# microsoft/tutel

Measured on AMD Instinct MI355X. Metric: MoE-layer fwd tokens/sec, 4096 tok x H=2048 x E=64 top-2, higher is better.
Workload: dtype bf16

## Files before the change

### include/tutel_amd.h

```cpp
#ifndef TUTEL_AMD_H
#define TUTEL_AMD_H

#include <stddef.h>
#include <stdint.h>

#ifdef __cplusplus
extern "C" {
#endif

#define TUTEL_AMD_ABI_VERSION 1

typedef void *tutel_stream_t;

enum { TUTEL_F32 = 0, TUTEL_F16 = 1, TUTEL_BF16 = 2, TUTEL_F64 = 3 };
enum { TUTEL_ACT_NONE = 0, TUTEL_ACT_RELU = 1, TUTEL_ACT_GELU = 2, TUTEL_ACT_SILU = 3 };

int tutel_amd_abi_version(void);
const char *tutel_amd_target_arch(void);
const char *tutel_amd_last_error(void);

size_t tutel_amd_routing_workspace_bytes(int T, int E, int k);

int tutel_amd_gate_topk(const void *in, int dtype, int apply_softmax, int T, int E, int k,
                        int normalize_gate, void *scores_out, int32_t *idx, void *gates, void *ws,
// ... 16 lines not shown

int tutel_amd_slot_map(const int32_t *idx, const int32_t *loc, int T, int E, int k, int capacity,
                       int32_t *slot_map, tutel_stream_t stream);

int tutel_amd_cumsum_sub_one(const int32_t *mask, int32_t *out, int T, int E,
                             tutel_stream_t stream);

int tutel_amd_fast_encode(const void *x, int dtype, const int32_t *slot_map, const void *gates,
                          int gate_dtype, int T, int M, int n_slots, int capacity, int num_experts,
                          int chunk_rows, int expert_slice, int ep_world, void *out,
                          tutel_stream_t stream);

int tutel_amd_fast_decode(const void *buf, int dtype, const int32_t *idx, const int32_t *loc,
                          const void *gates, int gate_dtype, int T, int M, int k, int capacity,
                          int num_experts, int chunk_rows, int expert_slice, int ep_world, void *out,
                          tutel_stream_t stream);

int tutel_amd_gate_grad(const void *x, const void *buf, int dtype, const int32_t *idx,
                        const int32_t *loc, int T, int M, int k, int capacity, float *ggate,
                        tutel_stream_t stream);

int tutel_amd_expert_gemm(const void *A, int64_t a_stride_e, int64_t a_stride_w, int a_rows_per_w,
                          int lda, const void *W, int w_kmajor, int64_t w_stride_e, int ldw,
                          const void *bias, int64_t bias_stride_e, void *D, int64_t d_stride_e,
                          int64_t d_stride_w, int d_rows_per_w, int ldd, int E_loc, int R, int N,
                          int K, int dtype, int act, const int32_t *row_counts, int row_align,
                          tutel_stream_t stream);

int tutel_amd_expert_gemm_gather(const void *X, int ldx, const int32_t *slot_map, int T,
                                 const void *zero_row, const void *W, int w_kmajor,
                                 int64_t w_stride_e, int ldw, const void *bias,
                                 int64_t bias_stride_e, void *D, int64_t d_stride_e, int ldd,
                                 int E_loc, int R, int N, int K, int dtype, int act,
                                 const int32_t *row_counts, int row_align, tutel_stream_t stream);

int tutel_amd_expert_ffn(const void *A, int64_t x_stride_e, int ldx, const int32_t *slot_map, int T, const void *zero_row,
                         const void *W1, int64_t w1_stride_e, int ldw1, const void *b1, int64_t b1_stride_e, void *hid,
                         int64_t hid_stride_e, int ldh, const void *W2, int64_t w2_stride_e, int ldw2, const void *b2,
                         int64_t b2_stride_e, void *D, int64_t d_stride_e, int ldd, int E_loc, int R, int M, int H, int M_out,
                         int dtype, int act, tutel_stream_t stream);

int tutel_amd_expert_gemm_glu(const void *A, int64_t a_stride_e, int64_t a_stride_w,
                              int a_rows_per_w, int lda, const void *W, int w_kmajor,
                              int64_t w_stride_e, int ldw, const void *bias, int64_t bias_stride_e,
                              const void *G, void *D, int64_t d_stride_e, int64_t d_stride_w,
                              int d_rows_per_w, int ldd, int E_loc, int R, int N, int K, int dtype,
                              int act, const int32_t *row_counts, int row_align,
                              tutel_stream_t stream);

int tutel_amd_expert_gemm_gate_up(const void *A, int64_t a_stride_e, int64_t a_stride_w, int a_rows_per_w, int lda,
                                  const void *W_gate, const void *W_up, int64_t w_stride_e, int ldw, void *D, int64_t d_stride_e,
                                  int64_t d_stride_w, int d_rows_per_w, int ldd, int E_loc, int R, int N, int K, int dtype, int act,
                                  const int32_t *row_counts, int row_align, tutel_stream_t stream);

typedef struct tutel_amd_ep_comm tutel_amd_ep_comm_t;
#define TUTEL_AMD_EP_ID_BYTES 128

int tutel_amd_ep_load_rccl(const char *path_hint );
int tutel_amd_ep_unique_id(void *out, size_t bytes );
int tutel_amd_ep_comm_create(const void *id, size_t bytes, int world, int rank, tutel_amd_ep_comm_t **out);
int tutel_amd_ep_comm_destroy(tutel_amd_ep_comm_t *comm);
typedef int (*tutel_amd_exchange_fn)(void *user, const void *send, void *recv, size_t bytes_per_peer, int world);
int tutel_amd_ep_comm_create_hosted(int world, int rank, tutel_amd_exchange_fn fn, void *user, tutel_amd_ep_comm_t **out);
int tutel_amd_ep_comm_info(const tutel_amd_ep_comm_t *comm, int *world, int *rank);

typedef struct tutel_amd_ep_segment tutel_amd_ep_segment_t;
#define TUTEL_AMD_IPC_HANDLE_BYTES 64
int tutel_amd_ep_segment_alloc(size_t bytes, int flag_memory, tutel_amd_ep_segment_t **out, void *handle_out, size_t handle_bytes);
int tutel_amd_ep_segment_open(tutel_amd_ep_segment_t *seg, int world, int rank, const void *handles, size_t handle_bytes);
void *tutel_amd_ep_segment_ptr(const tutel_amd_ep_segment_t *seg, int peer);
int tutel_amd_ep_segment_read(const tutel_amd_ep_segment_t *seg, size_t off, void *dst, size_t bytes, tutel_stream_t stream);
int tutel_amd_ep_segment_free(tutel_amd_ep_segment_t *seg);
size_t tutel_amd_ep_flag_bytes(void);
int tutel_amd_ep_comm_create_ipc(int world, int rank, tutel_amd_ep_comm_t **out);
int tutel_amd_ep_comm_attach_ipc(tutel_amd_ep_comm_t *comm, tutel_amd_ep_segment_t *flags, int timeout_ms);
int tutel_amd_ep_comm_has_ipc(const tutel_amd_ep_comm_t *comm);
int tutel_amd_ep_ipc_set_timeout(tutel_amd_ep_comm_t *comm, int timeout_ms);
int tutel_amd_ep_ipc_status(tutel_amd_ep_comm_t *comm);
int tutel_amd_ep_ipc_exchange(tutel_amd_ep_comm_t *comm, tutel_amd_ep_segment_t *seg, const void *send, size_t bytes_per_peer,
                              size_t recv_off, tutel_stream_t stream);
int tutel_amd_ep_ipc_selfcheck(tutel_amd_ep_comm_t *comm, tutel_amd_ep_segment_t *seg, size_t bytes_per_peer, int passes, int flavour,
                               int side_stream, unsigned long long *mismatch, tutel_stream_t stream);

int tutel_amd_ep_all_to_all(tutel_amd_ep_comm_t *comm, const void *send, void *recv, size_t bytes_per_peer,
                            tutel_stream_t stream);

typedef int (*tutel_amd_exchange_v_fn)(void *user, const void *send, void *recv, const uint64_t *send_bytes,
                                       const uint64_t *send_offsets, const uint64_t *recv_bytes, int world);
int tutel_amd_ep_comm_set_hosted_v(tutel_amd_ep_comm_t *comm, tutel_amd_exchange_v_fn fn);
int tutel_amd_ep_all_to_all_v(tutel_amd_ep_comm_t *comm, const void *send, void *recv, const uint64_t *send_bytes,
                              const uint64_t *recv_bytes, tutel_stream_t stream);
int tutel_amd_ep_all_gather_v(tutel_amd_ep_comm_t *comm, const void *send, void *recv, const uint64_t *recv_bytes,
                              tutel_stream_t stream);

typedef struct {
  int sliced;
  int experts_per_stage;
  int chunk;
  int rows;
  int gemm_rows;
} tutel_amd_ep_plan_t;
int tutel_amd_ep_plan(int num_experts, int world, int capacity, int degree, int allow_sliced, tutel_amd_ep_plan_t *out);

typedef struct {
  int T, M, H, M_out;
  int num_experts, world, k;
  int capacity;
  int degree;
  int allow_sliced;
  int dtype, gate_dtype, act;
  int is_postscore;
  int w2_kmajor;
  int fuse_encode;
  const void *x;
  const int32_t *slot_map;
  const int32_t *idx, *loc;
  const void *gates;
  const void *w1, *b1, *w2, *b2;
  void *enc, *recv, *hid, *send, *back;
  const void *zero_row;
  const int32_t *row_counts;
  int row_align;
  void *y;
  const struct tutel_amd_ep_segment *peer_seg;
} tutel_amd_ep_args_t;
int tutel_amd_ep_forward(tutel_amd_ep_comm_t *comm, const tutel_amd_ep_args_t *args, tutel_stream_t stream);

typedef struct {
  tutel_amd_ep_args_t ep;
  const void *logits;
  int logits_dtype;
  int normalize_gate;
  void *ws;
  size_t ws_bytes;
  int32_t *dispatch_count;
  int32_t *stats;
  void *l_aux;
  int capacity_limit, alignment, max_capacity;
  int *capacity_out;
  const void *gate_w;
  float *gate_partials;
  size_t gate_partial_bytes;
  void *logits_out;
  void *fl_ws;
  size_t fl_ws_bytes;
} tutel_amd_moe_args_t;
#define TUTEL_AMD_EAGAIN 1000
#define TUTEL_AMD_ENOTSUP 1001
int tutel_amd_moe_forward(tutel_amd_ep_comm_t *comm, const tutel_amd_moe_args_t *args, tutel_stream_t stream);

typedef struct {
  void *ws;
  size_t ws_bytes;
  int32_t *offsets;
  int32_t *capacity;
} tutel_amd_packed_args_t;
typedef struct {
  int rows_bound;
  int tiles_bound;
  int tile_rows;
  int row_limit;
  size_t ws_bytes;
} tutel_amd_packed_plan_t;
int tutel_amd_packed_plan(int T, int E, int k, int M, int H, int M_out, int dtype, int capacity_limit, int alignment,
                          tutel_amd_packed_plan_t *out);
size_t tutel_amd_moe_packed_workspace_bytes(int T, int E, int k, int M, int H, int M_out, int dtype, int capacity_limit,
                                            int alignment);
int tutel_amd_moe_forward_packed(tutel_amd_ep_comm_t *comm, const tutel_amd_moe_args_t *args,
                                 const tutel_amd_packed_args_t *packed, tutel_stream_t stream);
int tutel_amd_moe_forward_packed_glu(tutel_amd_ep_comm_t *comm, const tutel_amd_moe_args_t *args,
                                     const tutel_amd_packed_args_t *packed, const void *w_up, tutel_stream_t stream);

int tutel_amd_packed_layout(const int32_t *dispatch_count, const int32_t *idx, const int32_t *loc, int T, int E, int k,
                            int capacity_limit, int alignment, int rows_bound, int tiles_bound, int32_t *offsets, int32_t *tiles,
                            int32_t *ntiles, int32_t *capacity, int32_t *slot_map, tutel_stream_t stream);
int tutel_amd_expert_gemm_packed(const void *A, int lda, const int32_t *a_rows, int T, const void *zero_row, const void *W,
                                 int w_kmajor, int64_t w_stride_e, int ldw, const void *bias, int64_t bias_stride_e, const void *mul,
// ... 55 lines not shown
```

### tutel_amd/_lib.py

```python
import ctypes
import os
import subprocess

_HERE = os.path.dirname(os.path.abspath(__file__))
LIB_PATH = os.path.join(_HERE, "lib", "libtutel_amd.so")
CSRC_DIR = os.path.join(_HERE, "csrc")

F32, F16, BF16, F64 = 0, 1, 2, 3
ACT_NONE, ACT_RELU, ACT_GELU, ACT_SILU = 0, 1, 2, 3
OPT_GEMM_IMPL, OPT_GEMM_TILE, OPT_DECODE, OPT_EP_STAGE_GRID, OPT_GEMM_PERSIST, OPT_EP_STREAMS, OPT_EP_CANARY, OPT_GEMM_SPLITK, OPT_GEMM_GATHER, OPT_FUSED_LOCATION, OPT_GEMM_STORE, OPT_TIE_RULE, OPT_FFN_FUSED = 0, 1, 2, 3, 4, 5, 6, 7, 8, 9, 10, 11, 12

_vp, _i, _i64, _sz = ctypes.c_void_p, ctypes.c_int, ctypes.c_int64, ctypes.c_size_t

SIGNATURES = {
    "tutel_amd_abi_version": (_i, []),
    "tutel_amd_target_arch": (ctypes.c_char_p, []),
    "tutel_amd_last_error": (ctypes.c_char_p, []),
    "tutel_amd_routing_workspace_bytes": (_sz, [_i, _i, _i]),
    "tutel_amd_gate_topk": (_i, [_vp, _i, _i, _i, _i, _i, _i, _vp, _vp, _vp, _vp, _sz, _vp, _i, _vp]),
    "tutel_amd_gate_proj_splits": (_i, [_i, _i, _i, _i]),
    "tutel_amd_gate_proj": (_i, [_vp, _vp, _i, _i, _i, _i, _vp, _sz, _vp]),
    "tutel_amd_gate_topk_partials": (_i, [_vp, _i, _i, _i, _i, _i, _i, _vp, _vp, _vp, _vp, _vp, _sz, _vp, _i, _vp]),
    "tutel_amd_cache_warm": (_i, [_vp, _sz, _i, _sz, _i, _vp, _vp]),
    "tutel_amd_compute_location": (_i, [_vp, _i, _i, _i, _i, _vp, _sz, _vp, _vp, _vp, _vp, _i, _i, _vp, _i, _vp]),
    "tutel_amd_slot_map": (_i, [_vp, _vp, _i, _i, _i, _i, _vp, _vp]),
    "tutel_amd_cumsum_sub_one": (_i, [_vp, _vp, _i, _i, _vp]),
    "tutel_amd_fast_encode": (_i, [_vp, _i, _vp, _vp, _i, _i, _i, _i, _i, _i, _i, _i, _i, _vp, _vp]),
    "tutel_amd_fast_decode": (_i, [_vp, _i, _vp, _vp, _vp, _i, _i, _i, _i, _i, _i, _i, _i, _i, _vp, _vp]),
    "tutel_amd_gate_grad": (_i, [_vp, _vp, _i, _vp, _vp, _i, _i, _i, _i, _vp, _vp]),
    "tutel_amd_expert_gemm": (_i, [_vp, _i64, _i64, _i, _i, _vp, _i, _i64, _i, _vp, _i64, _vp, _i64,
                                   _i64, _i, _i, _i, _i, _i, _i, _i, _i, _vp, _i, _vp]),
    "tutel_amd_expert_gemm_gather": (_i, [_vp, _i, _vp, _i, _vp, _vp, _i, _i64, _i, _vp, _i64, _vp, _i64, _i,
                                          _i, _i, _i, _i, _i, _i, _vp, _i, _vp]),
    "tutel_amd_expert_ffn": (_i, [_vp, _i64, _i, _vp, _i, _vp, _vp, _i64, _i, _vp, _i64, _vp, _i64, _i, _vp, _i64, _i, _vp, _i64, _vp, _i64, _i,
                                  _i, _i, _i, _i, _i, _i, _i, _vp]),
    "tutel_amd_expert_gemm_glu": (_i, [_vp, _i64, _i64, _i, _i, _vp, _i, _i64, _i, _vp, _i64, _vp, _vp, _i64,
                                       _i64, _i, _i, _i, _i, _i, _i, _i, _i, _vp, _i, _vp]),
    "tutel_amd_expert_gemm_gate_up": (_i, [_vp, _i64, _i64, _i, _i, _vp, _vp, _i64, _i, _vp, _i64, _i64, _i, _i,
                                           _i, _i, _i, _i, _i, _i, _vp, _i, _vp]),
    "tutel_amd_set_option": (_i, [_i, _i]),
    "tutel_amd_probe_tr16": (_i, [_vp, _vp]),
}



class EpPlan(ctypes.Structure):
    _fields_ = [(n, _i) for n in ("sliced", "experts_per_stage", "chunk", "rows", "gemm_rows")]


class EpArgs(ctypes.Structure):
    _fields_ = ([(n, _i) for n in ("T", "M", "H", "M_out", "num_experts", "world", "k", "capacity", "degree", "allow_sliced",
                                   "dtype", "gate_dtype", "act", "is_postscore", "w2_kmajor", "fuse_encode")] +
                [(n, _vp) for n in ("x", "slot_map", "idx", "loc", "gates", "w1", "b1", "w2", "b2",
                                    "enc", "recv", "hid", "send", "back", "zero_row", "row_counts")] +
                [("row_align", _i), ("y", _vp), ("peer_seg", _vp)])


class MoeArgs(ctypes.Structure):
    _fields_ = [("ep", EpArgs), ("logits", _vp), ("logits_dtype", _i), ("normalize_gate", _i), ("ws", _vp), ("ws_bytes", _sz),
                ("dispatch_count", _vp), ("stats", _vp), ("l_aux", _vp),
                ("capacity_limit", _i), ("alignment", _i), ("max_capacity", _i), ("capacity_out", ctypes.POINTER(_i)),
                ("gate_w", _vp), ("gate_partials", _vp), ("gate_partial_bytes", _sz), ("logits_out", _vp),
                ("fl_ws", _vp), ("fl_ws_bytes", _sz)]


class PackedArgs(ctypes.Structure):
    _fields_ = [("ws", _vp), ("ws_bytes", _sz), ("offsets", _vp), ("capacity", _vp)]


class PackedPlan(ctypes.Structure):
    _fields_ = [("rows_bound", _i), ("tiles_bound", _i), ("tile_rows", _i), ("row_limit", _i), ("ws_bytes", _sz)]


SIGNATURES.update({
    "tutel_amd_moe_forward": (_i, [_vp, ctypes.POINTER(MoeArgs), _vp]),
    "tutel_amd_packed_plan": (_i, [_i] * 9 + [ctypes.POINTER(PackedPlan)]),
    "tutel_amd_moe_packed_workspace_bytes": (_sz, [_i] * 9),
    "tutel_amd_moe_forward_packed": (_i, [_vp, ctypes.POINTER(MoeArgs), ctypes.POINTER(PackedArgs), _vp]),
    "tutel_amd_moe_forward_packed_glu": (_i, [_vp, ctypes.POINTER(MoeArgs), ctypes.POINTER(PackedArgs), _vp, _vp]),
    "tutel_amd_packed_layout": (_i, [_vp, _vp, _vp] + [_i] * 7 + [_vp] * 6),
    "tutel_amd_expert_gemm_packed": (_i, [_vp, _i, _vp, _i, _vp, _vp, _i, _i64, _i, _vp, _i64, _vp, _vp] + [_i] * 7 + [_vp] * 4 + [_i, _vp]),
    "tutel_amd_expert_wgrad_packed": (_i, [_vp, _i, _vp, _i, _vp, _i, _i, _vp, _vp] + [_i] * 5 + [_vp, _vp]),
    "tutel_amd_expert_bgrad_packed": (_i, [_vp, _i, _vp, _i, _i, _i, _vp, _vp]),
    "tutel_amd_expert_wgrad_packed_f32": (_i, [_vp, _i, _vp, _i, _vp, _i, _i, _vp, _vp] + [_i] * 5 + [_vp, _vp]),
    "tutel_amd_expert_bgrad_packed_f32": (_i, [_vp, _i, _vp, _i, _i, _i, _vp, _vp]),
    "tutel_amd_gate_grad_packed": (_i, [_vp, _vp, _i, _vp, _vp] + [_i] * 4 + [_vp, _vp, _vp]),
    "tutel_amd_fast_decode_packed": (_i, [_vp, _i, _vp, _vp, _vp] + [_i] * 5 + [_vp, _vp, _vp]),
    "tutel_amd_ep_load_rccl": (_i, [ctypes.c_char_p]),
    "tutel_amd_ep_unique_id": (_i, [_vp, _sz]),
    "tutel_amd_ep_comm_create": (_i, [_vp, _sz, _i, _i, ctypes.POINTER(_vp)]),
    "tutel_amd_ep_comm_destroy": (_i, [_vp]),
    "tutel_amd_ep_comm_create_hosted": (_i, [_i, _i, _vp, _vp, ctypes.POINTER(_vp)]),
    "tutel_amd_ep_comm_info": (_i, [_vp, ctypes.POINTER(_i), ctypes.POINTER(_i)]),
    "tutel_amd_ep_all_to_all": (_i, [_vp, _vp, _vp, _sz, _vp]),
    "tutel_amd_ep_comm_set_hosted_v": (_i, [_vp, _vp]),
    "tutel_amd_ep_all_to_all_v": (_i, [_vp, _vp, _vp, ctypes.POINTER(ctypes.c_uint64), ctypes.POINTER(ctypes.c_uint64), _vp]),
    "tutel_amd_ep_all_gather_v": (_i, [_vp, _vp, _vp, ctypes.POINTER(ctypes.c_uint64), _vp]),
    "tutel_amd_ep_plan": (_i, [_i, _i, _i, _i, _i, ctypes.POINTER(EpPlan)]),
    "tutel_amd_ep_forward": (_i, [_vp, ctypes.POINTER(EpArgs), _vp]),
    "tutel_amd_ep_segment_alloc": (_i, [_sz, _i, ctypes.POINTER(_vp), _vp, _sz]),
    "tutel_amd_ep_segment_open": (_i, [_vp, _i, _i, _vp, _sz]),
    "tutel_amd_ep_segment_ptr": (_vp, [_vp, _i]),
    "tutel_amd_ep_segment_read": (_i, [_vp, _sz, _vp, _sz, _vp]),
    "tutel_amd_ep_segment_free": (_i, [_vp]),
    "tutel_amd_ep_flag_bytes": (_sz, []),
    "tutel_amd_ep_comm_create_ipc": (_i, [_i, _i, ctypes.POINTER(_vp)]),
    "tutel_amd_ep_comm_attach_ipc": (_i, [_vp, _vp, _i]),
    "tutel_amd_ep_comm_has_ipc": (_i, [_vp]),
# ... 64 lines not shown
```

### tutel_amd/csrc/common.h

```cpp
#pragma once
#include <hip/hip_runtime.h>
#include <stdint.h>
#include <stdio.h>
#include <string.h>

#include "../../include/tutel_amd.h"

#define WAVE 64

void tutel_set_error(const char *fmt, ...);
int tutel_get_option(int key);

int tutel_stage_begin(int stage, hipStream_t st);
void tutel_stage_end(int token, hipStream_t st);
void tutel_stage_hint(int stage);
void tutel_gemm_corun_hint(int on);
int tutel_gemm_corun();
void tutel_stage_range_push(int stage);
void tutel_stage_range_pop();
struct StageScope {
  int token;
  hipStream_t st;
  StageScope(int stage, hipStream_t s) : token(tutel_stage_begin(stage, s)), st(s) { tutel_stage_range_push(stage); }
  ~StageScope() {
    tutel_stage_end(token, st);
    tutel_stage_range_pop();
  }
};

#define EP_NCAN 16
struct PeerCanary {
  const uint32_t *epoch;
  long long off;
  int world;
  int stale;
};
struct EncodePeer {
  const uint64_t *tab;
  long long off;
  int rank, rows;
  int slot0;
  PeerCanary can;
};
int tutel_encode_launch(const void *x, int dtype, const int32_t *slot_map, const void *gates, int gate_dtype, int T, int M,
                        int n_slots, int capacity, int num_experts, int chunk_rows, int expert_slice, int ep_world, void *out,
                        const EncodePeer &peer, hipStream_t st);
int tutel_expert_gemm_peer(const void *A, int64_t a_stride_e, int64_t a_stride_w, int a_rows_per_w, int lda, const void *W,
                           int w_kmajor, int64_t w_stride_e, int ldw, const void *bias, int64_t bias_stride_e,
                           const uint64_t *d_peer, int64_t d_peer_off, int64_t d_stride_e, int d_rows_per_w, int ldd, int E_loc,
                           int R, int N, int K, int dtype, int act, const PeerCanary &can, hipStream_t st);

int tutel_expert_gemm_gather_fl(const void *X, int ldx, int32_t *slot_map, int T, const void *zero_row, const void *W, int64_t w_stride_e,
                                int ldw, const void *bias, int64_t bias_stride_e, void *D, int64_t d_stride_e, int ldd, int E_loc, int R,
                                int N, int K, int dtype, int act, const uint8_t *idx8, int n, int32_t *loc, hipStream_t st);
int tutel_expert_ffn(const void *X, int64_t x_stride_e, int ldx, const int32_t *slot_map, int T, const void *zero_row, const void *W1,
                     int64_t w1_stride_e, int ldw1, const void *b1, int64_t b1_stride_e, void *hid, int64_t hid_stride_e, int ldh,
                     const void *W2, int64_t w2_stride_e, int ldw2, const void *b2, int64_t b2_stride_e, void *D, int64_t d_stride_e, int ldd,
                     int E_loc, int R, int M, int H, int M_out, int dtype, int act, const uint8_t *idx8, int n, int32_t *loc, int query,
                     hipStream_t st);
struct RouteFinish;
void tutel_route_finish_args(int T, int E, int k, void *ws, RouteFinish *out);
int tutel_decode_finish_launch(const void *buf, int dtype, const int32_t *idx, const int32_t *loc, const void *gates, int gate_dtype, int T, int M,
                               int k, int capacity, int num_experts, void *out, const RouteFinish &fin, hipStream_t st);
#define PK_TILE_ROWS 256
int tutel_expert_gemm_packed(const void *A, int lda, const int32_t *a_rows, int T, const void *zero_row, const void *W, int64_t w_stride_e,
                             int ldw, const void *bias, int64_t bias_stride_e, void *D, int ldd, int E, int rows_bound, int N, int K, int dtype,
                             int act, const int32_t *off, const int32_t *tiles, const int32_t *ntiles, const int32_t *cap, int tiles_bound,
                             hipStream_t st);
int tutel_expert_gemm_packed_ex(const void *A, int lda, const int32_t *a_rows, int T, const void *zero_row, const void *W, int w_kmajor,
                                int64_t w_stride_e, int ldw, const void *bias, int64_t bias_stride_e, const void *mul, void *D, int ldd, int E,
                                int rows_bound, int N, int K, int dtype, int act, const int32_t *off, const int32_t *tiles, const int32_t *ntiles,
                                const int32_t *cap, int tiles_bound, hipStream_t st);
int tutel_expert_gemm_gate_up_packed(const void *A, int lda, const int32_t *a_rows, int T, const void *zero_row, const void *W_gate,
                                     const void *W_up, int64_t w_stride_e, int ldw, void *D, int ldd, int E, int rows_bound, int N, int K,
                                     int dtype, int act, const int32_t *off, const int32_t *tiles, const int32_t *ntiles, const int32_t *cap,
                                     int tiles_bound, hipStream_t st);
int tutel_decode_packed_launch(const void *buf, int dtype, const int32_t *idx, const int32_t *loc, const void *gates, int gate_dtype, int T,
                               int M, int k, int row_limit, const int32_t *off, void *out, hipStream_t st);
int tutel_gate_topk_launch(const void *in, const float *partials, int splits, int dtype, int T, int E, int k, int normalize_gate,
                           void *logits_out, int32_t *idx, void *gates, void *ws, int32_t *clear_map, int clear_n, uint8_t *idx8,
                           hipStream_t st);

#define TUTEL_REQUIRE(cond, ...)           \
  do {                                     \
    if (!(cond)) {                         \
      tutel_set_error(__VA_ARGS__);        \
      return -1;                           \
    }                                      \
  } while (0)

#define TUTEL_CHECK_LAUNCH(what)                                                    \
  do {                                                                              \
    hipError_t _e = hipGetLastError();                                              \
    if (_e != hipSuccess) {                                                         \
      tutel_set_error("%s: launch failed: %s", what, hipGetErrorString(_e));        \
      return (int)_e;                                                               \
    }                                                                               \
  } while (0)

struct bf16_t { uint16_t v; };
struct f16_t { _Float16 v; };

__device__ __forceinline__ uint16_t f32_to_bf16_bits(float f) {
  uint32_t u = __float_as_uint(f);
  if ((u & 0x7fffffffu) > 0x7f800000u) return 0x7fc0;
  u += 0x7fffu + ((u >> 16) & 1u);
  return (uint16_t)(u >> 16);
// ... 127 lines not shown
```

### tutel_amd/csrc/ep.hip

```cpp
#include <dlfcn.h>
#include <stdlib.h>

#include <vector>

#include <rccl/rccl.h>

#include "common.h"
#include "routing_dev.h"

struct RcclApi {
  void *handle;
  ncclResult_t (*GetUniqueId)(ncclUniqueId *);
  ncclResult_t (*CommInitRank)(ncclComm_t *, int, ncclUniqueId, int);
  ncclResult_t (*CommDestroy)(ncclComm_t);
  ncclResult_t (*AllToAll)(const void *, void *, size_t, ncclDataType_t, ncclComm_t, hipStream_t);
  const char *(*GetErrorString)(ncclResult_t);
  ncclResult_t (*GroupStart)();
  ncclResult_t (*GroupEnd)();
  ncclResult_t (*Send)(const void *, size_t, ncclDataType_t, int, ncclComm_t, hipStream_t);
  ncclResult_t (*Recv)(void *, size_t, ncclDataType_t, int, ncclComm_t, hipStream_t);
};
static RcclApi g_rccl = {};

extern "C" int tutel_amd_ep_load_rccl(const char *path) {
// ... 646 lines not shown

extern "C" int tutel_amd_ep_plan(int E, int W, int capacity, int degree, int allow_sliced, tutel_amd_ep_plan_t *out) {
  TUTEL_REQUIRE(out != nullptr && E >= 1 && W >= 1 && E % W == 0 && degree >= 1 && degree <= EP_MAX_SPLIT && capacity >= 0,
                "tutel_amd_ep_plan: bad sizes E=%d W=%d C=%d degree=%d", E, W, capacity, degree);
  const int E_loc = E / W;
  out->sliced = (allow_sliced && E_loc >= degree && E_loc % degree == 0) ? 1 : 0;
  if (out->sliced) {
    out->experts_per_stage = E_loc / degree;
    out->chunk = capacity;
  } else {
    TUTEL_REQUIRE(capacity % degree == 0, "tutel_amd_ep_plan: capacity %d is not a multiple of a2a_ffn_overlap_degree %d", capacity, degree);
    out->experts_per_stage = E_loc;
    out->chunk = capacity / degree;
  }
  out->rows = out->experts_per_stage * out->chunk;
  out->gemm_rows = W * out->chunk;
  return 0;
}

extern "C" int tutel_amd_ep_forward(tutel_amd_ep_comm_t *c, const tutel_amd_ep_args_t *a, tutel_stream_t stream) {
  TUTEL_REQUIRE(a != nullptr, "tutel_amd_ep_forward: null arguments");
  const int W = a->world, E = a->num_experts, C = a->capacity, T = a->T, M = a->M, H = a->H, Mo = a->M_out, k = a->k;
  TUTEL_REQUIRE(W >= 1 && E >= 1 && E % W == 0 && T >= 0 && M >= 1 && H >= 1 && Mo >= 1 && k >= 1 && C >= 0,
                "tutel_amd_ep_forward: bad sizes");
  TUTEL_REQUIRE(c == nullptr ? W == 1 : c->world == W, "tutel_amd_ep_forward: communicator world size does not match (%d)", W);
  TUTEL_REQUIRE(a->dtype == TUTEL_BF16 || a->dtype == TUTEL_F16, "tutel_amd_ep_forward: bf16 / fp16 experts only (got dtype %d)", a->dtype);
  TUTEL_REQUIRE((T == 0 || (a->x && a->idx && a->loc && a->y)) && (a->slot_map || C == 0) && a->w1 && a->w2, "tutel_amd_ep_forward: null pointer");
  if (T == 0 && c == nullptr) return 0;
  const int E_loc = E / W, es = 2;
  hipStream_t cur = (hipStream_t)stream;
  const void *enc_gates = a->is_postscore ? nullptr : a->gates;
  const void *dec_gates = a->is_postscore ? a->gates : nullptr;
  TUTEL_REQUIRE(a->gates != nullptr || T == 0, "tutel_amd_ep_forward: null gates");
  TUTEL_REQUIRE(a->row_counts == nullptr || (W == 1 && c == nullptr && a->degree <= 1), "tutel_amd_ep_forward: row counts (megablocks) need a single rank");
  const int32_t *rcnt = a->row_counts;
  const int ralign = a->row_counts != nullptr && a->row_align >= 1 ? a->row_align : 1;

  if (C == 0) {
    if (T > 0) HIP_CHECK(hipMemsetAsync(a->y, 0, (size_t)T * Mo * es, cur), "hipMemsetAsync");
    return 0;
  }

  if (c == nullptr && a->degree <= 1 && a->is_postscore && a->fuse_encode) {
    TUTEL_REQUIRE(a->hid && a->send && a->zero_row, "tutel_amd_ep_forward: null workspace");
    int rc = TUTEL_AMD_ENOTSUP;
    if (rcnt == nullptr && a->w2_kmajor) {
      Range r("tutel_amd.expert_ffn");
      rc = tutel_expert_ffn(a->x, 0, M, a->slot_map, T, a->zero_row, a->w1, (int64_t)H * M, M, a->b1, H, a->hid, (int64_t)C * H, H, a->w2,
                            (int64_t)H * Mo, H, a->b2, Mo, a->send, (int64_t)C * Mo, Mo, E_loc, C, M, H, Mo, a->dtype, a->act, nullptr, 0, nullptr, 0, cur);
      if (rc != 0 && rc != TUTEL_AMD_ENOTSUP) return rc;
    }
    if (rc == TUTEL_AMD_ENOTSUP) {
      Range r("tutel_amd.expert_fc1");
      rc = tutel_amd_expert_gemm_gather(a->x, M, a->slot_map, T, a->zero_row, a->w1, 1, (int64_t)H * M, M, a->b1, H, a->hid,
                                        (int64_t)C * H, H, E_loc, C, H, M, a->dtype, a->act, rcnt, ralign, cur);
      if (rc) return rc;
      Range r2("tutel_amd.expert_fc2");
      rc = tutel_amd_expert_gemm(a->hid, (int64_t)C * H, 0, C, H, a->w2, a->w2_kmajor, (int64_t)H * Mo, a->w2_kmajor ? H : Mo, a->b2,
                                 Mo, a->send, (int64_t)C * Mo, 0, C, Mo, E_loc, C, Mo, H, a->dtype, TUTEL_ACT_NONE, rcnt, ralign, cur);
      if (rc) return rc;
    }
    Range r("tutel_amd.fast_decode");
    return tutel_amd_fast_decode(a->send, a->dtype, a->idx, a->loc, dec_gates, a->gate_dtype, T, Mo, k, C, E, 0, 0, 1, a->y, cur);
  }

  const bool ipc = a->peer_seg != nullptr;
  TUTEL_REQUIRE(a->recv && a->hid && a->back && (ipc || (a->enc && a->send)), "tutel_amd_ep_forward: null workspace");
  TUTEL_REQUIRE(rcnt == nullptr, "tutel_amd_ep_forward: row counts need the fused-encode single-rank route (is_postscore, fuse_encode)");
  const int degree = a->degree < 1 ? 1 : a->degree;
  tutel_amd_ep_plan_t pl;
  if (tutel_amd_ep_plan(E, W, C, degree, a->allow_sliced, &pl) != 0) return -1;
  const int s = pl.experts_per_stage, cc = pl.chunk, rows = pl.rows, R = pl.gemm_rows;
  const int chunk_rows = pl.sliced ? 0 : cc, expert_slice = pl.sliced ? s : 0;
  int rc;

  const size_t msg_in = (size_t)W * rows * M * es, msg_out = (size_t)W * rows * Mo * es;
  const size_t hid_stage = (size_t)s * R * H * es;
  const tutel_amd_ep_segment *seg = a->peer_seg;
  long long recv_off = 0, back_off = 0;
  if (ipc) {
    if (ipc_check(c, "tutel_amd_ep_forward") != 0) return -1;
    TUTEL_REQUIRE(seg->tab_dev != nullptr && seg->world == W && seg->rank == c->rank, "tutel_amd_ep_forward: the peer segment is not open for this communicator");
    recv_off = (const char *)a->recv - (const char *)seg->local;
    back_off = (const char *)a->back - (const char *)seg->local;
    TUTEL_REQUIRE(recv_off >= 0 && back_off >= 0 && (size_t)recv_off + degree * msg_in <= seg->bytes && (size_t)back_off + degree * msg_out <= seg->bytes &&
                      recv_off % 16 == 0 && back_off % 16 == 0,
                  "tutel_amd_ep_forward: recv / back must lie inside the peer segment");
  }
  auto stage_gemms = [&](int i, hipStream_t st) -> int {
    const char *recv_i = (const char *)a->recv + (size_t)i * msg_in;
    char *hid_i = (char *)a->hid + (size_t)i * hid_stage;
    const int e0 = pl.sliced ? i * s : 0;
    const char *w1 = (const char *)a->w1 + (size_t)e0 * H * M * es, *w2 = (const char *)a->w2 + (size_t)e0 * H * Mo * es;
    const char *b1 = a->b1 ? (const char *)a->b1 + (size_t)e0 * H * es : nullptr, *b2 = a->b2 ? (const char *)a->b2 + (size_t)e0 * Mo * es : nullptr;
    int r1;
    {
      Range r("tutel_amd.expert_fc1");
      tutel_stage_hint(TUTEL_STAGE_FC1);
      r1 = tutel_amd_expert_gemm(recv_i, (int64_t)cc * M, (int64_t)rows * M, cc, M, w1, 1, (int64_t)H * M, M, b1, H, hid_i,
                                 (int64_t)R * H, 0, R, H, s, R, H, M, a->dtype, a->act, nullptr, 1, st);
      tutel_stage_hint(-1);
      if (r1) return r1;
    }
    Range r("tutel_amd.expert_fc2");
    if (ipc)
      return tutel_expert_gemm_peer(hid_i, (int64_t)R * H, 0, R, H, w2, a->w2_kmajor, (int64_t)H * Mo, a->w2_kmajor ? H : Mo, b2, Mo, seg->tab_dev,
                                    back_off + (long long)(((size_t)i * W + c->rank) * rows * Mo * es), (int64_t)cc * Mo, cc, Mo, s, R, Mo, H, a->dtype,
                                    TUTEL_ACT_NONE, producer_canary(c, seg, 1, i), st);
    char *send_i = (char *)a->send + (size_t)i * msg_out;
    return tutel_amd_expert_gemm(hid_i, (int64_t)R * H, 0, R, H, w2, a->w2_kmajor, (int64_t)H * Mo, a->w2_kmajor ? H : Mo, b2, Mo, send_i,
                                 (int64_t)cc * Mo, (int64_t)rows * Mo, cc, Mo, s, R, Mo, H, a->dtype, TUTEL_ACT_NONE, nullptr, 1, st);
  };
// ... 135 lines not shown
    splits = tutel_amd_gate_proj_splits(T, a.M, E, a.dtype);
    TUTEL_REQUIRE(splits > 0, "tutel_amd_moe_forward: the in-call gate projection does not cover T=%d, M=%d, E=%d, dtype=%d (pass logits)", T, a.M, E, a.dtype);
    TUTEL_REQUIRE(a.x != nullptr && m->gate_partials != nullptr && m->gate_partial_bytes >= (size_t)splits * T * E * sizeof(float),
                  "tutel_amd_moe_forward: gate_partials must hold %d x %d x %d floats", splits, T, E);
  }
  TUTEL_REQUIRE(a.slot_map && (T == 0 || (a.idx && a.loc && a.gates)), "tutel_amd_moe_forward: null routing buffers");
  if (T == 0 && c == nullptr) return 0;
  const bool dropless = a.capacity <= 0;
  TUTEL_REQUIRE(!dropless || (c == nullptr && a.world == 1 && m->stats != nullptr && m->capacity_out != nullptr && m->max_capacity >= 1),
                "tutel_amd_moe_forward: dropless routing needs a single rank, stats, capacity_out and max_capacity");
  int32_t *smap = const_cast<int32_t *>(a.slot_map);
  int rc;
  const int Ho = a.H, Mo = a.M_out;
  bool fl = !dropless && c == nullptr && a.world == 1 && a.degree <= 1 && a.is_postscore && a.fuse_encode && T > 0 && k <= 8 && E <= 128 &&
            (long long)k * T <= 15360 && m->fl_ws != nullptr && m->fl_ws_bytes >= (((size_t)k * T + 15) & ~(size_t)15) &&
            (a.dtype == TUTEL_BF16 || a.dtype == TUTEL_F16) && a.row_counts == nullptr && a.hid && a.send && a.zero_row && a.loc && a.w1 &&
            ((uintptr_t)m->fl_ws & 15) == 0;
  if (fl) {
    TUTEL_REQUIRE(k >= 1 && k <= E, "tutel_amd_moe_forward: need 1 <= k <= E (got k=%d, E=%d)", k, E);
    TUTEL_REQUIRE(m->ws_bytes >= tutel_amd_routing_workspace_bytes(T, E, k), "tutel_amd_moe_forward: routing workspace too small (%zu bytes, need %zu)",
                  m->ws_bytes, tutel_amd_routing_workspace_bytes(T, E, k));
  }
  if (fl) {
    char keep[512];
    strncpy(keep, tutel_amd_last_error(), sizeof(keep) - 1);
    keep[sizeof(keep) - 1] = 0;
    fl = tutel_expert_gemm_gather_fl(a.x, a.M, smap, T, a.zero_row, a.w1, (int64_t)Ho * a.M, a.M, a.b1, Ho, a.hid, (int64_t)a.capacity * Ho, Ho, E,
                                     a.capacity, Ho, a.M, a.dtype, a.act, (const uint8_t *)m->fl_ws, k * T, nullptr, (hipStream_t)stream) == 0;
    if (!fl) tutel_set_error("%s", keep);
  }
  if (fl) {
    hipStream_t st = (hipStream_t)stream;
    uint8_t *idx8 = (uint8_t *)m->fl_ws;
    if (project) {
      rc = tutel_amd_gate_proj(a.x, m->gate_w, a.dtype, T, a.M, E, m->gate_partials, m->gate_partial_bytes, stream);
      if (rc) return rc;
    }
    rc = tutel_gate_topk_launch(project ? nullptr : m->logits, project ? m->gate_partials : nullptr, splits, m->logits_dtype, T, E, k,
                                m->normalize_gate, project ? m->logits_out : nullptr, const_cast<int32_t *>(a.idx), const_cast<void *>(a.gates),
                                m->ws, nullptr, 0, idx8, st);
    if (rc) return rc;
    if (m->capacity_out != nullptr) *m->capacity_out = a.capacity;
    rc = TUTEL_AMD_ENOTSUP;
    if (a.w2_kmajor) {
      Range r("tutel_amd.expert_ffn");
      rc = tutel_expert_ffn(a.x, 0, a.M, smap, T, a.zero_row, a.w1, (int64_t)Ho * a.M, a.M, a.b1, Ho, a.hid, (int64_t)a.capacity * Ho, Ho, a.w2,
                            (int64_t)Ho * Mo, Ho, a.b2, Mo, a.send, (int64_t)a.capacity * Mo, Mo, E, a.capacity, a.M, Ho, Mo, a.dtype, a.act, idx8, k * T,
                            const_cast<int32_t *>(a.loc), 0, st);
      if (rc != 0 && rc != TUTEL_AMD_ENOTSUP) return rc;
    }
    if (rc == TUTEL_AMD_ENOTSUP) {
      Range r("tutel_amd.expert_fc1");
      rc = tutel_expert_gemm_gather_fl(a.x, a.M, smap, T, a.zero_row, a.w1, (int64_t)Ho * a.M, a.M, a.b1, Ho, a.hid, (int64_t)a.capacity * Ho, Ho,
                                       E, a.capacity, Ho, a.M, a.dtype, a.act, idx8, k * T, const_cast<int32_t *>(a.loc), st);
      if (rc) return rc;
      Range r2("tutel_amd.expert_fc2");
      rc = tutel_amd_expert_gemm(a.hid, (int64_t)a.capacity * Ho, 0, a.capacity, Ho, a.w2, a.w2_kmajor, (int64_t)Ho * Mo, a.w2_kmajor ? Ho : Mo,
                                 a.b2, Mo, a.send, (int64_t)a.capacity * Mo, 0, a.capacity, Mo, E, a.capacity, Mo, Ho, a.dtype, TUTEL_ACT_NONE,
                                 nullptr, 1, stream);
      if (rc) return rc;
    }
    Range r("tutel_amd.fast_decode");
    RouteFinish fin;
    tutel_route_finish_args(T, E, k, m->ws, &fin);
    fin.on = 1;
    fin.dispatch_count = m->dispatch_count;
    fin.stats = m->stats;
    fin.l_aux = m->l_aux;
    fin.l_aux_dtype = m->logits_dtype;
    return tutel_decode_finish_launch(a.send, a.dtype, a.idx, a.loc, a.gates, m->logits_dtype, T, Mo, k, a.capacity, E, a.y, fin, st);
  }
  if (project && T > 0) {
    rc = tutel_amd_gate_proj(a.x, m->gate_w, a.dtype, T, a.M, E, m->gate_partials, m->gate_partial_bytes, stream);
    if (rc) return rc;
    rc = tutel_amd_gate_topk_partials(m->gate_partials, splits, a.dtype, T, E, k, m->normalize_gate, m->logits_out, nullptr,
                                      const_cast<int32_t *>(a.idx), const_cast<void *>(a.gates), m->ws, m->ws_bytes,
                                      dropless ? nullptr : smap, dropless ? 0 : E * a.capacity, stream);
  } else {
    rc = tutel_amd_gate_topk(m->logits, m->logits_dtype, 1, T, E, k, m->normalize_gate, nullptr, const_cast<int32_t *>(a.idx),
                             const_cast<void *>(a.gates), m->ws, m->ws_bytes, dropless ? nullptr : smap, dropless ? 0 : E * a.capacity, stream);
  }
  if (rc) return rc;
  rc = tutel_amd_compute_location(a.idx, T, E, k, 1, m->ws, m->ws_bytes, const_cast<int32_t *>(a.loc), m->dispatch_count, m->stats,
                                  m->l_aux, m->logits_dtype, dropless ? 0 : a.capacity, dropless ? nullptr : smap, dropless ? 0 : 1, stream);
  if (rc) return rc;
  tutel_amd_ep_args_t e = a;
  e.gate_dtype = m->logits_dtype;
  if (dropless) {
    hipStream_t st = (hipStream_t)stream;
    HIP_CHECK(hipMemcpyAsync(m->capacity_out, m->stats, sizeof(int), hipMemcpyDeviceToHost, st), "hipMemcpyAsync");
    HIP_CHECK(hipStreamSynchronize(st), "hipStreamSynchronize");
    int cap = *m->capacity_out;
    if (m->capacity_limit > 0 && cap > m->capacity_limit) cap = m->capacity_limit;
    const int al = m->alignment >= 1 ? m->alignment : 1;
    cap = (cap + al - 1) / al * al;
    *m->capacity_out = cap;
    if (cap > m->max_capacity) return TUTEL_AMD_EAGAIN;
    if (cap == 0) return hipMemsetAsync(a.y, 0, (size_t)T * a.M_out * 2, st) == hipSuccess ? 0 : -1;
    rc = tutel_amd_slot_map(a.idx, a.loc, T, E, k, cap, smap, stream);
    if (rc) return rc;
    e.capacity = cap;
  } else if (m->capacity_out != nullptr) {
    *m->capacity_out = a.capacity;
  }
  return tutel_amd_ep_forward(c, &e, stream);
}
```

### tutel_amd/csrc/expert_gemm.hip

```cpp
#include <stdlib.h>

#include <mutex>

#include "common.h"

#include "gemm_dev.h"

template <typename T, bool W_KMAJOR, int ACT, bool NT, bool ROT, bool PACKED = false>
__global__ __launch_bounds__(GM_THREADS, 2) void expert_gemm_kernel(GemmArgs p) {
  constexpr int BK = 64, NBUF = 2;
  constexpr int LDK = BK + 8;
  constexpr int A_TILE = GM_BM * LDK;
  constexpr int W_TILE = W_KMAJOR ? GM_BN * LDK : BK * GM_LDN;
  constexpr int CPR = BK / 8;
  constexpr int RPP = GM_THREADS / CPR;
  constexpr int NLA = GM_BM / RPP;
  constexpr int NLW = W_KMAJOR ? GM_BN / RPP : BK / 16;
  extern __shared__ __attribute__((aligned(16))) unsigned char smem[];
  uint16_t *sA = reinterpret_cast<uint16_t *>(smem);
  uint16_t *sW = sA + NBUF * A_TILE;

  const int tid = threadIdx.x, lane = tid & 63, wid = tid >> 6;
  const int wm = wid >> 1, wn = wid & 1;

  int nb = gridDim.x;
  if (PACKED) {
    nb = min(nb, __builtin_amdgcn_readfirstlane(*p.pk_ntiles) * 2 * p.ntn);
    if ((int)blockIdx.x >= nb) return;
  }
  int w;
  {
    const int b = blockIdx.x, q = nb >> 3, r = nb & 7, xcd = b & 7, pos = b >> 3;
    w = (xcd < r ? xcd * (q + 1) : r * (q + 1) + (xcd - r) * q) + pos;
  }
  int nt, e, m0, row_limit;
  bool rot_on = p.rot_on;
  if (PACKED) {
    const int h = w / p.ntn, ti = h >> 1;
    nt = w % p.ntn;
    e = __builtin_amdgcn_readfirstlane(p.pk_tiles[2 * ti]);
    m0 = __builtin_amdgcn_readfirstlane(p.pk_tiles[2 * ti + 1]) + (h & 1) * GM_BM;
    row_limit = __builtin_amdgcn_readfirstlane(p.pk_off[e + 1]);
    rot_on = __builtin_amdgcn_readfirstlane(*p.pk_cap) < GB_BM;
  } else {
    const int mt = w % p.ntm;
    nt = (w / p.ntm) % p.ntn;
    e = w / (p.ntm * p.ntn);
    m0 = mt * GM_BM;
    row_limit = p.R;
    if (p.row_counts != nullptr) {
      int c = p.row_counts[e];
      c = (c + p.row_align - 1) / p.row_align * p.row_align;
      row_limit = min(row_limit, c);
    }
  }
  const int n0 = nt * GM_BN;
  if (m0 >= row_limit) return;

  const uint16_t *Ae = reinterpret_cast<const uint16_t *>(p.A) + (size_t)e * p.a_stride_e;
// ... 220 lines not shown
  do {                                                                                 \
    _Pragma("unroll") for (int mi = 0; mi < 2; ++mi)                                   \
      FA[mi] = *reinterpret_cast<const u32x4 *>(ca + a_row + mi * 32 * GL_BK + frag_k[KK]); \
    _Pragma("unroll") for (int ni = 0; ni < 2; ++ni) {                                 \
      if (W_KMAJOR) {                                                                  \
        FW[ni] = *reinterpret_cast<const u32x4 *>(cw + wk_row + ni * 32 * GL_BK + frag_k[KK]); \
      } else {                                                                         \
        const uint16_t *ptr = cw + wt_row + (KK) * 16 * GM_BN + (ni ? wt_c1 : wt_c0);  \
        s16x4_t lo = __builtin_amdgcn_ds_read_tr16_b64_v4i16(                          \
            (__attribute__((address_space(3))) s16x4_t *)(ptr));                       \
        s16x4_t hi = __builtin_amdgcn_ds_read_tr16_b64_v4i16(                          \
            (__attribute__((address_space(3))) s16x4_t *)(ptr + 4 * GM_BN));           \
        u32x2 lo2 = __builtin_bit_cast(u32x2, lo), hi2 = __builtin_bit_cast(u32x2, hi); \
        u32x4 f = {lo2[0], lo2[1], hi2[0], hi2[1]};                                    \
        FW[ni] = f;                                                                    \
      }                                                                                \
    }                                                                                  \
  } while (0)
#define GL_MMA(FA, FW)                                                                 \
  do {                                                                                 \
    _Pragma("unroll") for (int ni = 0; ni < 2; ++ni)                                   \
      _Pragma("unroll") for (int mi = 0; mi < 2; ++mi)                                 \
        acc[ni][mi] = Mma<T>::run(FW[ni], FA[mi], acc[ni][mi]);                        \
  } while (0)

  GL_ISSUE(0, 0);
  __syncthreads();

  for (int kt = 0; kt < nk; ++kt) {
    const int buf = kt & 1;
    if (kt + 1 < nk) GL_ISSUE(kt + 1, buf ^ 1);

    const uint16_t *ca = sA + buf * GL_STAGE, *cw = sW + buf * GL_STAGE;
    u32x4 fa[4][2], fw[4][2];
    GL_LOAD_FRAGS(fa[0], fw[0], 0);
    GL_LOAD_FRAGS(fa[1], fw[1], 1);
    GL_LOAD_FRAGS(fa[2], fw[2], 2);
    GL_LOAD_FRAGS(fa[3], fw[3], 3);
    __builtin_amdgcn_sched_barrier(0);
    GL_MMA(fa[0], fw[0]);
    GL_MMA(fa[1], fw[1]);
    GL_MMA(fa[2], fw[2]);
    GL_MMA(fa[3], fw[3]);

    __syncthreads();
  }
#undef GL_ISSUE
#undef GL_LOAD_FRAGS
#undef GL_MMA

  gemm_epilogue<T, ACT>(p, acc, bias_r, e, m0, n0, wm, wn, l31, kg, row_limit);
}

template <typename T, bool W_KMAJOR, int ACT, int NI, int NS, bool BUF = false, int BM = GB_BM, bool FL = false>
__global__ __launch_bounds__(BM * 2, 2) void expert_gemm_big_kernel(GemmArgs p) {
  extern __shared__ __attribute__((aligned(16))) unsigned char smem[];
  const int nb = gridDim.x;
  int w;
  {
    const int b = blockIdx.x, q = nb >> 3, r = nb & 7, xcd = b & 7, pos = b >> 3;
    w = (xcd < r ? xcd * (q + 1) : r * (q + 1) + (xcd - r) * q) + pos;
  }
  gemm_big_tile<T, W_KMAJOR, ACT, NI, NS, BUF, BM, FL>(p, w / (p.ntm * p.ntn), w % p.ntm, (w / p.ntm) % p.ntn, smem);
}

#define PP_BUF (4 * GL_STAGE)

template <typename T, int ACT, bool W_ONCE, bool RAGGED = false, bool EARLY_BIAS = false, bool SPLITK = false, bool PACKED = false,
          bool GATE_UP = false>
__global__ __launch_bounds__(GB_THREADS, 2) void expert_gemm_pp_kernel(GemmArgs p) {
  extern __shared__ __attribute__((aligned(16))) unsigned char smem[];
  uint16_t *lds = reinterpret_cast<uint16_t *>(smem);

  const int tid = threadIdx.x, lane = tid & 63;
  const int wid = __builtin_amdgcn_readfirstlane(tid >> 6);
  const int wm = wid >> 1, wn = wid & 1;

  static_assert(!(PACKED && SPLITK), "the packed layout never splits K");
  static_assert(!GATE_UP || (!SPLITK && !EARLY_BIAS), "the gate/up form: no split, no bias");
  constexpr bool packed = PACKED;
  int nb = gridDim.x;
  if (packed) {
    nb = min(nb, __builtin_amdgcn_readfirstlane(*p.pk_ntiles) * p.ntn);
    if ((int)blockIdx.x >= nb) return;
  }
  int w;
  {
    const int b = blockIdx.x, q = nb >> 3, r = nb & 7, xcd = b & 7, pos = b >> 3;
    w = (xcd < r ? xcd * (q + 1) : r * (q + 1) + (xcd - r) * q) + pos;
  }
  const int half = SPLITK ? (w & 1) : 0;
  if (SPLITK) w >>= 1;
  const int tile_id = w;
  int e, nt, m0, row_limit;
  bool rot_on = p.rot_on;
  if constexpr (packed) {
    const int ti = w / p.ntn;
    nt = w % p.ntn;
    e = __builtin_amdgcn_readfirstlane(p.pk_tiles[2 * ti]);
    m0 = __builtin_amdgcn_readfirstlane(p.pk_tiles[2 * ti + 1]);
    row_limit = __builtin_amdgcn_readfirstlane(p.pk_off[e + 1]);
    rot_on = __builtin_amdgcn_readfirstlane(*p.pk_cap) < GB_BM;
  } else {
    const int mt = w % p.ntm;
    nt = (w / p.ntm) % p.ntn;
    e = w / (p.ntm * p.ntn);
    m0 = mt * GB_BM;
    row_limit = p.R;
    if (p.row_counts != nullptr) {
      int c = p.row_counts[e];
      c = (c + p.row_align - 1) / p.row_align * p.row_align;
      row_limit = min(row_limit, c);
    }
  }
  const int n0 = nt * (GATE_UP ? 128 : 256);
  if (m0 >= row_limit) return;
// ... 314 lines not shown
  const size_t lds = (size_t)8 * 64 * EP_PITCH;
  auto kern = expert_gemm_pp_kernel<T, ACT, false, false, false, true>;
  if (!tutel_lds_optin((const void *)kern, lds)) return -1;
  hipLaunchKernelGGL(kern, dim3((unsigned)(2 * tiles)), dim3(GB_THREADS), lds, st, b);
  TUTEL_CHECK_LAUNCH("tutel_amd_expert_gemm");
  return 0;
}

template <typename T, int ACT>
static int launch_pp(const GemmArgs &a, hipStream_t st) {
  GemmArgs b = a;
  b.ntm = (a.R + GB_BM - 1) / GB_BM;
  b.ntn = (a.N + 255) / 256;
  const int tail_rows = b.R % GB_BM;
  const bool ragged = b.row_counts != nullptr || (tail_rows != 0 && tail_rows <= GB_BM - 32);
  const bool early = tutel_get_option(TUTEL_OPT_GEMM_PERSIST) != 0;
  if (b.ntm == 1 && (long long)b.E_loc * b.ntn >= 256)
    return ragged ? launch_pp_cfg<T, ACT, true, true>(b, st) : (early ? launch_pp_cfg<T, ACT, true, false, true>(b, st) : launch_pp_cfg<T, ACT, true>(b, st));
  return ragged ? launch_pp_cfg<T, ACT, false, true>(b, st) : (early ? launch_pp_cfg<T, ACT, false, false, true>(b, st) : launch_pp_cfg<T, ACT, false>(b, st));
}

template <typename T, int ACT>
static int launch_pp_packed(const GemmArgs &a, int tiles_bound, hipStream_t st) {
  GemmArgs b = a;
  b.ntm = 1;
  b.ntn = (a.N + 255) / 256;
  const long long grid = (long long)tiles_bound * b.ntn;
  TUTEL_REQUIRE(grid >= 1 && grid < 0x7fffffffLL, "tutel_expert_gemm_packed: grid too large");
  const size_t lds = (size_t)8 * 64 * EP_PITCH;
  auto kern = (long long)a.E_loc * b.ntn >= 256 ? expert_gemm_pp_kernel<T, ACT, true, true, false, false, true>
                                                 : expert_gemm_pp_kernel<T, ACT, false, true, false, false, true>;
  if (!tutel_lds_optin((const void *)kern, lds)) return -1;
  hipLaunchKernelGGL(kern, dim3((unsigned)grid), dim3(GB_THREADS), lds, st, b);
  TUTEL_CHECK_LAUNCH("tutel_expert_gemm_packed");
  return 0;
}

template <typename T, int ACT, bool PACKED>
static int launch_gate_up(const GemmArgs &a, int tiles_bound, hipStream_t st) {
  GemmArgs b = a;
  b.ntm = PACKED ? 1 : (a.R + GB_BM - 1) / GB_BM;
  b.ntn = (a.N + 127) / 128;
  const long long grid = PACKED ? (long long)tiles_bound * b.ntn : (long long)a.E_loc * b.ntm * b.ntn;
  TUTEL_REQUIRE(grid >= 1 && grid < 0x7fffffffLL, "tutel_amd_expert_gemm_gate_up: grid too large");
  const size_t lds = (size_t)8 * 64 * EP_PITCH;
  auto kern = PACKED && (long long)a.E_loc * b.ntn >= 256 ? expert_gemm_pp_kernel<T, ACT, PACKED, true, false, false, PACKED, true>
                                                          : expert_gemm_pp_kernel<T, ACT, false, true, false, false, PACKED, true>;
  if (!tutel_lds_optin((const void *)kern, lds)) return -1;
  hipLaunchKernelGGL(kern, dim3((unsigned)grid), dim3(GB_THREADS), lds, st, b);
  TUTEL_CHECK_LAUNCH("tutel_amd_expert_gemm_gate_up");
  return 0;
}

template <typename T, bool KM, int ACT, int NI, int NS = 2, bool BUF = false, int BM = GB_BM, bool FL = false>
static int launch_big(const GemmArgs &a, hipStream_t st) {
  GemmArgs b = a;
  b.ntm = (a.R + BM - 1) / BM;
  b.ntn = (a.N + NI * 64 - 1) / (NI * 64);
  const size_t lds_k = (size_t)NS * (BM / 128 + NI / 2) * GL_STAGE * 2 + (FL ? 16384 : 0), lds_e = BUF ? (size_t)(BM / 32) * 64 * (NI * 64 + 16) : 0;
  const size_t lds = lds_k > lds_e ? lds_k : lds_e;
  auto kern = expert_gemm_big_kernel<T, KM, ACT, NI, NS, BUF, BM, FL>;
  if (!tutel_lds_optin((const void *)kern, lds)) return -1;
  hipLaunchKernelGGL(kern, dim3(a.E_loc * b.ntm * b.ntn), dim3(BM * 2), lds, st, b);
  TUTEL_CHECK_LAUNCH("tutel_amd_expert_gemm");
  return 0;
}

template <typename T, bool KM, int ACT>
static int launch_glds(const GemmArgs &a, int grid, hipStream_t st) {
  hipLaunchKernelGGL((expert_gemm_glds_kernel<T, KM, ACT, true, true>), dim3(grid), dim3(GM_THREADS),
                     (size_t)4 * GL_STAGE * 2, st, a);
  TUTEL_CHECK_LAUNCH("tutel_amd_expert_gemm");
  return 0;
}

__global__ void probe_tr16_kernel(uint16_t *out) {
  __shared__ __attribute__((aligned(16))) uint16_t lds[256];
  const int l = threadIdx.x;
  for (int i = l; i < 256; i += 64) lds[i] = (uint16_t)i;
  __syncthreads();
  s16x4_t t = __builtin_amdgcn_ds_read_tr16_b64_v4i16((__attribute__((address_space(3))) s16x4_t *)(lds + l * 4));
#pragma unroll
  for (int j = 0; j < 4; ++j) out[l * 4 + j] = (uint16_t)t[j];
}

extern "C" int tutel_amd_probe_tr16(uint16_t *out, tutel_stream_t stream) {
  TUTEL_REQUIRE(out != nullptr, "tutel_amd_probe_tr16: null pointer");
  hipLaunchKernelGGL(probe_tr16_kernel, dim3(1), dim3(64), 0, (hipStream_t)stream, out);
  TUTEL_CHECK_LAUNCH("tutel_amd_probe_tr16");
  return 0;
}

static constexpr size_t gemm_lds_bytes(bool kmajor) {
  return (size_t)(2 * GM_BM * (64 + 8) + 2 * (kmajor ? GM_BN * (64 + 8) : 64 * GM_LDN)) * 2;
}

template <typename T, bool KM, int ACT>
static int launch_cfg(const GemmArgs &a, int grid, hipStream_t st) {
  const size_t lds = gemm_lds_bytes(KM);
  auto kern = expert_gemm_kernel<T, KM, ACT, true, true>;
  if (lds > 65536 && !tutel_lds_optin((const void *)kern, lds)) return -1;
  hipLaunchKernelGGL(kern, dim3(grid), dim3(GM_THREADS), lds, st, a);
  TUTEL_CHECK_LAUNCH("tutel_amd_expert_gemm");
  return 0;
}

template <typename T, bool KM, int ACT>
static int launch_gemm(const GemmArgs &a, int grid, hipStream_t st) {
  const int impl = tutel_get_option(TUTEL_OPT_GEMM_IMPL), big = tutel_get_option(TUTEL_OPT_GEMM_TILE);
  const bool ring256_ok = KM && a.fits32 && a.N >= 256 && a.R <= GM_BM;
  const bool ring256 = ring256_ok && (impl == 4 || (impl < 0 && (long long)a.E_loc * ((a.N + 255) / 256) >= 256));
  if (a.fl_idx8 != nullptr) {
    if (!(ring256 && KM && big <= 0 && a.a_rows != nullptr && a.row_counts == nullptr && a.fl_n >= 1 && a.fl_n <= 15360 && a.E_loc <= 128 && a.K >= 2 * GL_BK)) {
      tutel_set_error("tutel_expert_gemm_gather_fl: this launch does not take the fused-location ring kernel");
      return TUTEL_AMD_ENOTSUP;
    }
    if (a.fl_loc == nullptr) return 0;
    return launch_big<T, true, ACT, 4, 3, true, 128, KM>(a, st);
  }
  if (a.N >= GM_BN && big != 0) {
    const long long mt256 = (long long)a.E_loc * ((a.R + GB_BM - 1) / GB_BM);
    const long long t256 = mt256 * ((a.N + 255) / 256), t128 = mt256 * ((a.N + 127) / 128);
    const bool corun_pp = tutel_gemm_corun() && big < 0 && a.R > GM_BM && t256 >= 96 && t256 < 192;
    if (KM && a.fits32 && a.mul == nullptr && a.R > GM_BM && t256 >= 96 && t256 < 192 && (big < 0 || big == 4) &&
        tutel_get_option(TUTEL_OPT_GEMM_SPLITK) == 1) {
      const int rc = launch_pp_splitk<T, ACT>(a, st);
      if (rc <= 0) return rc;
    }
    const bool pp_one_round = big < 0 && a.R > GM_BM && t256 > 128 && t256 < 192;
    if (KM && a.fits32 && (big == 4 || corun_pp || pp_one_round || (big < 0 && a.R > GM_BM && t256 >= 192))) return launch_pp<T, ACT>(a, st);
    if (big == 1 || big == 4 || (big < 0 && a.R > GM_BM && t256 >= 192)) return launch_big<T, KM, ACT, 4>(a, st);
    if (KM && big == 2) return launch_big<T, true, ACT, 2, 2>(a, st);
    if (KM && (big == 3 || (big < 0 && a.R > GM_BM && t128 >= 192)))
      return a.fits32 && tutel_get_option(TUTEL_OPT_GEMM_IMPL) != 2 ? launch_big<T, true, ACT, 2, 3, true>(a, st) : launch_big<T, true, ACT, 2, 3>(a, st);
  }
  if (ring256) return launch_big<T, true, ACT, 4, 3, true, 128>(a, st);
  const bool use_dma = impl < 0 ? KM : (impl == 1 || impl == 4);
  if (use_dma) return launch_glds<T, KM, ACT>(a, grid, st);
  return launch_cfg<T, KM, ACT>(a, grid, st);
}

template <typename T, bool KM>
static int launch_gemm_act(const GemmArgs &a, int act, int grid, hipStream_t st) {
  switch (act) {
    case TUTEL_ACT_NONE: return launch_gemm<T, KM, TUTEL_ACT_NONE>(a, grid, st);
    case TUTEL_ACT_RELU: return launch_gemm<T, KM, TUTEL_ACT_RELU>(a, grid, st);
    case TUTEL_ACT_GELU: return launch_gemm<T, KM, TUTEL_ACT_GELU>(a, grid, st);
    case TUTEL_ACT_SILU: return launch_gemm<T, KM, TUTEL_ACT_SILU>(a, grid, st);
    default: tutel_set_error("tutel_amd_expert_gemm: unknown activation %d", act); return -1;
  }
}

int tutel_gemm_args(const void *A, int64_t a_stride_e, int64_t a_stride_w, int a_rows_per_w, int lda, const void *W, int w_kmajor,
                    int64_t w_stride_e, int ldw, const void *bias, int64_t bias_stride_e, void *D, int64_t d_stride_e, int64_t d_stride_w,
                    int d_rows_per_w, int ldd, int E_loc, int R, int N, int K, int dtype, int act, const int32_t *row_counts, int row_align,
                    const int32_t *a_rows, int a_rows_mod, const void *a_zero, const void *mul, const uint64_t *d_peer, int64_t d_peer_off,
                    const PeerCanary *d_can, const uint8_t *fl_idx8, int fl_n, int32_t *fl_loc, GemmArgs *out) {
  (void)w_kmajor; (void)act;
  TUTEL_REQUIRE(dtype == TUTEL_BF16 || dtype == TUTEL_F16, "tutel_amd_expert_gemm: dtype must be bf16 or fp16 (got %d)", dtype);
  TUTEL_REQUIRE(E_loc >= 0 && R >= 0 && N >= 1 && K >= 1, "tutel_amd_expert_gemm: bad sizes E_loc=%d R=%d N=%d K=%d", E_loc, R, N, K);
  TUTEL_REQUIRE(K % 64 == 0, "tutel_amd_expert_gemm: K=%d must be a multiple of 64", K);
  TUTEL_REQUIRE(N % 8 == 0, "tutel_amd_expert_gemm: N=%d must be a multiple of 8", N);
  if (E_loc == 0 || R == 0) return 1;
  TUTEL_REQUIRE(A && W && (D || d_peer), "tutel_amd_expert_gemm: null pointer");
  TUTEL_REQUIRE(d_peer == nullptr || (mul == nullptr && d_peer_off % 16 == 0), "tutel_amd_expert_gemm: peer stores exclude the gated form");
  TUTEL_REQUIRE(a_rows_per_w >= 1 && d_rows_per_w >= 1, "tutel_amd_expert_gemm: rows_per_w must be >= 1");
  TUTEL_REQUIRE(lda % 8 == 0 && ldw % 8 == 0 && ldd % 4 == 0 && a_stride_e % 8 == 0 && a_stride_w % 8 == 0 &&
                    w_stride_e % 8 == 0 && d_stride_e % 4 == 0 && d_stride_w % 4 == 0 && bias_stride_e % 4 == 0,
                "tutel_amd_expert_gemm: leading dimensions / strides must keep rows 16-byte aligned");
  TUTEL_REQUIRE(((uintptr_t)A % 16) == 0 && ((uintptr_t)W % 16) == 0 && ((uintptr_t)D % 8) == 0 && ((uintptr_t)bias % 8) == 0,
                "tutel_amd_expert_gemm: pointers must be 16-byte aligned");
  TUTEL_REQUIRE(row_counts == nullptr || row_align >= 1, "tutel_amd_expert_gemm: row_align must be >= 1");

  GemmArgs &a = *out;
  a.A = A; a.a_stride_e = a_stride_e; a.a_stride_w = a_stride_w; a.a_rpw = a_rows_per_w; a.lda = lda;
  a.W = W; a.w_stride_e = w_stride_e; a.ldw = ldw;
  a.bias = bias; a.bias_stride_e = bias_stride_e;
  a.D = D; a.d_stride_e = d_stride_e; a.d_stride_w = d_stride_w; a.d_rpw = d_rows_per_w; a.ldd = ldd;
  a.E_loc = E_loc; a.R = R; a.N = N; a.K = K;
  a.row_counts = row_counts; a.row_align = row_align < 1 ? 1 : row_align;
  a.a_rows = a_rows; a.a_rows_mod = a_rows_mod; a.a_zero = a_zero;
  a.a_span_bytes = 0;
  bool fits32 = true;
  {
    const long long span = a_rows != nullptr ? (long long)a_rows_mod * lda * 2
                                             : ((long long)((R - 1) / a_rows_per_w) * a_stride_w + (long long)a_rows_per_w * lda) * 2;
    fits32 = span < 0x7ffff000LL;
    a.a_span_bytes = (int)span;
  }
  fits32 = fits32 && ((long long)N * ldw + K) * 2 < 0xffffff00LL;
  a.fits32 = fits32;
  a.rot_on = R < GB_BM;
  a.sgather = tutel_get_option(TUTEL_OPT_GEMM_GATHER) != 0 && (long long)E_loc * R * 4 < 0x7fffffffLL;
  {
    const int ds = tutel_get_option(TUTEL_OPT_GEMM_STORE);
    const long long span = ((long long)((R - 1) / d_rows_per_w) * (d_stride_w < 0 ? -d_stride_w : d_stride_w) + (long long)(d_rows_per_w < R ? d_rows_per_w : R) * ldd + N) * 2;
    a.d_store = (ds == 0 || span >= 0x7fffffffLL) ? 0 : (ds == 2 ? 2 : 1);
    if (d_peer != nullptr) {
      const long long pspan = ((long long)E_loc * d_stride_e + (long long)d_rows_per_w * ldd + N) * 2;
      a.d_store = (ds != 0 && d_rows_per_w % 8 == 0 && pspan < 0x7fffffffLL) ? 1 : 0;
    }
  }
  a.mul = mul;
  a.fl_idx8 = fl_idx8; a.fl_n = fl_n; a.fl_loc = fl_loc;
  a.d_peer = d_peer; a.d_peer_off = d_peer_off;
  a.d_can = d_can != nullptr ? *d_can : PeerCanary{nullptr, 0, 0, 0};
  TUTEL_REQUIRE(((uintptr_t)mul % 8) == 0, "tutel_amd_expert_gemm_glu: gating operand must be 8-byte aligned");
  TUTEL_REQUIRE(a_rows == nullptr || (a_rows_mod >= 1 && a_zero != nullptr && ((uintptr_t)a_zero % 16) == 0),
                "tutel_amd_expert_gemm_gather: need a_rows_mod >= 1 and a 16-byte aligned zero row");
  a.ntm = (R + GM_BM - 1) / GM_BM;
  a.ntn = (N + GM_BN - 1) / GM_BN;
  a.pk_off = a.pk_tiles = a.pk_ntiles = a.pk_cap = nullptr;
  a.w_up = nullptr;
  return 0;
}

static int expert_gemm_impl(const void *A, int64_t a_stride_e, int64_t a_stride_w,
                                     int a_rows_per_w, int lda, const void *W, int w_kmajor,
                                     int64_t w_stride_e, int ldw, const void *bias,
                                     int64_t bias_stride_e, void *D, int64_t d_stride_e,
                                     int64_t d_stride_w, int d_rows_per_w, int ldd, int E_loc,
                                     int R, int N, int K, int dtype, int act,
                                     const int32_t *row_counts, int row_align,
                                     const int32_t *a_rows, int a_rows_mod, const void *a_zero,
                                     const void *mul, tutel_stream_t stream, const uint64_t *d_peer = nullptr,
                                     int64_t d_peer_off = 0, const PeerCanary *d_can = nullptr, const uint8_t *fl_idx8 = nullptr,
                                     int fl_n = 0, int32_t *fl_loc = nullptr) {
  GemmArgs a;
  const int brc = tutel_gemm_args(A, a_stride_e, a_stride_w, a_rows_per_w, lda, W, w_kmajor, w_stride_e, ldw, bias, bias_stride_e, D, d_stride_e,
                                  d_stride_w, d_rows_per_w, ldd, E_loc, R, N, K, dtype, act, row_counts, row_align, a_rows, a_rows_mod, a_zero, mul,
                                  d_peer, d_peer_off, d_can, fl_idx8, fl_n, fl_loc, &a);
  if (brc != 0) return brc < 0 ? brc : 0;
  long long grid_ll = (long long)E_loc * a.ntm * a.ntn;
  TUTEL_REQUIRE(grid_ll < 0x7fffffffLL, "tutel_amd_expert_gemm: grid too large");
  const int grid = (int)grid_ll;
  hipStream_t st = (hipStream_t)stream;
  auto go = [&]() -> int {
    if (dtype == TUTEL_BF16)
      return w_kmajor ? launch_gemm_act<bf16_t, true>(a, act, grid, st) : launch_gemm_act<bf16_t, false>(a, act, grid, st);
    return w_kmajor ? launch_gemm_act<f16_t, true>(a, act, grid, st) : launch_gemm_act<f16_t, false>(a, act, grid, st);
  };
  if (fl_idx8 != nullptr && fl_loc == nullptr) return go();
  StageScope stage(act != TUTEL_ACT_NONE ? TUTEL_STAGE_FC1 : TUTEL_STAGE_FC2, st);
  return go();
}

extern "C" int tutel_amd_expert_gemm(const void *A, int64_t a_stride_e, int64_t a_stride_w,
                                     int a_rows_per_w, int lda, const void *W, int w_kmajor,
                                     int64_t w_stride_e, int ldw, const void *bias,
                                     int64_t bias_stride_e, void *D, int64_t d_stride_e,
                                     int64_t d_stride_w, int d_rows_per_w, int ldd, int E_loc,
                                     int R, int N, int K, int dtype, int act,
                                     const int32_t *row_counts, int row_align,
                                     tutel_stream_t stream) {
  return expert_gemm_impl(A, a_stride_e, a_stride_w, a_rows_per_w, lda, W, w_kmajor, w_stride_e, ldw, bias,
                          bias_stride_e, D, d_stride_e, d_stride_w, d_rows_per_w, ldd, E_loc, R, N, K, dtype, act,
                          row_counts, row_align, nullptr, 0, nullptr, nullptr, stream);
}

int tutel_expert_gemm_peer(const void *A, int64_t a_stride_e, int64_t a_stride_w, int a_rows_per_w, int lda, const void *W,
                           int w_kmajor, int64_t w_stride_e, int ldw, const void *bias, int64_t bias_stride_e,
                           const uint64_t *d_peer, int64_t d_peer_off, int64_t d_stride_e, int d_rows_per_w, int ldd, int E_loc,
                           int R, int N, int K, int dtype, int act, const PeerCanary &can, hipStream_t st) {
  TUTEL_REQUIRE(d_peer != nullptr, "tutel_expert_gemm_peer: null peer table");
  return expert_gemm_impl(A, a_stride_e, a_stride_w, a_rows_per_w, lda, W, w_kmajor, w_stride_e, ldw, bias, bias_stride_e, nullptr,
                          d_stride_e, 0, d_rows_per_w, ldd, E_loc, R, N, K, dtype, act, nullptr, 1, nullptr, 0, nullptr, nullptr,
                          (tutel_stream_t)st, d_peer, d_peer_off, &can);
}

int tutel_expert_gemm_gather_fl(const void *X, int ldx, int32_t *slot_map, int T, const void *zero_row, const void *W, int64_t w_stride_e,
                                int ldw, const void *bias, int64_t bias_stride_e, void *D, int64_t d_stride_e, int ldd, int E_loc, int R,
                                int N, int K, int dtype, int act, const uint8_t *idx8, int n, int32_t *loc, hipStream_t st) {
  TUTEL_REQUIRE(slot_map != nullptr && idx8 != nullptr && T >= 1 && ((uintptr_t)idx8 & 15) == 0, "tutel_expert_gemm_gather_fl: bad arguments");
  if (tutel_get_option(TUTEL_OPT_FUSED_LOCATION) == 0) return TUTEL_AMD_ENOTSUP;
  return expert_gemm_impl(X, 0, 0, R > 0 ? R : 1, ldx, W, 1, w_stride_e, ldw, bias, bias_stride_e, D, d_stride_e, 0, R > 0 ? R : 1, ldd, E_loc,
                          R, N, K, dtype, act, nullptr, 1, slot_map, T, zero_row, nullptr, (tutel_stream_t)st, nullptr, 0, nullptr, idx8, n, loc);
}

extern "C" int tutel_amd_expert_gemm_glu(const void *A, int64_t a_stride_e, int64_t a_stride_w,
                                         int a_rows_per_w, int lda, const void *W, int w_kmajor,
                                         int64_t w_stride_e, int ldw, const void *bias,
                                         int64_t bias_stride_e, const void *G, void *D, int64_t d_stride_e,
                                         int64_t d_stride_w, int d_rows_per_w, int ldd, int E_loc,
                                         int R, int N, int K, int dtype, int act,
                                         const int32_t *row_counts, int row_align,
                                         tutel_stream_t stream) {
  TUTEL_REQUIRE(G != nullptr || E_loc == 0 || R == 0, "tutel_amd_expert_gemm_glu: null gating operand");
  return expert_gemm_impl(A, a_stride_e, a_stride_w, a_rows_per_w, lda, W, w_kmajor, w_stride_e, ldw, bias,
                          bias_stride_e, D, d_stride_e, d_stride_w, d_rows_per_w, ldd, E_loc, R, N, K, dtype, act,
                          row_counts, row_align, nullptr, 0, nullptr, G, stream);
}

extern "C" int tutel_amd_expert_gemm_gather(const void *X, int ldx, const int32_t *slot_map, int T,
                                            const void *zero_row, const void *W, int w_kmajor,
                                            int64_t w_stride_e, int ldw, const void *bias,
                                            int64_t bias_stride_e, void *D, int64_t d_stride_e, int ldd,
                                            int E_loc, int R, int N, int K, int dtype, int act,
                                            const int32_t *row_counts, int row_align,
                                            tutel_stream_t stream) {
  TUTEL_REQUIRE(slot_map != nullptr && T >= 1, "tutel_amd_expert_gemm_gather: need a slot map and T >= 1");
  return expert_gemm_impl(X, 0, 0, R > 0 ? R : 1, ldx, W, w_kmajor, w_stride_e, ldw, bias, bias_stride_e, D,
                          d_stride_e, 0, R > 0 ? R : 1, ldd, E_loc, R, N, K, dtype, act, row_counts, row_align,
                          slot_map, T, zero_row, nullptr, stream);
}

int tutel_expert_gemm_packed(const void *A, int lda, const int32_t *a_rows, int T, const void *zero_row, const void *W, int64_t w_stride_e,
                             int ldw, const void *bias, int64_t bias_stride_e, void *D, int ldd, int E, int rows_bound, int N, int K, int dtype,
                             int act, const int32_t *off, const int32_t *tiles, const int32_t *ntiles, const int32_t *cap, int tiles_bound,
                             hipStream_t st) {
  return tutel_expert_gemm_packed_ex(A, lda, a_rows, T, zero_row, W, 1, w_stride_e, ldw, bias, bias_stride_e, nullptr, D, ldd, E, rows_bound, N,
                                     K, dtype, act, off, tiles, ntiles, cap, tiles_bound, st);
}

template <typename T, int ACT>
static int launch_packed_nmajor(const GemmArgs &a, int tiles_bound, hipStream_t st) {
  GemmArgs b = a;
  b.ntm = 1;
  b.ntn = (a.N + GM_BN - 1) / GM_BN;
  const long long grid = (long long)tiles_bound * 2 * b.ntn;
  TUTEL_REQUIRE(grid >= 1 && grid < 0x7fffffffLL, "tutel_amd_expert_gemm_packed: grid too large");
  const size_t lds = gemm_lds_bytes(false);
  auto kern = expert_gemm_kernel<T, false, ACT, true, true, true>;
  if (lds > 65536 && !tutel_lds_optin((const void *)kern, lds)) return -1;
  hipLaunchKernelGGL(kern, dim3((unsigned)grid), dim3(GM_THREADS), lds, st, b);
  TUTEL_CHECK_LAUNCH("tutel_amd_expert_gemm_packed");
  return 0;
}

int tutel_expert_gemm_packed_ex(const void *A, int lda, const int32_t *a_rows, int T, const void *zero_row, const void *W, int w_kmajor,
                                int64_t w_stride_e, int ldw, const void *bias, int64_t bias_stride_e, const void *mul, void *D, int ldd, int E,
// ... 88 lines not shown
```

### tutel_amd/csrc/gemm_dev.h

```cpp
#pragma once
#include "common.h"

#ifndef GEMM_PROBE
#define GEMM_PROBE(i)
#endif

struct GemmArgs;
int tutel_gemm_args(const void *A, int64_t a_stride_e, int64_t a_stride_w, int a_rows_per_w, int lda, const void *W, int w_kmajor,
                    int64_t w_stride_e, int ldw, const void *bias, int64_t bias_stride_e, void *D, int64_t d_stride_e, int64_t d_stride_w,
                    int d_rows_per_w, int ldd, int E_loc, int R, int N, int K, int dtype, int act, const int32_t *row_counts, int row_align,
                    const int32_t *a_rows, int a_rows_mod, const void *a_zero, const void *mul, const uint64_t *d_peer, int64_t d_peer_off,
                    const PeerCanary *d_can, const uint8_t *fl_idx8, int fl_n, int32_t *fl_loc, GemmArgs *out);
bool tutel_lds_optin(const void *kern, size_t lds);

#define GM_BM 128
#define GM_BN 128
#define GM_THREADS 256
#define GM_LDN (GM_BN + 32)

typedef __attribute__((ext_vector_type(16))) float f32x16;
typedef __attribute__((ext_vector_type(8))) __bf16 bf16x8_t;
typedef __attribute__((ext_vector_type(8))) _Float16 f16x8_t;
typedef __attribute__((ext_vector_type(4))) short s16x4_t;
typedef __attribute__((ext_vector_type(4))) uint32_t u32x4;
typedef __attribute__((ext_vector_type(2))) uint32_t u32x2;
typedef int sgv4 __attribute__((ext_vector_type(4)));
typedef int sgv8 __attribute__((ext_vector_type(8)));

template <typename T> struct Mma;
template <> struct Mma<bf16_t> {
  __device__ static __forceinline__ f32x16 run(u32x4 a, u32x4 b, f32x16 c) {
    return __builtin_amdgcn_mfma_f32_32x32x16_bf16(__builtin_bit_cast(bf16x8_t, a),
                                                  __builtin_bit_cast(bf16x8_t, b), c, 0, 0, 0);
  }
};
template <> struct Mma<f16_t> {
  __device__ static __forceinline__ f32x16 run(u32x4 a, u32x4 b, f32x16 c) {
    return __builtin_amdgcn_mfma_f32_32x32x16_f16(__builtin_bit_cast(f16x8_t, a),
                                                 __builtin_bit_cast(f16x8_t, b), c, 0, 0, 0);
  }
};

#define GEMM_ACT_RUNTIME 99
template <int ACT> __device__ __forceinline__ float activate(float v) {
  if (ACT == TUTEL_ACT_RELU) return fmaxf(v, 0.f);
  if (ACT == TUTEL_ACT_GELU) return 0.5f * v * (1.f + erff(v * 0.70710678118654752440f));
  if (ACT == TUTEL_ACT_SILU) return v / (1.f + expf(-v));
  return v;
}

#define GM_PRELOAD_BIAS() GM_PRELOAD_BIAS_N(2)
#define GM_PRELOAD_BIAS_N(NI_)                                                                    \
  uint2 bias_r[NI_][4];                                                                           \
  {                                                                                               \
    const uint16_t *be_ = p.bias ? reinterpret_cast<const uint16_t *>(p.bias) + (size_t)e * p.bias_stride_e : nullptr; \
    _Pragma("unroll") for (int ni_ = 0; ni_ < NI_; ++ni_)                                         \
      _Pragma("unroll") for (int rg_ = 0; rg_ < 4; ++rg_) {                                       \
        int n_ = n0 + wn * (NI_ * 32) + ni_ * 32 + rg_ * 8 + kg * 4;                              \
        n_ = n_ < p.N ? n_ : p.N - 4;                                                             \
        bias_r[ni_][rg_] = be_ ? *reinterpret_cast<const uint2 *>(be_ + n_) : make_uint2(0u, 0u); \
      }                                                                                           \
  }

struct GemmArgs {
  const void *A; long long a_stride_e, a_stride_w; int a_rpw, lda;
  const void *W; long long w_stride_e; int ldw;
  const void *bias; long long bias_stride_e;
  void *D; long long d_stride_e, d_stride_w; int d_rpw, ldd;
  int E_loc, R, N, K;
  const int32_t *row_counts; int row_align;
  const int32_t *a_rows; int a_rows_mod; const void *a_zero;
  int a_span_bytes;
  bool fits32;
  bool rot_on;
  bool sgather;
  int d_store;
  const uint8_t *fl_idx8; int fl_n; int32_t *fl_loc;
  const void *mul;
  const uint64_t *d_peer; long long d_peer_off;
  PeerCanary d_can;
  float *sk_ws; uint32_t *sk_flags;
  int ntm, ntn;
  int act_rt;
  const int32_t *pk_off, *pk_tiles, *pk_ntiles, *pk_cap;
  const void *w_up;
};

__device__ __forceinline__ uint16_t *gemm_out_row(const GemmArgs &p, int e, int m) {
  const int w = m / p.d_rpw, l = m % p.d_rpw;
  if (p.d_peer != nullptr)
    return reinterpret_cast<uint16_t *>(p.d_peer[w] + p.d_peer_off) + (size_t)e * p.d_stride_e + (size_t)l * p.ldd;
  return reinterpret_cast<uint16_t *>(p.D) + (size_t)e * p.d_stride_e + (size_t)w * p.d_stride_w + (size_t)l * p.ldd;
}

template <typename T, int ACT, int NI = 2>
__device__ __forceinline__ void gemm_epilogue(const GemmArgs &p, f32x16 (&acc)[NI][2], uint2 (&bias_r)[NI][4],
                                              int e, int m0, int n0, int wm, int wn, int l31, int kg,
                                              int row_limit) {
  uint16_t *De = reinterpret_cast<uint16_t *>(p.D) + (size_t)e * p.d_stride_e;
  const uint16_t *Me = p.mul ? reinterpret_cast<const uint16_t *>(p.mul) + (size_t)e * p.d_stride_e : nullptr;
  const bool has_bias = p.bias != nullptr;
#pragma unroll
  for (int mi = 0; mi < 2; ++mi) {
    const int m = m0 + wm * 64 + mi * 32 + l31;
    if (m >= row_limit) continue;
    const size_t roff = (size_t)(m / p.d_rpw) * p.d_stride_w + (size_t)(m % p.d_rpw) * p.ldd;
    uint16_t *drow = p.d_peer != nullptr ? gemm_out_row(p, e, m) : De + roff;
#pragma unroll
    for (int ni = 0; ni < NI; ++ni) {
#pragma unroll
      for (int rg = 0; rg < 4; ++rg) {
        const int n = n0 + wn * (NI * 32) + ni * 32 + rg * 8 + kg * 4;
        if (n >= p.N) continue;
        float v[4];
#pragma unroll
        for (int r = 0; r < 4; ++r) v[r] = acc[ni][mi][rg * 4 + r];
        if (has_bias) {
          const uint2 bb = bias_r[ni][rg];
          uint16_t b4[4] = {(uint16_t)(bb.x & 0xffff), (uint16_t)(bb.x >> 16), (uint16_t)(bb.y & 0xffff), (uint16_t)(bb.y >> 16)};
#pragma unroll
          for (int r = 0; r < 4; ++r) {
            T tb;
            __builtin_memcpy(&tb, &b4[r], 2);
            v[r] += Elem<T>::to_f32(tb);
          }
        }
#pragma unroll
        for (int r = 0; r < 4; ++r) v[r] = activate<ACT>(v[r]);
        if (Me) {
          const uint2 mm = *reinterpret_cast<const uint2 *>(Me + roff + n);
          uint16_t m4[4] = {(uint16_t)(mm.x & 0xffff), (uint16_t)(mm.x >> 16), (uint16_t)(mm.y & 0xffff), (uint16_t)(mm.y >> 16)};
#pragma unroll
          for (int r = 0; r < 4; ++r) {
            T tm;
            __builtin_memcpy(&tm, &m4[r], 2);
            v[r] *= Elem<T>::to_f32(tm);
          }
        }
        uint16_t o[4];
#pragma unroll
        for (int r = 0; r < 4; ++r) {
          T tv = Elem<T>::from_f32(v[r]);
          __builtin_memcpy(&o[r], &tv, 2);
        }
        uint2 ov;
        ov.x = (uint32_t)o[0] | ((uint32_t)o[1] << 16);
        ov.y = (uint32_t)o[2] | ((uint32_t)o[3] << 16);
        *reinterpret_cast<uint2 *>(drow + n) = ov;
      }
    }
  }
  if (p.d_peer != nullptr) peer_canary_store(p.d_peer, p.d_can);
}

__device__ __forceinline__ void gather_rows4(const GemmArgs &p, int e, const int (&gr)[4], int (&q)[4]) {
  q[0] = q[1] = q[2] = q[3] = 0;
  if (p.a_rows != nullptr) {
    const int32_t *m = p.a_rows + (size_t)e * p.R;
    const int q0 = m[gr[0]], q1 = m[gr[1]], q2 = m[gr[2]], q3 = m[gr[3]];
    q[0] = q0; q[1] = q1; q[2] = q2; q[3] = q3;
  }
}

template <bool NT> __device__ __forceinline__ u32x4 ld16(const uint16_t *p) {
  if (NT) return __builtin_nontemporal_load(reinterpret_cast<const u32x4 *>(p));
  return *reinterpret_cast<const u32x4 *>(p);
}

#define GL_BK 64
#define GL_STAGE (GM_BM * GL_BK)

__device__ __forceinline__ void glds16(const uint16_t *g, uint16_t *l, bool nt) {
  if (nt)
    __builtin_amdgcn_global_load_lds((const __attribute__((address_space(1))) void *)g,
                                     (__attribute__((address_space(3))) void *)l, 16, 0, 2);
  else
    __builtin_amdgcn_global_load_lds((const __attribute__((address_space(1))) void *)g,
                                     (__attribute__((address_space(3))) void *)l, 16, 0, 0);
}

template <bool NT>
__device__ __forceinline__ void bdma16(__amdgpu_buffer_rsrc_t rs, int voff, int soff, uint16_t *l) {
  __builtin_amdgcn_raw_ptr_buffer_load_lds(rs, (__attribute__((address_space(3))) void *)l, 16, voff, soff, 0, NT ? 2 : 0);
}

#define EP_PITCH 272
template <typename T, int ACT, int NI = 4, bool GATE_UP = false>
__device__ __forceinline__ void gemm_epilogue_lds(const GemmArgs &p, f32x16 (&acc)[GATE_UP ? 2 * NI : NI][2], uint2 (&bias_r)[NI][4],
                                                  unsigned char *stage, int e, int m0, int n0, int wm, int wn,
                                                  int lane, int row_limit) {
  constexpr int PITCH = NI * 64 + 16;
  const int l31 = lane & 31, kg = lane >> 5;
  uint16_t *De = reinterpret_cast<uint16_t *>(p.D) + (size_t)e * p.d_stride_e;
  const uint16_t *Me = p.mul ? reinterpret_cast<const uint16_t *>(p.mul) + (size_t)e * p.d_stride_e : nullptr;
  const bool has_bias = p.bias != nullptr;
#pragma unroll
  for (int mi = 0; mi < 2; ++mi) {
    const int m = m0 + wm * 64 + mi * 32 + l31;
    size_t roff = 0;
    if (Me) {
      const int mc = min(m, p.R - 1);
      roff = (size_t)(mc / p.d_rpw) * p.d_stride_w + (size_t)(mc % p.d_rpw) * p.ldd;
    }
    unsigned char *srow = stage + (mi * 32 + l31) * PITCH + kg * 8;
#pragma unroll
    for (int ni = 0; ni < NI; ++ni) {
#pragma unroll
      for (int rg = 0; rg < 4; ++rg) {
        float v[4];
#pragma unroll
        for (int r = 0; r < 4; ++r) v[r] = acc[ni][mi][rg * 4 + r];
        if constexpr (GATE_UP) {
#pragma unroll
          for (int r = 0; r < 4; ++r) {
            float a = activate<ACT>(v[r]);
            asm("" : "+v"(a));
            const T g = Elem<T>::from_f32(a);
            v[r] = acc[NI + ni][mi][rg * 4 + r];
            v[r] *= Elem<T>::to_f32(g);
          }
        } else {
        if (has_bias) {
          const uint2 bb = bias_r[ni][rg];
          uint16_t b4[4] = {(uint16_t)(bb.x & 0xffff), (uint16_t)(bb.x >> 16), (uint16_t)(bb.y & 0xffff), (uint16_t)(bb.y >> 16)};
#pragma unroll
          for (int r = 0; r < 4; ++r) {
            T tb;
            __builtin_memcpy(&tb, &b4[r], 2);
            v[r] += Elem<T>::to_f32(tb);
          }
        }
#pragma unroll
        for (int r = 0; r < 4; ++r) v[r] = activate<ACT>(v[r]);
        }
        if (Me) {
          const int n = min(n0 + wn * (NI * 32) + ni * 32 + rg * 8 + kg * 4, p.N - 4);
// ... 22 lines not shown
  constexpr int LPR = NI * 4, RPI = 64 / LPR;
  const int c16 = lane % LPR, r4 = lane / LPR;
  const int n = n0 + wn * (NI * 32) + c16 * 8;
  if (p.d_store != 0 && p.d_peer != nullptr) {
    const int mw = __builtin_amdgcn_readfirstlane(m0 + wm * 64);
    const int wmax = (p.R - 1) / p.d_rpw;
#pragma unroll 4
    for (int it = 0; it < 64 / RPI; ++it) {
      const int mf = mw + it * RPI;
      const int w = min(mf / p.d_rpw, wmax), l0 = mf - (mf / p.d_rpw) * p.d_rpw;
      const __amdgpu_buffer_rsrc_t rs_w = __builtin_amdgcn_make_buffer_rsrc(reinterpret_cast<void *>(p.d_peer[w] + p.d_peer_off), 0, -1, 0x00020000);
      const int row = it * RPI + r4;
      const u32x4 val = *reinterpret_cast<const u32x4 *>(stage + row * PITCH + c16 * 16);
      if (mw + row < row_limit && n < p.N)
        __builtin_amdgcn_raw_buffer_store_b128(val, rs_w, (int)(((size_t)e * p.d_stride_e + (size_t)(l0 + r4) * p.ldd + n) * 2), 0, 17);
    }
    peer_canary_store(p.d_peer, p.d_can);
    return;
  }
  if (p.d_store != 0) {
    const __amdgpu_buffer_rsrc_t rs_d = __builtin_amdgcn_make_buffer_rsrc(De, 0, -1, 0x00020000);
#define EP_STORE_LOOP(AUX)                                                                                        \
    _Pragma("unroll 4") for (int it = 0; it < 64 / RPI; ++it) {                                                   \
      const int row = it * RPI + r4;                                                                              \
      const int m = m0 + wm * 64 + row;                                                                           \
      const u32x4 val = *reinterpret_cast<const u32x4 *>(stage + row * PITCH + c16 * 16);                         \
      if (m < row_limit && n < p.N) {                                                                             \
        const size_t roff = (size_t)(m / p.d_rpw) * p.d_stride_w + (size_t)(m % p.d_rpw) * p.ldd;                 \
        __builtin_amdgcn_raw_buffer_store_b128(val, rs_d, (int)((roff + n) * 2), 0, AUX);                         \
      }                                                                                                           \
    }
    if (p.d_store == 1) { EP_STORE_LOOP(17); } else { EP_STORE_LOOP(2); }
#undef EP_STORE_LOOP
    return;
  }
#pragma unroll 4
  for (int it = 0; it < 64 / RPI; ++it) {
    const int row = it * RPI + r4;
    const int m = m0 + wm * 64 + row;
    const u32x4 val = *reinterpret_cast<const u32x4 *>(stage + row * PITCH + c16 * 16);
    if (m < row_limit && n < p.N) {
      const size_t roff = (size_t)(m / p.d_rpw) * p.d_stride_w + (size_t)(m % p.d_rpw) * p.ldd;
      uint16_t *drow = p.d_peer != nullptr ? gemm_out_row(p, e, m) : De + roff;
      *reinterpret_cast<u32x4 *>(drow + n) = val;
    }
  }
  if (p.d_peer != nullptr) peer_canary_store(p.d_peer, p.d_can);
}

#define GB_BM 256
#define GB_THREADS 512

struct GemmNoHook { __device__ __forceinline__ void operator()() const {} };
template <typename T, bool W_KMAJOR, int ACT, int NI, int NS, bool BUF = false, int BM = GB_BM, bool FL = false, typename Tail = GemmNoHook>
__device__ __forceinline__ void gemm_big_tile(const GemmArgs &p, const int e, const int mt, const int nt, unsigned char *smem,
                                              Tail tail = Tail()) {
  static_assert(!FL || (BUF && NS == 3 && BM == 128 && W_KMAJOR), "FL: the 128 x 256 ring kernel only");
  constexpr int NW = BM / 32;
  constexpr int NSUB = NI / 2;
  constexpr int WPW = 16 * NSUB / NW;
  constexpr int BN = NI * 64;
  constexpr int A_STAGE = (BM / 128) * GL_STAGE;
  uint16_t *sA = reinterpret_cast<uint16_t *>(smem);
  uint16_t *sW = sA + NS * A_STAGE;

  const int tid = threadIdx.x, lane = tid & 63;
  const int wid = __builtin_amdgcn_readfirstlane(tid >> 6);
  const int wm = wid >> 1, wn = wid & 1;
  const int wsub = (wn * NI * 32) / GM_BN, wcol = (wn * NI * 32) % GM_BN;

  const int m0 = mt * BM, n0 = nt * BN;
  GEMM_PROBE(0);

  int row_limit = p.R;
  if (p.row_counts != nullptr) {
    int c = p.row_counts[e];
    c = (c + p.row_align - 1) / p.row_align * p.row_align;
    row_limit = min(row_limit, c);
  }
  if (m0 >= row_limit) {
    tail();
    return;
  }

  const uint16_t *Ae = reinterpret_cast<const uint16_t *>(p.A) + (size_t)e * p.a_stride_e;
  const uint16_t *We = reinterpret_cast<const uint16_t *>(p.W) + (size_t)e * p.w_stride_e;

  const uint16_t *a_src[4], *w_src[WPW];
  int gr4[4], slot4[4];
  constexpr bool SG = BUF && NS == 3;
  typedef int sgv8u __attribute__((ext_vector_type(8), aligned(4)));
  sgv8u sg_q[4];
  const bool fl_on = FL && p.fl_idx8 != nullptr;
  const int mo_ = e * p.R + m0 + 32 * wid;
  const bool sg_on = SG && p.a_rows != nullptr && p.sgather && !fl_on && mo_ + 32 <= p.E_loc * p.R;
#pragma unroll
  for (int i = 0; i < 4; ++i) gr4[i] = min(m0 + 8 * (wid * 4 + i) + (lane >> 3), p.R - 1);
  if (!sg_on && !fl_on) gather_rows4(p, e, gr4, slot4);
#define GB_A_ADDR()                                                                                             \
  _Pragma("unroll") for (int i = 0; i < 4; ++i) {                                                              \
    const int r = 8 * (wid * 4 + i) + (lane >> 3);                                                             \
    const int c = (lane & 7) ^ ((r >> 1) & 7);                                                                 \
    const int gr = gr4[i];                                                                                     \
    a_src[i] = Ae + (size_t)(gr / p.a_rpw) * p.a_stride_w + (size_t)(gr % p.a_rpw) * p.lda + c * 8;            \
    if (p.a_rows != nullptr) {                                                                                 \
      const int q = slot4[i];                                                                                  \
      a_src[i] = (q >= 0 ? reinterpret_cast<const uint16_t *>(p.A) + (size_t)(q % p.a_rows_mod) * p.lda        \
                         : reinterpret_cast<const uint16_t *>(p.a_zero)) + c * 8;                              \
    }                                                                                                          \
  }
  if (!sg_on && !fl_on) { GB_A_ADDR(); }
#pragma unroll
  for (int i = 0; i < WPW; ++i) {
    const int g = wid * WPW + i, dg = g >> 4, j = g & 15;
    if (W_KMAJOR) {
      const int r = 8 * j + (lane >> 3);
      const int c = (lane & 7) ^ ((r >> 1) & 7);
      const int gn = min(n0 + dg * GM_BN + r, p.N - 1);
      w_src[i] = We + (size_t)gn * p.ldw + c * 8;
    } else {
      const int kr = 4 * j + (lane >> 4);
      const int cn = (lane & 15) ^ ((kr & 3) << 2);
      const int gn = min(n0 + dg * GM_BN + cn * 8, p.N - 8);
      w_src[i] = We + (size_t)kr * p.ldw + gn;
    }
  }
  const size_t w_step = W_KMAJOR ? (size_t)GL_BK : (size_t)GL_BK * p.ldw;
  const int piece_a = wid * 4 * 512, piece_w = wid * WPW * 512;
  int a_off[4], w_off[WPW];
  const uint16_t *abase = p.a_rows != nullptr ? reinterpret_cast<const uint16_t *>(p.A) : Ae;
#define GB_A_OFF()                                                                                              \
  _Pragma("unroll") for (int i = 0; i < 4; ++i) {                                                              \
    const int r = 8 * (wid * 4 + i) + (lane >> 3);                                                             \
    a_off[i] = (int)(unsigned)((const char *)a_src[i] - (const char *)abase);                                  \
    if ((p.a_rows != nullptr && slot4[i] < 0) || m0 + r >= row_limit)                                          \
      a_off[i] = (int)0x7ffff000u + (((lane & 7) ^ ((r >> 1) & 7)) << 4);   \
  }
  if (BUF) {
    if (!sg_on && !fl_on) { GB_A_OFF(); }
#pragma unroll
    for (int i = 0; i < WPW; ++i) w_off[i] = (int)(unsigned)((const char *)w_src[i] - (const char *)We);
  }
  const __amdgpu_buffer_rsrc_t rs_a = __builtin_amdgcn_make_buffer_rsrc(
      const_cast<uint16_t *>(p.a_rows != nullptr ? reinterpret_cast<const uint16_t *>(p.A) : Ae), 0, p.a_span_bytes, 0x00020000);
  const __amdgpu_buffer_rsrc_t rs_w = __builtin_amdgcn_make_buffer_rsrc(const_cast<uint16_t *>(We), 0, -1, 0x00020000);
  const bool w_once = NI == 4 && p.ntm == 1 && gridDim.x >= 256;

  f32x16 acc[NI][2];
#pragma unroll
  for (int i = 0; i < NI; ++i)
#pragma unroll
    for (int j = 0; j < 2; ++j)
#pragma unroll
      for (int r = 0; r < 16; ++r) acc[i][j][r] = 0.f;

  const int l31 = lane & 31, kg = lane >> 5;
  const int sw = (l31 >> 1) & 7;
  int frag_k[4];
#pragma unroll
  for (int kk = 0; kk < 4; ++kk) frag_k[kk] = (((kk * 2 + kg) ^ sw) << 3);
  const int a_row = (wm * 64 + l31) * GL_BK;
  const int wk_row = (wcol + l31) * GL_BK;
  const int g16 = lane >> 4, i16 = lane & 15, q4 = i16 >> 2;
  const int c_lo = wcol / 8 + (g16 & 1) * 2 + ((i16 & 3) >> 1);
  const int wt_row = ((g16 >> 1) * 8 + q4) * GM_BN;
  int wt_c[NI];
#pragma unroll
  for (int ni = 0; ni < NI; ++ni) wt_c[ni] = (((c_lo + 4 * ni) ^ (q4 << 2)) << 3) + (i16 & 1) * 4;

  const int nk = p.K / GL_BK;
  const int npair = NI == 4 ? p.ntn : (p.ntn + 1) >> 1, pair = NI == 4 ? nt : nt >> 1;
  const int rot = p.rot_on ? (int)(((long long)(pair + 3 * e) * nk / npair) % nk) : 0;

#define GB_ISSUE_A(KT, STG)                                                            \
  do {                                                                                 \
    int kr_ = (KT) + rot; kr_ = kr_ >= nk ? kr_ - nk : kr_;                            \
    uint16_t *da_ = sA + (STG) * A_STAGE + piece_a;                                    \
    if (BUF) {                                                                         \
      const int ao_ = kr_ * (GL_BK * 2);                                               \
      _Pragma("unroll") for (int i_ = 0; i_ < 4; ++i_) bdma16<false>(rs_a, a_off[i_], ao_, da_ + i_ * 512); \
    } else {                                                                           \
      const size_t ao_ = (size_t)kr_ * GL_BK;                                          \
      _Pragma("unroll") for (int i_ = 0; i_ < 4; ++i_) glds16(a_src[i_] + ao_, da_ + i_ * 512, false); \
    }                                                                                  \
  } while (0)
#define GB_ISSUE_W(KT, STG)                                                            \
  do {                                                                                 \
    int kr_ = (KT) + rot; kr_ = kr_ >= nk ? kr_ - nk : kr_;                            \
    uint16_t *dw_ = sW + (STG) * NSUB * GL_STAGE + piece_w;                            \
    if (BUF) {                                                                         \
      const int wo_ = (int)(kr_ * (w_step * 2));                                       \
      if (w_once) { _Pragma("unroll") for (int i_ = 0; i_ < WPW; ++i_) bdma16<true>(rs_w, w_off[i_], wo_, dw_ + i_ * 512); } \
      else { _Pragma("unroll") for (int i_ = 0; i_ < WPW; ++i_) bdma16<false>(rs_w, w_off[i_], wo_, dw_ + i_ * 512); } \
    } else {                                                                           \
      const size_t wo_ = (size_t)kr_ * w_step;                                         \
      _Pragma("unroll") for (int i_ = 0; i_ < WPW; ++i_) glds16(w_src[i_] + wo_, dw_ + i_ * 512, w_once); \
    }                                                                                  \
  } while (0)
#define GB_ISSUE(KT, STG) do { GB_ISSUE_A(KT, STG); GB_ISSUE_W(KT, STG); } while (0)
#define GB_LOAD_FRAGS(FA, FW, KK)                                                      \
  do {                                                                                 \
    _Pragma("unroll") for (int mi = 0; mi < 2; ++mi)                                   \
      FA[mi] = *reinterpret_cast<const u32x4 *>(ca + a_row + mi * 32 * GL_BK + frag_k[KK]); \
    _Pragma("unroll") for (int ni = 0; ni < NI; ++ni) {                                \
      if (W_KMAJOR) {                                                                  \
        FW[ni] = *reinterpret_cast<const u32x4 *>(cw + wk_row + ni * 32 * GL_BK + frag_k[KK]); \
      } else {                                                                         \
        const uint16_t *ptr = cw + wt_row + (KK) * 16 * GM_BN + wt_c[ni];              \
        s16x4_t lo = __builtin_amdgcn_ds_read_tr16_b64_v4i16(                          \
            (__attribute__((address_space(3))) s16x4_t *)(ptr));                       \
        s16x4_t hi = __builtin_amdgcn_ds_read_tr16_b64_v4i16(                          \
            (__attribute__((address_space(3))) s16x4_t *)(ptr + 4 * GM_BN));           \
        u32x2 lo2 = __builtin_bit_cast(u32x2, lo), hi2 = __builtin_bit_cast(u32x2, hi); \
        u32x4 f = {lo2[0], lo2[1], hi2[0], hi2[1]};                                    \
        FW[ni] = f;                                                                    \
      }                                                                                \
    }                                                                                  \
  } while (0)
#define GB_MMA(FA, FW)                                                                 \
  do {                                                                                 \
    _Pragma("unroll") for (int ni = 0; ni < NI; ++ni)                                  \
      _Pragma("unroll") for (int mi = 0; mi < 2; ++mi)                                 \
        acc[ni][mi] = Mma<T>::run(FW[ni], FA[mi], acc[ni][mi]);                        \
  } while (0)

#define GB_TILE(BUF)                                                                   \
  do {                                                                                 \
    const uint16_t *ca = sA + (BUF) * A_STAGE, *cw = sW + ((BUF) * NSUB + wsub) * GL_STAGE; \
                                                     \
    u32x4 fa[2][2], fw[2][NI];                                                         \
    GB_LOAD_FRAGS(fa[0], fw[0], 0);                                                    \
    GB_LOAD_FRAGS(fa[1], fw[1], 1);                                                    \
    __builtin_amdgcn_sched_barrier(0);                                                 \
    GB_MMA(fa[0], fw[0]);                                                              \
    GB_MMA(fa[1], fw[1]);                                                              \
    __builtin_amdgcn_sched_barrier(0);                                                 \
    GB_LOAD_FRAGS(fa[0], fw[0], 2);                                                    \
    GB_LOAD_FRAGS(fa[1], fw[1], 3);                                                    \
    __builtin_amdgcn_sched_barrier(0);                                                 \
    GB_MMA(fa[0], fw[0]);                                                              \
    GB_MMA(fa[1], fw[1]);                                                              \
  } while (0)

  if (NS == 2) {
    GB_ISSUE(0, 0);
    __syncthreads();
    for (int kt = 0; kt < nk; ++kt) {
      const int buf = kt & 1;
      if (kt + 1 < nk) GB_ISSUE(kt + 1, buf ^ 1);
      GB_TILE(buf);
      __syncthreads();
    }
  } else {
    constexpr int OPS = 4 + WPW;
    static_assert(NS <= 3, "the prologue order below is worked out for rings of at most three slots");
    constexpr int FL_CH = 4;
    unsigned char *s_fl = smem + (size_t)NS * (A_STAGE + NSUB * GL_STAGE) * 2;
    if (FL && fl_on) {
      static_assert(!FL || WPW * (NS - 1) == 16, "the vmcnt(16) of the fused-location prologue counts the weight ops of the first two tiles");
      const __amdgpu_buffer_rsrc_t rs_i = __builtin_amdgcn_make_buffer_rsrc(const_cast<uint8_t *>(p.fl_idx8), 0, (p.fl_n + 15) & ~15, 0x00020000);
      const int per_ = (((p.fl_n + 255) >> 8) + 15) & ~15, ipw = per_ >> 4;
      for (int i = wid * ipw; i < (wid + 1) * ipw; ++i)
        if (i < 15) bdma16<false>(rs_i, i * 1024 + lane * 16, 0, reinterpret_cast<uint16_t *>(s_fl + i * 1024));
    }
    if (sg_on) {
      asm volatile("" ::"s"(reinterpret_cast<uintptr_t>(We)), "s"(rot), "s"(nk), "s"((int)w_once), "s"((int)(w_step * 2)));
#pragma unroll
      for (int i = 0; i < WPW; ++i) asm volatile("" ::"v"(w_off[i]));
      const __attribute__((address_space(4))) sgv8u *mp =
          reinterpret_cast<const __attribute__((address_space(4))) sgv8u *>(reinterpret_cast<uintptr_t>(p.a_rows) + (size_t)mo_ * 4);
#pragma unroll
      for (int i = 0; i < 4; ++i) sg_q[i] = mp[i];
    }
#pragma unroll
    for (int t = 0; t < NS - 1; ++t)
      if (t < nk) GB_ISSUE_W(t, t);
    if (sg_on) {
      const int rl_ = lane >> 3;
#pragma unroll
      for (int i = 0; i < 4; ++i) {
        int q = sg_q[i][0];
#pragma unroll
        for (int j = 1; j < 8; ++j) q = (rl_ == j) ? sg_q[i][j] : q;
        slot4[i] = q;
      }
      GB_A_ADDR();
      GB_A_OFF();
    }
    if (FL && fl_on) {
      int *s_slot = reinterpret_cast<int *>(s_fl + 15360);
      int *s_wt = s_slot + 128;
      if (tid < 128) s_slot[tid] = -1;
      asm volatile("s_waitcnt vmcnt(16)" ::: "memory");
      const int per = (((p.fl_n + 255) >> 8) + 15) & ~15;
      const int nch = per >> 4;
      const int fl_e0 = tid * per;
      const uint32_t eb = (uint32_t)e * 0x01010101u;
      uint32_t fl_t[FL_CH][4];
      int cnt = 0;
#pragma unroll
      for (int c = 0; c < FL_CH; ++c) {
        if (c < nch) {
          const u32x4 v = *reinterpret_cast<const u32x4 *>(s_fl + min(fl_e0 + c * 16, 15360 - 16));
#pragma unroll
          for (int d = 0; d < 4; ++d) {
            const uint32_t x = v[d] ^ eb;
            fl_t[c][d] = ~(((x & 0x7f7f7f7fu) + 0x7f7f7f7fu) | x | 0x7f7f7f7fu);
          }
        } else {
#pragma unroll
          for (int d = 0; d < 4; ++d) fl_t[c][d] = 0u;
        }
      }
      if (fl_e0 + per > p.fl_n) {
#pragma unroll
        for (int c = 0; c < FL_CH; ++c)
#pragma unroll
          for (int d = 0; d < 4; ++d) {
            const int nv = p.fl_n - (fl_e0 + c * 16 + d * 4);
            fl_t[c][d] = nv >= 4 ? fl_t[c][d] : (nv <= 0 ? 0u : (fl_t[c][d] & ((1u << (8 * nv)) - 1u)));
          }
      }
#pragma unroll
      for (int c = 0; c < FL_CH; ++c)
#pragma unroll
        for (int d = 0; d < 4; ++d) cnt += __popc(fl_t[c][d]);
      int below = 0;
#pragma unroll
      for (int bit = 0; bit < 7; ++bit) {
        const unsigned long long bb = __ballot((cnt >> bit) & 1);
        below += __popcll(bb & ((1ull << lane) - 1ull)) << bit;
      }
      const int wtot = __shfl(below + cnt, 63, 64);
      if (lane == 0) s_wt[wid] = wtot;
      asm volatile("s_waitcnt lgkmcnt(0)" ::: "memory");
      __builtin_amdgcn_s_barrier();
      asm volatile("" ::: "memory");
      int r = below;
      for (int w2 = 0; w2 < wid; ++w2) r += s_wt[w2];
      const bool first_tile = nt == 0;
      if (cnt != 0) {
#pragma unroll
        for (int c = 0; c < FL_CH; ++c)
#pragma unroll
          for (int d = 0; d < 4; ++d) {
            uint32_t t = fl_t[c][d];
            while (t) {
              const int q = fl_e0 + c * 16 + d * 4 + ((__ffs(t) - 1) >> 3);
              if (first_tile) p.fl_loc[q] = r;
              if (r < p.R) s_slot[r] = q;
              ++r;
              t &= t - 1;
            }
          }
      }
      asm volatile("s_waitcnt lgkmcnt(0)" ::: "memory");
      __builtin_amdgcn_s_barrier();
      asm volatile("" ::: "memory");
#pragma unroll
      for (int i = 0; i < 4; ++i) slot4[i] = s_slot[8 * (wid * 4 + i) + (lane >> 3)];
      if (first_tile && tid < p.R) const_cast<int32_t *>(p.a_rows)[(size_t)e * p.R + tid] = s_slot[tid];
      GB_A_ADDR();
      GB_A_OFF();
    }
#pragma unroll
    for (int t = 0; t < NS - 1; ++t)
      if (t < nk) GB_ISSUE_A(t, t);
    int kt = 0, slot = 0;
    GEMM_PROBE(1);
    for (; kt + NS - 1 < nk; ++kt) {
      if (kt == 0) asm volatile("s_waitcnt vmcnt(%0)" ::"n"(4 * (NS - 2)) : "memory");
      else asm volatile("s_waitcnt vmcnt(%0)" ::"n"(OPS * (NS - 2)) : "memory");
      __builtin_amdgcn_s_barrier();
      if (kt == 0) { GEMM_PROBE(2); }
      const int nslot = slot == 0 ? NS - 1 : slot - 1;
      GB_ISSUE(kt + NS - 1, nslot);
      GB_TILE(slot);
      slot = slot + 1 == NS ? 0 : slot + 1;
    }
    GEMM_PROBE(3);
    for (; kt < nk; ++kt) {
      asm volatile("s_waitcnt vmcnt(0)" ::: "memory");
      __builtin_amdgcn_s_barrier();
      GB_TILE(slot);
      slot = slot + 1 == NS ? 0 : slot + 1;
    }
    GEMM_PROBE(4);
  }
#undef GB_TILE
#undef GB_A_ADDR
#undef GB_A_OFF
#undef GB_ISSUE
#undef GB_ISSUE_A
#undef GB_ISSUE_W
#undef GB_LOAD_FRAGS
#undef GB_MMA

  tail();
  GM_PRELOAD_BIAS_N(NI);
  if (BUF && !((p.ldd & 7) || (p.d_stride_e & 7) || (p.d_stride_w & 7) || (reinterpret_cast<uintptr_t>(p.D) & 15))) {
    __syncthreads();
    unsigned char *stage = smem + wid * (64 * (NI * 64 + 16));
    if (ACT == GEMM_ACT_RUNTIME) {
      if (p.act_rt == TUTEL_ACT_NONE) gemm_epilogue_lds<T, TUTEL_ACT_NONE, NI>(p, acc, bias_r, stage, e, m0, n0, wm, wn, lane, row_limit);
      else if (p.act_rt == TUTEL_ACT_RELU) gemm_epilogue_lds<T, TUTEL_ACT_RELU, NI>(p, acc, bias_r, stage, e, m0, n0, wm, wn, lane, row_limit);
      else if (p.act_rt == TUTEL_ACT_GELU) gemm_epilogue_lds<T, TUTEL_ACT_GELU, NI>(p, acc, bias_r, stage, e, m0, n0, wm, wn, lane, row_limit);
      else gemm_epilogue_lds<T, TUTEL_ACT_SILU, NI>(p, acc, bias_r, stage, e, m0, n0, wm, wn, lane, row_limit);
      return;
    }
    gemm_epilogue_lds<T, ACT == GEMM_ACT_RUNTIME ? TUTEL_ACT_NONE : ACT, NI>(p, acc, bias_r, stage, e, m0, n0, wm, wn, lane, row_limit);
    return;
  }
  static_assert(ACT != GEMM_ACT_RUNTIME || BUF, "the run-time activation switch lives in the LDS epilogue");
  gemm_epilogue<T, ACT == GEMM_ACT_RUNTIME ? TUTEL_ACT_NONE : ACT, NI>(p, acc, bias_r, e, m0, n0, wm, wn, l31, kg, row_limit);
}
```

### tutel_amd/experts/ffn.py

```python
import os

import torch
import torch.nn.functional as F

from .. import net, ops

_PREPACK = int(os.environ.get("TUTEL_AMD_PREPACK", "1")) != 0
_TRAIN_FUSED = int(os.environ.get("TUTEL_AMD_TRAIN_FUSED", "1")) != 0


def _FFN_FUSED_ON():
    from .. import _lib
    return ops.get_option(_lib.OPT_FFN_FUSED) > 0


class _FFNTrain(torch.autograd.Function):

    @staticmethod
    def forward(ctx, x, w1, b1, w2, b2):
        hid = ops.expert_gemm(x, w1, b1, True, act="relu")
        y = ops.expert_gemm(hid, w2, b2, False)
        ctx.save_for_backward(x, w1, w2, hid)
        ctx.has_bias = (b1 is not None, b2 is not None)
        return y

    @staticmethod
    def backward(ctx, gy):
        x, w1, w2, hid = ctx.saved_tensors
        gy = gy.contiguous()
        need_x, need_w1, need_b1, need_w2, need_b2 = ctx.needs_input_grad
        gx = gw1 = gb1 = gw2 = gb2 = None
        if need_w2:
            gw2 = torch.matmul(hid.transpose(1, 2), gy)
        if need_b2 and ctx.has_bias[1]:
            gb2 = gy.sum(dim=1)
        if need_x or need_w1 or (need_b1 and ctx.has_bias[0]):
            ghid = ops.expert_gemm(gy, w2, None, True, mul=(hid > 0).to(hid.dtype))
            if need_x:
                gx = ops.expert_gemm(ghid, w1, None, False)
            if need_w1:
                gw1 = torch.matmul(ghid.transpose(1, 2), x)
            if need_b1 and ctx.has_bias[0]:
                gb1 = ghid.sum(dim=1)
        return gx, gw1, gb1, gw2, gb2


class KMajorCache:

    def __init__(self):
        self._store = {}

    def get(self, name, w, transpose=True, dtype=None):
        try:
            version = w._version
        except RuntimeError:
            version = -1
        key = (w.data_ptr(), version, w.dtype, w.device, tuple(w.shape), bool(transpose), dtype)
        hit = self._store.get(name)
        if hit is None or hit[0] != key:
            t = w.detach()
            if dtype is not None and t.dtype != dtype:
                t = t.to(dtype)
            t = t.transpose(1, 2).contiguous() if transpose else t.contiguous()
            hit = (key, t)
            self._store[name] = hit
        return hit[1]

    def invalidate(self):
        self._store.clear()


def _probe_points():
    lin = torch.linspace(-16.0, 16.0, 2049)
    mag = torch.logspace(-30, 38, 545)
    big = torch.tensor([60000.0, 65504.0, 1e5, 3.3e38])
    return torch.cat([lin, mag, -mag, big, -big, torch.zeros(1)])


_PROBE = _probe_points()
_REFS = (("relu", F.relu), ("gelu", F.gelu), ("silu", F.silu), ("none", lambda t: t))
_KNOWN_FNS = {F.relu: "relu", torch.relu: "relu", F.gelu: "gelu", F.silu: "silu"}


def classify_activation(fn, dtype=None):
    if isinstance(fn, str):
        return fn if fn in ops.ACT_CODES else None
    tag = getattr(fn, "_tutel_amd_act", None)
    if tag in ops.ACT_CODES:
        return tag
    try:
        if fn in _KNOWN_FNS:
            return _KNOWN_FNS[fn]
    except TypeError:
        pass
    if isinstance(fn, torch.nn.Module):
        if type(fn) is torch.nn.ReLU:
            return "relu"
        if type(fn) is torch.nn.SiLU:
            return "silu"
        if type(fn) is torch.nn.GELU and getattr(fn, "approximate", "none") == "none":
            return "gelu"
        if type(fn) is torch.nn.Identity:
            return "none"
    try:
        with torch.no_grad():
            found = None
            for dt in ([torch.float32] + ([dtype] if dtype not in (None, torch.float32) else [])):
                lim = torch.finfo(dt).max
                probe = _PROBE.clamp(-lim, lim).to(dt)
                a, b = fn(probe.clone()), fn(probe.clone())
                if not (torch.is_tensor(a) and a.shape == probe.shape and a.dtype == dt and torch.equal(a, b)):
                    return None
                name = None
                for cand, ref in _REFS:
                    r = ref(probe)
                    if torch.allclose(a.float(), r.float(), rtol=0, atol=1e-7 if dt == torch.float32 else 0.0, equal_nan=True):
                        name = cand
                        break
                if name is None or (found is not None and name != found):
# ... 71 lines not shown
        key = (self.training, self.batched_fc1_w.dtype)
        if key not in self._act_cache:
            self._act_cache[key] = classify_activation(self.activation_fn, key[1])
        return self._act_cache[key]

    def _no_autograd(self, x):
        return not (torch.is_grad_enabled() and (x.requires_grad or any(p.requires_grad for p in self.parameters())))

    def compute_dtype(self, x):
        w = self.batched_fc1_w
        if x.dtype not in (torch.bfloat16, torch.float16):
            return None
        if w.dtype == x.dtype:
            return x.dtype
        if torch.is_autocast_enabled() and w.dtype == torch.float32 and x.dtype == torch.get_autocast_dtype(x.device.type):
            return x.dtype
        return None

    def can_fuse(self, x, ctx):
        if self.skip_expert or not x.is_cuda or not self._no_autograd(x):
            return False
        if getattr(ctx, "adaptive_degree", 1) == 0 or getattr(ctx, "sharded_count", 1) > 1:
            return False
        w1, w2 = self.batched_fc1_w, self.batched_fc2_w
        dt = self.compute_dtype(x)
        return (dt is not None and ops.gemm_supported(dt, w1.size(1), w1.size(2)) and
                ops.gemm_supported(dt, w2.size(2), w2.size(1)) and self.fused_activation() is not None)

    def can_fuse_training(self, x, ctx):
        if (not _TRAIN_FUSED or self.skip_expert or not x.is_cuda or x.dim() != 3 or self._no_autograd(x)
                or getattr(ctx, "adaptive_degree", 1) == 0 or getattr(ctx, "sharded_count", 1) > 1):
            return False
        w1, w2 = self.batched_fc1_w, self.batched_fc2_w
        dt = self.compute_dtype(x)
        b2 = self.batched_fc2_bias
        return (dt is not None and self.fused_activation() == "relu" and x.size(0) == w1.size(0) and (b2 is None or b2.size(-1) == self.output_dim)
                and ops.gemm_supported(dt, w1.size(1), w1.size(2)) and ops.gemm_supported(dt, w2.size(2), w2.size(1))
                and ops.gemm_supported(dt, w2.size(1), w2.size(2)) and ops.gemm_supported(dt, w1.size(2), w1.size(1)))

    def fused_params(self, dtype):
        w1, b1, w2, b2 = self.batched_fc1_w, self.batched_fc1_bias, self.batched_fc2_w, self.batched_fc2_bias
        cast = None if w1.dtype == dtype else dtype
        kmajor = self.w2_kmajor_now()
        if cast is not None:
            w1 = self._kmajor.get("fc1.cast", w1, transpose=False, dtype=cast)
            b1 = self._kmajor.get("b1.cast", b1, transpose=False, dtype=cast) if b1 is not None else None
        if kmajor or cast is not None:
            w2 = self._kmajor.get("fc2", w2, transpose=kmajor, dtype=cast)
        if b2 is not None:
            if b2.size(-1) != self.output_dim or cast is not None:
                b2 = self._kmajor.get("b2.cast", b2[:, :self.output_dim], transpose=False, dtype=cast)
        return w1, b1, w2, b2, kmajor

    def forward_fused(self, x, ctx, a_layout=None, R=None, out=None, d_layout=None, slot_map=None, expert_range=None):
        counts, align = None, 1
        if getattr(ctx, "megablocks_size", 0) > 0:
            counts, align = ctx.dispatch_count, int(ctx.megablocks_size)
        w1, b1, w2, b2, w2_kmajor = self.fused_params(self.compute_dtype(x))
        if expert_range is not None:
            lo, hi = expert_range
            w1, w2 = w1[lo:hi], w2[lo:hi]
            b1 = b1[lo:hi] if b1 is not None else None
            b2 = b2[lo:hi] if b2 is not None else None
            assert counts is None, "megablocks row counts are not sliced"
        if _FFN_FUSED_ON() and w2_kmajor and counts is None and out is None and a_layout is None and d_layout is None and (slot_map is not None or x.dim() == 3):
            y = ops.expert_ffn(x, w1, b1, w2, b2, self.fused_activation(), R=R, smap=slot_map)
            if y is not None:
                return y
        if slot_map is not None:
            h = ops.expert_gemm_gather(x, slot_map, w1, b1, True, self.fused_activation(), R,
                                       row_counts=counts, row_align=align)
        else:
            h = ops.expert_gemm(x, w1, b1, True, act=self.fused_activation(), E_loc=w1.size(0), R=R,
                                a_layout=a_layout, row_counts=counts, row_align=align)
        return ops.expert_gemm(h, w2, b2, w2_kmajor, out=out, d_layout=d_layout, row_counts=counts, row_align=align)

    def w2_kmajor_now(self):
        return _PREPACK and not self.training

    def invalidate_prepacked(self):
        self._kmajor.invalidate()

    def train(self, mode=True):
        self._kmajor.invalidate()
        return super().train(mode)

    def _apply(self, fn, *args, **kwargs):
        self._kmajor.invalidate()
        return super()._apply(fn, *args, **kwargs)

    def _load_from_state_dict(self, *args, **kwargs):
        self._kmajor.invalidate()
        return super()._load_from_state_dict(*args, **kwargs)

    def forward(self, x, ctx):
        if self.skip_expert:
            return x
        if self.can_fuse(x, ctx):
            return self.forward_fused(x.contiguous(), ctx)

        if self.can_fuse_training(x, ctx):
            dt = self.compute_dtype(x)
            b1, b2 = self.batched_fc1_bias, self.batched_fc2_bias
            return _FFNTrain.apply(x.contiguous(), self.batched_fc1_w.to(dt), b1.to(dt) if b1 is not None else None,
                                   self.batched_fc2_w.to(dt), b2.to(dt) if b2 is not None else None)

        w1, w2 = self.batched_fc1_w, self.batched_fc2_w
        b1 = self.batched_fc1_bias.unsqueeze(1) if self.batched_fc1_bias is not None else None
        b2 = self.batched_fc2_bias.unsqueeze(1) if self.batched_fc2_bias is not None else None

        if ctx.adaptive_degree == 0:
            E = ctx.num_global_experts
            w1 = net.zero_gather(w1, group=ctx.group).view(E, -1, w1.size(2))
            w2 = net.zero_gather(w2, group=ctx.group).view(E, -1, w2.size(2))
            if b1 is not None:
                b1 = net.zero_gather(b1, group=ctx.group).view(E, 1, -1)
            if b2 is not None:
                b2 = net.zero_gather(b2, group=ctx.group).view(E, 1, -1)
        elif ctx.sharded_count > 1:
            mesh = net.get_world_size(ctx.group)
            if 1 < mesh < net.get_world_size():
                ctx.adaptive_degree = ctx.sharded_count
            group_size = ctx.sharded_count // ctx.adaptive_degree
            if group_size > 1:
                zg = net.create_groups_from_world(group_count=-group_size, parent_group=ctx.group).model_group
                w1 = net.zero_gather(w1, group=zg).view(1, -1, ctx.model_dim)
                w2 = net.zero_gather(w2, group=zg).view(1, -1, self.output_dim)
                if b1 is not None:
# ... 32 lines not shown
```

### tutel_amd/impls/ep_native.py

```python
import ctypes
import logging
import os

import torch
import torch.distributed as dist

from .. import _lib, ops

ENABLED = int(os.environ.get("TUTEL_AMD_NATIVE_EP", "1")) != 0
FAST_PATH = int(os.environ.get("TUTEL_AMD_FAST_PATH", "1")) != 0
_FUSED_LOCATION = int(os.environ.get("TUTEL_AMD_FUSED_LOCATION", "1")) != 0
HOSTED = int(os.environ.get("TUTEL_AMD_NATIVE_HOSTED", "0")) != 0
TRANSPORT = os.environ.get("TUTEL_AMD_EP_TRANSPORT", "auto").lower()
IPC_VERIFIED = os.environ.get("TUTEL_AMD_EP_IPC_VERIFIED", "0") == "1"
IPC_TIMEOUT_MS = int(os.environ.get("TUTEL_AMD_EP_TIMEOUT_MS", "120000"))
_FORCE_COMM = False
_comms = {}
_groups = {}
_zero_rows = {}


class Segment:

    def __init__(self, handle, nbytes):
# ... 437 lines not shown
        a.is_postscore, a.fuse_encode = int(bool(layer.is_postscore)), int(fuse)
        self.bufs = {}

        def buf(name, rows, cols, alias=None):
            t = self.bufs[alias] if alias is not None else torch.empty([rows, cols], dtype=dt, device=dev)
            self.bufs[name] = t
            setattr(a, name, t.data_ptr())
        buf("hid", E_loc * W * C_cap, H)
        self.segment = None
        if comm is not None and comm.ipc:
            es = x.element_size()
            recv_bytes = (E * C_cap * M * es + 255) // 256 * 256
            sg = comm.segment(("ep", M, Mo, str(dt), E, C_cap), recv_bytes + E * C_cap * Mo * es)
            a.recv, a.back, a.peer_seg = sg.ptr, sg.ptr + recv_bytes, sg.handle
            self.segment = sg
            self.args, self.comm = a, comm
            return
        buf("send", E * C_cap, Mo)
        if not fuse:
            buf("enc", E * C_cap, M)
            buf("recv", E * C_cap, M, alias="enc" if comm is None else None)
            buf("back", E * C_cap, Mo, alias="send" if comm is None else None)
        else:
            z = _zero_rows.get((dev, dt))
            if z is None or z.numel() < M:
                z = _zero_rows[(dev, dt)] = torch.zeros([max(M, 8192)], dtype=dt, device=dev)
            self.bufs["zero_row"] = z
            a.zero_row = z.data_ptr()
        self.args, self.comm = a, comm
        if comm is not None and hasattr(comm, "register"):
            for t in self.bufs.values():
                comm.register(t)


def _workspace(layer, static_key, T, C, make, exact_capacity=False):
    import collections
    cache = layer.__dict__.get("_ep_workspaces")
    if not isinstance(cache, collections.OrderedDict):
        cache = layer.__dict__["_ep_workspaces"] = collections.OrderedDict()
    C_cap = _bucket_capacity(C)
    for key, ws in cache.items():
        if key[0] == static_key and ws.T_cap >= T and (ws.C_cap == C_cap if exact_capacity else ws.C_cap >= C):
            cache.move_to_end(key)
            return ws
    T_cap = _bucket_tokens(T)
    ws = make(T_cap, C_cap)
    cache[(static_key, T_cap, C_cap)] = ws
    layer.__dict__["_ep_workspace_allocations"] = layer.__dict__.get("_ep_workspace_allocations", 0) + 1
    while len(cache) > WS_MAX:
        cache.popitem(last=False)
    return ws


def forward(layer, x, crit, degree):
    ex = layer.experts
    W = layer.world_size
    with_comm = W > 1 or (_FORCE_COMM and dist.is_initialized())
    comm = communicator(layer.group, x.device) if with_comm else None
    if with_comm and comm is None:
        return None
    if getattr(layer, "megablocks_size", 0) > 0 and with_comm:
        return None
    if not with_comm:
        degree = 1
    k = crit.idx2d.shape[0]
    key = ("ep", x.shape[1], x.dtype, x.device, crit[0], k, degree, bool(layer.is_postscore), ex.fused_activation(), ops._stream(), with_comm,
           bool(comm is not None and comm.ipc))
    ws = _workspace(layer, key, x.shape[0], crit[4], lambda Tc, Cc: _Workspace(layer, x, crit[0], Cc, k, degree, comm, Tc),
                    exact_capacity=bool(comm is not None and comm.ipc))
    a = ws.args
    a.T, a.capacity = x.shape[0], crit[4]
    w1, b1, w2, b2, kmajor = ex.fused_params(x.dtype)
    gates = crit.gates2d
    y = torch.empty([x.shape[0], ex.output_dim], dtype=x.dtype, device=x.device)
    a.w2_kmajor = int(kmajor)
    a.x, a.slot_map, a.idx, a.loc, a.gates = x.data_ptr(), crit.slot_map.data_ptr(), crit.idx2d.data_ptr(), crit.loc2d.data_ptr(), gates.data_ptr()
    a.gate_dtype = ops._DT[gates.dtype]
    a.w1, a.w2 = w1.data_ptr(), w2.data_ptr()
    a.b1 = b1.data_ptr() if b1 is not None else None
    a.b2 = b2.data_ptr() if b2 is not None else None
    a.y = y.data_ptr()
    mega = int(getattr(layer, "megablocks_size", 0))
    if mega > 0 and not with_comm:
        a.row_counts, a.row_align = layer.dispatch_count.data_ptr(), mega
    else:
        a.row_counts, a.row_align = None, 1
    _lib.check(_lib.lib().tutel_amd_ep_forward(comm.handle if comm is not None else None, ctypes.byref(a), ops._stream()),
               "tutel_amd_ep_forward")
    layer.protected_shape = torch.Size([layer.num_local_experts, W * crit[4], ex.output_dim])
    return y


class _MoeWorkspace(_Workspace):

    def __init__(self, layer, x, logits, k, capacity, degree, comm, T_cap):
        E, T = logits.shape[1], int(T_cap)
        dev = x.device
        super().__init__(layer, x, E, capacity, k, degree, comm, T_cap)
        self.idx = torch.empty([k, T], dtype=torch.int32, device=dev)
        self.loc = torch.empty([k, T], dtype=torch.int32, device=dev)
        self.gates = torch.empty([k, T], dtype=logits.dtype, device=dev)
        self.slot_map = torch.empty([E * capacity], dtype=torch.int32, device=dev)
        self.ws = torch.empty([max(int(_lib.lib().tutel_amd_routing_workspace_bytes(64 * 128, E, k)), 4)], dtype=torch.uint8, device=dev)
        self.stats = torch.empty([1], dtype=torch.int32, device=dev)
        self.cap_host = torch.zeros([1], dtype=torch.int32).pin_memory()
        self.cap_c = ctypes.c_int.from_address(self.cap_host.data_ptr())
        m = _lib.MoeArgs()
        m.ep = self.args
        m.ep.slot_map, m.ep.idx, m.ep.loc, m.ep.gates = (self.slot_map.data_ptr(), self.idx.data_ptr(), self.loc.data_ptr(),
                                                          self.gates.data_ptr())
        m.logits_dtype = ops._DT[logits.dtype]
        m.ws, m.ws_bytes, m.stats = self.ws.data_ptr(), self.ws.numel(), self.stats.data_ptr()
        m.capacity_out = ctypes.pointer(self.cap_c)
        self.margs = m
        self.gate_partials, self.gate_partials_keep = None, []
        self.fl_ws = None
        if comm is None and _FUSED_LOCATION:
            self.fl_ws = torch.empty([(k * T + 15) // 16 * 16 + 16], dtype=torch.uint8, device=dev)
            m.fl_ws, m.fl_ws_bytes = self.fl_ws.data_ptr(), self.fl_ws.numel()


def forward_from_logits(layer, x, logits, k, capacity, degree, normalize_gate, want_loss, dropless=None, megablocks_size=0, gate_w=None):
    ex = layer.experts
    W = layer.world_size
    with_comm = W > 1 or (_FORCE_COMM and dist.is_initialized())
    if dropless is not None and with_comm:
        return None
    comm = communicator(layer.group, x.device) if with_comm else None
    if with_comm and comm is None:
        return None
    if not with_comm:
        degree = 1
    sizes = layer.__dict__.setdefault("_ep_dropless_cap", {})
    skey = (tuple(x.shape), logits.shape[1], k)
    if dropless is not None:
        capacity = max(capacity, sizes.get(skey, 0))
    for attempt in range(4):
        key = ("moe", x.shape[1], x.dtype, x.device, logits.shape[1], logits.dtype, k, degree, bool(layer.is_postscore),
               ex.fused_activation(), ops._stream(), with_comm, bool(comm is not None and comm.ipc))
        ws = _workspace(layer, key, x.shape[0], capacity, lambda Tc, Cc: _MoeWorkspace(layer, x, logits, k, Cc, degree, comm, Tc),
                        exact_capacity=bool(comm is not None and comm.ipc))
        m = ws.margs
        a = m.ep
        a.T = x.shape[0]
        w1, b1, w2, b2, kmajor = ex.fused_params(x.dtype)
        dev = x.device
        y = torch.empty([x.shape[0], ex.output_dim], dtype=x.dtype, device=dev)
        cnt = torch.empty([logits.shape[1]], dtype=torch.int32, device=dev)
        l_aux = torch.empty([1], dtype=logits.dtype, device=dev) if want_loss else None
        a.w2_kmajor = int(kmajor)
        a.x, a.w1, a.w2 = x.data_ptr(), w1.data_ptr(), w2.data_ptr()
        a.b1 = b1.data_ptr() if b1 is not None else None
        a.b2 = b2.data_ptr() if b2 is not None else None
        a.y = y.data_ptr()
        if megablocks_size > 0 and not with_comm:
            a.row_counts, a.row_align = cnt.data_ptr(), int(megablocks_size)
        else:
            a.row_counts, a.row_align = None, 1
        m.normalize_gate = int(bool(normalize_gate))
        if gate_w is None:
            m.logits, m.gate_w, m.logits_out = logits.data_ptr(), None, None
        else:
            need = ops.gate_proj_splits(x.shape[0], x.shape[1], logits.shape[1], x.dtype) * x.shape[0] * logits.shape[1]
            if ws.gate_partials is None or ws.gate_partials.numel() < need:
                ws.gate_partials_keep.append(ws.gate_partials)
                ws.gate_partials = torch.empty([need], dtype=torch.float32, device=dev)
            m.logits, m.gate_w = None, gate_w.data_ptr()
            m.gate_partials, m.gate_partial_bytes = ws.gate_partials.data_ptr(), ws.gate_partials.numel() * 4
            layer.last_logits = torch.empty(list(logits.shape), dtype=x.dtype, device=dev) if getattr(layer, "_keep_routing", False) else None
            m.logits_out = layer.last_logits.data_ptr() if layer.last_logits is not None else None
        m.dispatch_count = cnt.data_ptr()
        m.l_aux = l_aux.data_ptr() if l_aux is not None else None
        cap_out = ws.cap_c
        if dropless is not None:
            a.capacity = 0
            m.capacity_limit, m.alignment, m.max_capacity = int(dropless[0]), int(dropless[1]), int(ws.C_cap)
        else:
            a.capacity = int(capacity)
            m.capacity_limit, m.alignment, m.max_capacity = 0, 1, int(capacity)
        rc = _lib.lib().tutel_amd_moe_forward(comm.handle if comm is not None else None, ctypes.byref(m), ops._stream())
        if rc == _lib.EAGAIN and dropless is not None:
            capacity = (int(cap_out.value) * 5 // 4 + 31) // 32 * 32
            sizes[skey] = capacity
            continue
        _lib.check(rc, "tutel_amd_moe_forward")
        used = int(cap_out.value) if dropless is not None else int(capacity)
        if getattr(layer, "_keep_routing", False):
            n = k * x.shape[0]
            layer.last_routing = (ws.idx.view(-1)[:n].view(k, -1).clone(), ws.loc.view(-1)[:n].view(k, -1).clone())
        layer.protected_shape = torch.Size([layer.num_local_experts, W * used, ex.output_dim])
        return y, (l_aux[0] if l_aux is not None else None), cnt, used
    raise _lib.TutelAmdError("tutel_amd_moe_forward: the dropless capacity kept growing")


def packed_plan(T, E, k, M, H, M_out, dtype, capacity_limit, alignment):
    p = _lib.PackedPlan()
    rc = _lib.lib().tutel_amd_packed_plan(int(T), int(E), int(k), int(M), int(H), int(M_out), ops._DT[dtype] if isinstance(dtype, torch.dtype)
                                          else int(dtype), int(capacity_limit), int(alignment), ctypes.byref(p))
    if rc == _lib.ENOTSUP:
        return None, _lib.lib().tutel_amd_last_error().decode("utf-8", "replace")
    _lib.check(rc, "tutel_amd_packed_plan")
    return {n: int(getattr(p, n)) for n, _ in _lib.PackedPlan._fields_}, None


def _swiglu(ex):
    from ..experts.llama_ffn import LlamaFFNNetwork
# ... 150 lines not shown
```

### tutel_amd/ops.py

```python
import torch

from . import _lib

_DT = {torch.float32: _lib.F32, torch.float16: _lib.F16, torch.bfloat16: _lib.BF16}
ACT_CODES = {"none": _lib.ACT_NONE, "relu": _lib.ACT_RELU, "gelu": _lib.ACT_GELU, "silu": _lib.ACT_SILU}


def _code(t):
    try:
        return _DT[t.dtype]
    except KeyError:
        raise _lib.TutelAmdError(f"tutel_amd: dtype {t.dtype} is not supported by the HIP kernels") from None


def _dev(*tensors):
    for t in tensors:
        if t is not None and not t.is_cuda:
            raise _lib.TutelAmdError(
                "tutel_amd: the MoE hot path runs on the HIP device only (got a CPU tensor); "
                "there is no CPU fallback.")


def _ptr(t):
    return None if t is None else t.data_ptr()
# ... 155 lines not shown


def fast_encode(x, smap, gates, n_slots, capacity=0, num_experts=0, chunk_rows=0, expert_slice=0, ep_world=1):
    _dev(x, smap, gates)
    assert x.dim() == 2 and x.is_contiguous() and smap.dtype == torch.int32 and smap.numel() == n_slots
    x = _a16(x)
    T, M = x.shape
    out = torch.empty([n_slots, M], dtype=x.dtype, device=x.device)
    if gates is not None:
        assert gates.is_contiguous()
    _lib.check(_lib.lib().tutel_amd_fast_encode(_ptr(x), _code(x), _ptr(smap), _ptr(gates),
                                                _code(gates) if gates is not None else 0, T, M,
                                                int(n_slots), int(capacity), int(num_experts), int(chunk_rows),
                                                int(expert_slice), int(ep_world), _ptr(out), _stream()),
               "tutel_amd_fast_encode")
    return out


def fast_decode(buf, idx, loc, gates, capacity, num_experts=0, chunk_rows=0, expert_slice=0, ep_world=1):
    _dev(buf, idx, loc, gates)
    assert buf.dim() == 2 and buf.is_contiguous()
    buf = _a16(buf)
    assert idx.dtype == torch.int32 and loc.dtype == torch.int32 and idx.is_contiguous() and loc.is_contiguous()
    k, T = idx.shape
    M = buf.shape[1]
    out = torch.empty([T, M], dtype=buf.dtype, device=buf.device)
    if gates is not None:
        assert gates.is_contiguous() and gates.shape == idx.shape
    _lib.check(_lib.lib().tutel_amd_fast_decode(_ptr(buf), _code(buf), _ptr(idx), _ptr(loc), _ptr(gates),
                                                _code(gates) if gates is not None else 0, T, M, k,
                                                int(capacity), int(num_experts), int(chunk_rows), int(expert_slice), int(ep_world),
                                                _ptr(out), _stream()),
               "tutel_amd_fast_decode")
    return out


def gate_grad(x, buf, idx, loc, capacity):
    _dev(x, buf, idx, loc)
    assert x.is_contiguous() and buf.is_contiguous() and x.dtype == buf.dtype
    x, buf = _a16(x), _a16(buf)
    k, T = idx.shape
    M = x.shape[1]
    out = torch.empty([k, T], dtype=torch.float32, device=x.device)
    _lib.check(_lib.lib().tutel_amd_gate_grad(_ptr(x), _ptr(buf), _code(x), _ptr(idx), _ptr(loc), T, M, k,
                                              int(capacity), _ptr(out), _stream()), "tutel_amd_gate_grad")
    return out


def gemm_supported(dtype, N, K):
    return dtype in (torch.bfloat16, torch.float16) and K % 64 == 0 and N % 8 == 0


def expert_gemm(a, w, bias, w_kmajor, act="none", E_loc=None, R=None, a_layout=None, out=None,
                d_layout=None, row_counts=None, row_align=1, mul=None):
    _dev(a, w, bias, out, row_counts, mul)
    assert w.dim() == 3 and w.is_contiguous()
    if w_kmajor:
        El, N, K = w.shape
    else:
        El, K, N = w.shape
    E_loc = El if E_loc is None else E_loc
    if a_layout is None:
        assert a.dim() == 3 and a.is_contiguous() and a.shape[0] == E_loc and a.shape[2] == K
        a = _a16(a)
        R = a.shape[1]
        a_layout = (R * K, 0, R, K)
    assert R is not None
    default_out = out is None
    if default_out:
        out = torch.empty([E_loc, R, N], dtype=a.dtype, device=a.device)
        d_layout = (R * N, 0, R, N)
    assert d_layout is not None
    if bias is not None:
        assert bias.is_contiguous() and bias.shape[-1] == N and bias.dtype == a.dtype
    assert w.dtype == a.dtype
    if mul is not None:
        assert mul.dtype == a.dtype
        if default_out:
            assert mul.is_contiguous() and mul.numel() == E_loc * R * N
        else:
            assert mul.shape == out.shape and mul.stride() == out.stride(), "mul must have the layout of out"
        _lib.check(_lib.lib().tutel_amd_expert_gemm_glu(
            _ptr(a), a_layout[0], a_layout[1], a_layout[2], a_layout[3],
            _ptr(w), int(bool(w_kmajor)), w.stride(0), w.stride(1),
            _ptr(bias), (bias.stride(0) if bias is not None else 0), _ptr(mul),
            _ptr(out), d_layout[0], d_layout[1], d_layout[2], d_layout[3],
            E_loc, R, N, K, _code(a), ACT_CODES[act],
            _ptr(row_counts), int(row_align), _stream()), "tutel_amd_expert_gemm_glu")
        return out
    _lib.check(_lib.lib().tutel_amd_expert_gemm(
        _ptr(a), a_layout[0], a_layout[1], a_layout[2], a_layout[3],
        _ptr(w), int(bool(w_kmajor)), w.stride(0), w.stride(1),
        _ptr(bias), (bias.stride(0) if bias is not None else 0),
        _ptr(out), d_layout[0], d_layout[1], d_layout[2], d_layout[3],
        E_loc, R, N, K, _code(a), ACT_CODES[act],
        _ptr(row_counts), int(row_align), _stream()), "tutel_amd_expert_gemm")
    return out


def expert_gemm_gate_up(a, w_gate, w_up, act="silu", row_counts=None, row_align=1):
    _dev(a, w_gate, w_up, row_counts)
    assert a.dim() == 3 and a.is_contiguous() and w_gate.dim() == 3 and w_gate.is_contiguous()
    assert w_up.shape == w_gate.shape and w_up.is_contiguous() and w_gate.dtype == a.dtype and w_up.dtype == a.dtype
    E, N, K = w_gate.shape
    assert a.shape[0] == E and a.shape[2] == K
    a = _a16(a)
    R = a.shape[1]
    out = torch.empty([E, R, N], dtype=a.dtype, device=a.device)
    _lib.check(_lib.lib().tutel_amd_expert_gemm_gate_up(
        _ptr(a), R * K, 0, R, K, _ptr(w_gate), _ptr(w_up), w_gate.stride(0), w_gate.stride(1),
        _ptr(out), R * N, 0, R, N, E, R, N, K, _code(a), ACT_CODES[act],
        _ptr(row_counts), int(row_align), _stream()), "tutel_amd_expert_gemm_gate_up")
    return out


_zero_rows = {}


def expert_gemm_gather(x, smap, w, bias, w_kmajor, act, R, row_counts=None, row_align=1):
    _dev(x, smap, w, bias, row_counts)
    assert x.dim() == 2 and x.is_contiguous() and w.dim() == 3 and w.is_contiguous() and w.dtype == x.dtype
    E_loc, N, K = (w.shape if w_kmajor else (w.shape[0], w.shape[2], w.shape[1]))
    assert x.shape[1] == K and smap.dtype == torch.int32 and smap.numel() == E_loc * R
    x = _a16(x)
    key = (x.device, x.dtype)
    z = _zero_rows.get(key)
    if z is None or z.numel() < K:
        z = _zero_rows[key] = torch.zeros([max(K, 8192)], dtype=x.dtype, device=x.device)
    out = torch.empty([E_loc, R, N], dtype=x.dtype, device=x.device)
    _lib.check(_lib.lib().tutel_amd_expert_gemm_gather(
        _ptr(x), x.stride(0), _ptr(smap), x.shape[0], _ptr(z), _ptr(w), int(bool(w_kmajor)), w.stride(0), w.stride(1),
        _ptr(bias), (bias.stride(0) if bias is not None else 0), _ptr(out), R * N, N, E_loc, R, N, K, _code(x),
        ACT_CODES[act], _ptr(row_counts), int(row_align), _stream()), "tutel_amd_expert_gemm_gather")
    return out


def expert_ffn(x, w1, b1, w2_kmajor, b2, act, R=None, smap=None, hid=None):
    _dev(x, w1, b1, w2_kmajor, b2, smap)
    assert w1.dim() == 3 and w2_kmajor.dim() == 3 and w1.is_contiguous() and w2_kmajor.is_contiguous() and w1.dtype == x.dtype == w2_kmajor.dtype
    E_loc, H, M = w1.shape
    M_out = w2_kmajor.shape[1]
    assert w2_kmajor.shape == (E_loc, M_out, H) and x.is_contiguous()
    x = _a16(x)
    if smap is None:
        assert x.dim() == 3 and x.shape[0] == E_loc and x.shape[2] == M
        R = x.shape[1]
        xs, ldx, T, z = R * M, M, 0, None
    else:
        assert x.dim() == 2 and x.shape[1] == M and smap.dtype == torch.int32 and smap.numel() == E_loc * R
        key = (x.device, x.dtype)
        z = _zero_rows.get(key)
        if z is None or z.numel() < M:
            z = _zero_rows[key] = torch.zeros([max(M, 8192)], dtype=x.dtype, device=x.device)
        xs, ldx, T = 0, x.stride(0), x.shape[0]
    if hid is None:
        hid = torch.empty([E_loc, R, H], dtype=x.dtype, device=x.device)
    out = torch.empty([E_loc, R, M_out], dtype=x.dtype, device=x.device)
    rc = _lib.lib().tutel_amd_expert_ffn(_ptr(x), xs, ldx, _ptr(smap), T, _ptr(z), _ptr(w1), w1.stride(0), w1.stride(1), _ptr(b1),
                                         (b1.stride(0) if b1 is not None else 0), _ptr(hid), R * H, H, _ptr(w2_kmajor), w2_kmajor.stride(0),
                                         w2_kmajor.stride(1), _ptr(b2), (b2.stride(0) if b2 is not None else 0), _ptr(out), R * M_out, M_out,
                                         E_loc, R, M, H, M_out, _code(x), ACT_CODES[act], _stream())
    if rc == _lib.ENOTSUP:
        return None
    _lib.check(rc, "tutel_amd_expert_ffn")
    return out


_OPT_ENV = {_lib.OPT_GEMM_IMPL: "TUTEL_AMD_GEMM_IMPL", _lib.OPT_GEMM_TILE: "TUTEL_AMD_GEMM_BIG", _lib.OPT_DECODE: "TUTEL_AMD_DECODE",
            _lib.OPT_EP_STAGE_GRID: "TUTEL_AMD_EP_STAGE_GRID", _lib.OPT_GEMM_PERSIST: "TUTEL_AMD_GEMM_PERSIST", _lib.OPT_EP_STREAMS: "TUTEL_AMD_EP_STREAMS",
            _lib.OPT_EP_CANARY: "TUTEL_AMD_EP_CANARY", _lib.OPT_GEMM_SPLITK: "TUTEL_AMD_GEMM_SPLITK", _lib.OPT_GEMM_STORE: "TUTEL_AMD_GEMM_STORE",
            _lib.OPT_GEMM_GATHER: "TUTEL_AMD_GEMM_GATHER", _lib.OPT_FUSED_LOCATION: "TUTEL_AMD_FUSED_LOCATION", _lib.OPT_TIE_RULE: "TUTEL_AMD_TIE_RULE", _lib.OPT_FFN_FUSED: "TUTEL_AMD_FFN_FUSED"}
_opts = {}


class PackedLayout:

    def __init__(self, E, rows_bound, tiles_bound, row_limit, device):
        self.E, self.rows_bound, self.tiles_bound, self.row_limit = int(E), int(rows_bound), int(tiles_bound), int(row_limit)
        self.offsets = torch.empty([E + 1], dtype=torch.int32, device=device)
        self.tiles = torch.empty([2 * max(tiles_bound, 1)], dtype=torch.int32, device=device)
        self.ntiles = torch.empty([1], dtype=torch.int32, device=device)
        self.capacity = torch.empty([1], dtype=torch.int32, device=device)
        self.slot_map = torch.empty([max(rows_bound, 1)], dtype=torch.int32, device=device)

    @property
    def decode_limit(self):
        return self.row_limit if self.row_limit > 0 else 0x7fffffff


def packed_layout(dispatch_count, idx, loc, capacity_limit, alignment, rows_bound, tiles_bound, row_limit, out=None):
    _dev(dispatch_count, idx, loc)
    k, T = idx.shape
    E = dispatch_count.numel()
    lay = out if out is not None else PackedLayout(E, rows_bound, tiles_bound, row_limit, idx.device)
    _lib.check(_lib.lib().tutel_amd_packed_layout(_ptr(dispatch_count), _ptr(idx), _ptr(loc), T, E, k, int(capacity_limit), int(alignment),
                                                  lay.rows_bound, lay.tiles_bound, _ptr(lay.offsets), _ptr(lay.tiles), _ptr(lay.ntiles),
                                                  _ptr(lay.capacity), _ptr(lay.slot_map), _stream()), "tutel_amd_packed_layout")
    return lay


def expert_gemm_packed(a, w, bias, w_kmajor, layout, act="none", gather=None, zero_row=None, mul=None, out=None):
    _dev(a, w, bias, mul)
    assert a.dim() == 2 and a.is_contiguous() and w.dim() == 3 and w.is_contiguous() and w.dtype == a.dtype
    E, N, K = (w.shape[0], w.shape[1], w.shape[2]) if w_kmajor else (w.shape[0], w.shape[2], w.shape[1])
    assert a.shape[1] == K and E == layout.E
    if bias is not None:
        assert bias.is_contiguous() and bias.shape[-1] == N and bias.dtype == a.dtype
    if mul is not None:
        assert mul.shape == (layout.rows_bound, N) and mul.is_contiguous() and mul.dtype == a.dtype
    a = _a16(a)
    if out is None:
        out = torch.empty([layout.rows_bound, N], dtype=a.dtype, device=a.device)
    else:
        _dev(out)
        assert out.shape == (layout.rows_bound, N) and out.is_contiguous() and out.dtype == a.dtype
    _lib.check(_lib.lib().tutel_amd_expert_gemm_packed(
        _ptr(a), K, _ptr(layout.slot_map) if gather else None, a.shape[0] if gather else 0, _ptr(zero_row) if gather else None,
        _ptr(w), int(bool(w_kmajor)), w.stride(0), w.stride(1), _ptr(bias), (bias.stride(0) if bias is not None else 0), _ptr(mul),
        _ptr(out), N, E, layout.rows_bound, N, K, _code(a), ACT_CODES[act], _ptr(layout.offsets), _ptr(layout.tiles), _ptr(layout.ntiles),
        _ptr(layout.capacity), layout.tiles_bound, _stream()), "tutel_amd_expert_gemm_packed")
# ... 112 lines not shown
```

Baseline: 16.85 million.

## Add prepacked bf16 expert weight image and packed-weight GEMM path

After: 17.02 million (median of 6 runs). 1.0% higher.

```diff
diff --git a/include/tutel_amd.h b/include/tutel_amd.h
--- a/include/tutel_amd.h
+++ b/include/tutel_amd.h
@@ -92,6 +92,17 @@
                                   const void *W_gate, const void *W_up, int64_t w_stride_e, int ldw, void *D, int64_t d_stride_e,
                                   int64_t d_stride_w, int d_rows_per_w, int ldd, int E_loc, int R, int N, int K, int dtype, int act,
                                   const int32_t *row_counts, int row_align, tutel_stream_t stream);
+
+size_t tutel_amd_wpack_bytes(int E, int N, int K);
+int tutel_amd_wpack_pack(const void *w_kmajor, int E, int N, int K, int ldw, void *out, tutel_stream_t stream);
+int tutel_amd_wpack_unpack(const void *pack, const void *raw, int E, int N, int K, void *out, tutel_stream_t stream);
+int tutel_amd_expert_gemm_wpack(const void *A, int64_t a_stride_e, int64_t a_stride_w, int a_rows_per_w, int lda, const void *W,
+                                int w_kmajor, int64_t w_stride_e, int ldw, const void *wpack, const void *bias, int64_t bias_stride_e,
+                                void *D, int64_t d_stride_e, int64_t d_stride_w, int d_rows_per_w, int ldd, int E_loc, int R, int N, int K,
+                                int dtype, int act, const int32_t *row_counts, int row_align, const int32_t *slot_map, int T,
+                                const void *zero_row, tutel_stream_t stream);
+int tutel_amd_wpack_mode(int value);
+long long tutel_amd_wpack_launches(void);
 
 typedef struct tutel_amd_ep_comm tutel_amd_ep_comm_t;
 #define TUTEL_AMD_EP_ID_BYTES 128
@@ -163,6 +174,7 @@
   int row_align;
   void *y;
   const struct tutel_amd_ep_segment *peer_seg;
+  const void *w1_pack, *w2_pack;
 } tutel_amd_ep_args_t;
 int tutel_amd_ep_forward(tutel_amd_ep_comm_t *comm, const tutel_amd_ep_args_t *args, tutel_stream_t stream);
 
diff --git a/tutel_amd/_lib.py b/tutel_amd/_lib.py
--- a/tutel_amd/_lib.py
+++ b/tutel_amd/_lib.py
@@ -39,6 +39,13 @@
     "tutel_amd_expert_gemm_gate_up": (_i, [_vp, _i64, _i64, _i, _i, _vp, _vp, _i64, _i, _vp, _i64, _i64, _i, _i,
                                            _i, _i, _i, _i, _i, _i, _vp, _i, _vp]),
     "tutel_amd_set_option": (_i, [_i, _i]),
+    "tutel_amd_wpack_bytes": (_sz, [_i, _i, _i]),
+    "tutel_amd_wpack_pack": (_i, [_vp, _i, _i, _i, _i, _vp, _vp]),
+    "tutel_amd_wpack_unpack": (_i, [_vp, _vp, _i, _i, _i, _vp, _vp]),
+    "tutel_amd_expert_gemm_wpack": (_i, [_vp, _i64, _i64, _i, _i, _vp, _i, _i64, _i, _vp, _vp, _i64, _vp, _i64, _i64, _i, _i,
+                                         _i, _i, _i, _i, _i, _i, _vp, _i, _vp, _i, _vp, _vp]),
+    "tutel_amd_wpack_mode": (_i, [_i]),
+    "tutel_amd_wpack_launches": (ctypes.c_longlong, []),
     "tutel_amd_probe_tr16": (_i, [_vp, _vp]),
 }
 
@@ -53,7 +60,7 @@
                                    "dtype", "gate_dtype", "act", "is_postscore", "w2_kmajor", "fuse_encode")] +
                 [(n, _vp) for n in ("x", "slot_map", "idx", "loc", "gates", "w1", "b1", "w2", "b2",
                                     "enc", "recv", "hid", "send", "back", "zero_row", "row_counts")] +
-                [("row_align", _i), ("y", _vp), ("peer_seg", _vp)])
+                [("row_align", _i), ("y", _vp), ("peer_seg", _vp), ("w1_pack", _vp), ("w2_pack", _vp)])
 
 
 class MoeArgs(ctypes.Structure):
diff --git a/tutel_amd/csrc/common.h b/tutel_amd/csrc/common.h
--- a/tutel_amd/csrc/common.h
+++ b/tutel_amd/csrc/common.h
@@ -10,6 +10,7 @@
 
 void tutel_set_error(const char *fmt, ...);
 int tutel_get_option(int key);
+int tutel_wpack_mode();
 
 int tutel_stage_begin(int stage, hipStream_t st);
 void tutel_stage_end(int token, hipStream_t st);
@@ -52,7 +53,8 @@
 
 int tutel_expert_gemm_gather_fl(const void *X, int ldx, int32_t *slot_map, int T, const void *zero_row, const void *W, int64_t w_stride_e,
                                 int ldw, const void *bias, int64_t bias_stride_e, void *D, int64_t d_stride_e, int ldd, int E_loc, int R,
-                                int N, int K, int dtype, int act, const uint8_t *idx8, int n, int32_t *loc, hipStream_t st);
+                                int N, int K, int dtype, int act, const uint8_t *idx8, int n, int32_t *loc, hipStream_t st,
+                                const void *wpack = nullptr);
 int tutel_expert_ffn(const void *X, int64_t x_stride_e, int ldx, const int32_t *slot_map, int T, const void *zero_row, const void *W1,
                      int64_t w1_stride_e, int ldw1, const void *b1, int64_t b1_stride_e, void *hid, int64_t hid_stride_e, int ldh,
                      const void *W2, int64_t w2_stride_e, int ldw2, const void *b2, int64_t b2_stride_e, void *D, int64_t d_stride_e, int ldd,
diff --git a/tutel_amd/csrc/ep.hip b/tutel_amd/csrc/ep.hip
--- a/tutel_amd/csrc/ep.hip
+++ b/tutel_amd/csrc/ep.hip
@@ -722,12 +722,13 @@
     }
     if (rc == TUTEL_AMD_ENOTSUP) {
       Range r("tutel_amd.expert_fc1");
-      rc = tutel_amd_expert_gemm_gather(a->x, M, a->slot_map, T, a->zero_row, a->w1, 1, (int64_t)H * M, M, a->b1, H, a->hid,
-                                        (int64_t)C * H, H, E_loc, C, H, M, a->dtype, a->act, rcnt, ralign, cur);
+      rc = tutel_amd_expert_gemm_wpack(a->x, 0, 0, 1, M, a->w1, 1, (int64_t)H * M, M, a->w1_pack, a->b1, H, a->hid, (int64_t)C * H, 0, C, H, E_loc,
+                                       C, H, M, a->dtype, a->act, rcnt, ralign, a->slot_map, T, a->zero_row, cur);
       if (rc) return rc;
       Range r2("tutel_amd.expert_fc2");
-      rc = tutel_amd_expert_gemm(a->hid, (int64_t)C * H, 0, C, H, a->w2, a->w2_kmajor, (int64_t)H * Mo, a->w2_kmajor ? H : Mo, a->b2,
-                                 Mo, a->send, (int64_t)C * Mo, 0, C, Mo, E_loc, C, Mo, H, a->dtype, TUTEL_ACT_NONE, rcnt, ralign, cur);
+      rc = tutel_amd_expert_gemm_wpack(a->hid, (int64_t)C * H, 0, C, H, a->w2, a->w2_kmajor, (int64_t)H * Mo, a->w2_kmajor ? H : Mo,
+                                       a->w2_kmajor ? a->w2_pack : nullptr, a->b2, Mo, a->send, (int64_t)C * Mo, 0, C, Mo, E_loc, C, Mo, H,
+                                       a->dtype, TUTEL_ACT_NONE, rcnt, ralign, nullptr, 0, nullptr, cur);
       if (rc) return rc;
     }
     Range r("tutel_amd.fast_decode");
@@ -969,12 +970,12 @@
     if (rc == TUTEL_AMD_ENOTSUP) {
       Range r("tutel_amd.expert_fc1");
       rc = tutel_expert_gemm_gather_fl(a.x, a.M, smap, T, a.zero_row, a.w1, (int64_t)Ho * a.M, a.M, a.b1, Ho, a.hid, (int64_t)a.capacity * Ho, Ho,
-                                       E, a.capacity, Ho, a.M, a.dtype, a.act, idx8, k * T, const_cast<int32_t *>(a.loc), st);
+                                       E, a.capacity, Ho, a.M, a.dtype, a.act, idx8, k * T, const_cast<int32_t *>(a.loc), st, a.w1_pack);
       if (rc) return rc;
       Range r2("tutel_amd.expert_fc2");
-      rc = tutel_amd_expert_gemm(a.hid, (int64_t)a.capacity * Ho, 0, a.capacity, Ho, a.w2, a.w2_kmajor, (int64_t)Ho * Mo, a.w2_kmajor ? Ho : Mo,
-                                 a.b2, Mo, a.send, (int64_t)a.capacity * Mo, 0, a.capacity, Mo, E, a.capacity, Mo, Ho, a.dtype, TUTEL_ACT_NONE,
-                                 nullptr, 1, stream);
+      rc = tutel_amd_expert_gemm_wpack(a.hid, (int64_t)a.capacity * Ho, 0, a.capacity, Ho, a.w2, a.w2_kmajor, (int64_t)Ho * Mo,
+                                       a.w2_kmajor ? Ho : Mo, a.w2_kmajor ? a.w2_pack : nullptr, a.b2, Mo, a.send, (int64_t)a.capacity * Mo, 0,
+                                       a.capacity, Mo, E, a.capacity, Mo, Ho, a.dtype, TUTEL_ACT_NONE, nullptr, 1, nullptr, 0, nullptr, stream);
       if (rc) return rc;
     }
     Range r("tutel_amd.fast_decode");
diff --git a/tutel_amd/csrc/expert_gemm.hip b/tutel_amd/csrc/expert_gemm.hip
--- a/tutel_amd/csrc/expert_gemm.hip
+++ b/tutel_amd/csrc/expert_gemm.hip
@@ -1,10 +1,14 @@
 #include <stdlib.h>
 
+#include <atomic>
 #include <mutex>
+#include <type_traits>
 
 #include "common.h"
 
 #include "gemm_dev.h"
+
+static std::atomic<long long> g_wpack_launches{0};
 
 template <typename T, bool W_KMAJOR, int ACT, bool NT, bool ROT, bool PACKED = false>
 __global__ __launch_bounds__(GM_THREADS, 2) void expert_gemm_kernel(GemmArgs p) {
@@ -331,7 +335,7 @@
   gemm_epilogue<T, ACT>(p, acc, bias_r, e, m0, n0, wm, wn, l31, kg, row_limit);
 }
 
-template <typename T, bool W_KMAJOR, int ACT, int NI, int NS, bool BUF = false, int BM = GB_BM, bool FL = false>
+template <typename T, bool W_KMAJOR, int ACT, int NI, int NS, bool BUF = false, int BM = GB_BM, bool FL = false, bool WP = false>
 __global__ __launch_bounds__(BM * 2, 2) void expert_gemm_big_kernel(GemmArgs p) {
   extern __shared__ __attribute__((aligned(16))) unsigned char smem[];
   const int nb = gridDim.x;
@@ -340,7 +344,7 @@
     const int b = blockIdx.x, q = nb >> 3, r = nb & 7, xcd = b & 7, pos = b >> 3;
     w = (xcd < r ? xcd * (q + 1) : r * (q + 1) + (xcd - r) * q) + pos;
   }
-  gemm_big_tile<T, W_KMAJOR, ACT, NI, NS, BUF, BM, FL>(p, w / (p.ntm * p.ntn), w % p.ntm, (w / p.ntm) % p.ntn, smem);
+  gemm_big_tile<T, W_KMAJOR, ACT, NI, NS, BUF, BM, FL, GemmNoHook, WP>(p, w / (p.ntm * p.ntn), w % p.ntm, (w / p.ntm) % p.ntn, smem);
 }
 
 #define PP_BUF (4 * GL_STAGE)
@@ -761,15 +765,16 @@
   return 0;
 }
 
-template <typename T, bool KM, int ACT, int NI, int NS = 2, bool BUF = false, int BM = GB_BM, bool FL = false>
+template <typename T, bool KM, int ACT, int NI, int NS = 2, bool BUF = false, int BM = GB_BM, bool FL = false, bool WP = false>
 static int launch_big(const GemmArgs &a, hipStream_t st) {
   GemmArgs b = a;
   b.ntm = (a.R + BM - 1) / BM;
   b.ntn = (a.N + NI * 64 - 1) / (NI * 64);
   const size_t lds_k = (size_t)NS * (BM / 128 + NI / 2) * GL_STAGE * 2 + (FL ? 16384 : 0), lds_e = BUF ? (size_t)(BM / 32) * 64 * (NI * 64 + 16) : 0;
   const size_t lds = lds_k > lds_e ? lds_k : lds_e;
-  auto kern = expert_gemm_big_kernel<T, KM, ACT, NI, NS, BUF, BM, FL>;
+  auto kern = expert_gemm_big_kernel<T, KM, ACT, NI, NS, BUF, BM, FL, WP>;
   if (!tutel_lds_optin((const void *)kern, lds)) return -1;
+  if (WP) ++g_wpack_launches;
   hipLaunchKernelGGL(kern, dim3(a.E_loc * b.ntm * b.ntn), dim3(BM * 2), lds, st, b);
   TUTEL_CHECK_LAUNCH("tutel_amd_expert_gemm");
   return 0;
@@ -819,12 +824,16 @@
   const int impl = tutel_get_option(TUTEL_OPT_GEMM_IMPL), big = tutel_get_option(TUTEL_OPT_GEMM_TILE);
   const bool ring256_ok = KM && a.fits32 && a.N >= 256 && a.R <= GM_BM;
   const bool ring256 = ring256_ok && (impl == 4 || (impl < 0 && (long long)a.E_loc * ((a.N + 255) / 256) >= 256));
+  constexpr bool WPK = KM && std::is_same<T, bf16_t>::value;
+  const bool wp = WPK && a.wpack != nullptr && tutel_wpack_mode() != 0 && a.N % WPACK_BN == 0 && a.mul == nullptr && a.d_peer == nullptr &&
+                  (long long)(a.N / WPACK_BN) * (a.K / WPACK_BK) * WPACK_TILE < 0x7fffffffLL;
   if (a.fl_idx8 != nullptr) {
     if (!(ring256 && KM && big <= 0 && a.a_rows != nullptr && a.row_counts == nullptr && a.fl_n >= 1 && a.fl_n <= 15360 && a.E_loc <= 128 && a.K >= 2 * GL_BK)) {
       tutel_set_error("tutel_expert_gemm_gather_fl: this launch does not take the fused-location ring kernel");
       return TUTEL_AMD_ENOTSUP;
     }
     if (a.fl_loc == nullptr) return 0;
+    if (wp) return launch_big<T, true, ACT, 4, 3, true, 128, KM, WPK>(a, st);
     return launch_big<T, true, ACT, 4, 3, true, 128, KM>(a, st);
   }
   if (a.N >= GM_BN && big != 0) {
@@ -843,6 +852,7 @@
     if (KM && (big == 3 || (big < 0 && a.R > GM_BM && t128 >= 192)))
       return a.fits32 && tutel_get_option(TUTEL_OPT_GEMM_IMPL) != 2 ? launch_big<T, true, ACT, 2, 3, true>(a, st) : launch_big<T, true, ACT, 2, 3>(a, st);
   }
+  if (ring256 && wp) return launch_big<T, true, ACT, 4, 3, true, 128, false, WPK>(a, st);
   if (ring256) return launch_big<T, true, ACT, 4, 3, true, 128>(a, st);
   const bool use_dma = impl < 0 ? KM : (impl == 1 || impl == 4);
   if (use_dma) return launch_glds<T, KM, ACT>(a, grid, st);
@@ -921,6 +931,7 @@
   a.ntn = (N + GM_BN - 1) / GM_BN;
   a.pk_off = a.pk_tiles = a.pk_ntiles = a.pk_cap = nullptr;
   a.w_up = nullptr;
+  a.wpack = nullptr;
   return 0;
 }
 
@@ -934,12 +945,14 @@
                                      const int32_t *a_rows, int a_rows_mod, const void *a_zero,
                                      const void *mul, tutel_stream_t stream, const uint64_t *d_peer = nullptr,
                                      int64_t d_peer_off = 0, const PeerCanary *d_can = nullptr, const uint8_t *fl_idx8 = nullptr,
-                                     int fl_n = 0, int32_t *fl_loc = nullptr) {
+                                     int fl_n = 0, int32_t *fl_loc = nullptr, const void *wpack = nullptr) {
   GemmArgs a;
   const int brc = tutel_gemm_args(A, a_stride_e, a_stride_w, a_rows_per_w, lda, W, w_kmajor, w_stride_e, ldw, bias, bias_stride_e, D, d_stride_e,
                                   d_stride_w, d_rows_per_w, ldd, E_loc, R, N, K, dtype, act, row_counts, row_align, a_rows, a_rows_mod, a_zero, mul,
                                   d_peer, d_peer_off, d_can, fl_idx8, fl_n, fl_loc, &a);
   if (brc != 0) return brc < 0 ? brc : 0;
+  TUTEL_REQUIRE(((uintptr_t)wpack & 15) == 0, "tutel_amd_expert_gemm_wpack: the packed image must be 16-byte aligned");
+  a.wpack = w_kmajor ? wpack : nullptr;
   long long grid_ll = (long long)E_loc * a.ntm * a.ntn;
   TUTEL_REQUIRE(grid_ll < 0x7fffffffLL, "tutel_amd_expert_gemm: grid too large");
   const int grid = (int)grid_ll;
@@ -979,12 +992,30 @@
 
 int tutel_expert_gemm_gather_fl(const void *X, int ldx, int32_t *slot_map, int T, const void *zero_row, const void *W, int64_t w_stride_e,
                                 int ldw, const void *bias, int64_t bias_stride_e, void *D, int64_t d_stride_e, int ldd, int E_loc, int R,
-                                int N, int K, int dtype, int act, const uint8_t *idx8, int n, int32_t *loc, hipStream_t st) {
+                                int N, int K, int dtype, int act, const uint8_t *idx8, int n, int32_t *loc, hipStream_t st, const void *wpack) {
   TUTEL_REQUIRE(slot_map != nullptr && idx8 != nullptr && T >= 1 && ((uintptr_t)idx8 & 15) == 0, "tutel_expert_gemm_gather_fl: bad arguments");
   if (tutel_get_option(TUTEL_OPT_FUSED_LOCATION) == 0) return TUTEL_AMD_ENOTSUP;
   return expert_gemm_impl(X, 0, 0, R > 0 ? R : 1, ldx, W, 1, w_stride_e, ldw, bias, bias_stride_e, D, d_stride_e, 0, R > 0 ? R : 1, ldd, E_loc,
-                          R, N, K, dtype, act, nullptr, 1, slot_map, T, zero_row, nullptr, (tutel_stream_t)st, nullptr, 0, nullptr, idx8, n, loc);
-}
+                          R, N, K, dtype, act, nullptr, 1, slot_map, T, zero_row, nullptr, (tutel_stream_t)st, nullptr, 0, nullptr, idx8, n, loc, wpack);
+}
+
+extern "C" int tutel_amd_expert_gemm_wpack(const void *A, int64_t a_stride_e, int64_t a_stride_w, int a_rows_per_w, int lda, const void *W,
+                                           int w_kmajor, int64_t w_stride_e, int ldw, const void *wpack, const void *bias,
+                                           int64_t bias_stride_e, void *D, int64_t d_stride_e, int64_t d_stride_w, int d_rows_per_w, int ldd,
+                                           int E_loc, int R, int N, int K, int dtype, int act, const int32_t *row_counts, int row_align,
+                                           const int32_t *slot_map, int T, const void *zero_row, tutel_stream_t stream) {
+  if (slot_map != nullptr) {
+    TUTEL_REQUIRE(T >= 1, "tutel_amd_expert_gemm_wpack: the gather form needs T >= 1");
+    return expert_gemm_impl(A, 0, 0, R > 0 ? R : 1, lda, W, w_kmajor, w_stride_e, ldw, bias, bias_stride_e, D, d_stride_e, 0, R > 0 ? R : 1, ldd,
+                            E_loc, R, N, K, dtype, act, row_counts, row_align, slot_map, T, zero_row, nullptr, stream, nullptr, 0, nullptr,
+                            nullptr, 0, nullptr, wpack);
+  }
+  return expert_gemm_impl(A, a_stride_e, a_stride_w, a_rows_per_w, lda, W, w_kmajor, w_stride_e, ldw, bias, bias_stride_e, D, d_stride_e,
+                          d_stride_w, d_rows_per_w, ldd, E_loc, R, N, K, dtype, act, row_counts, row_align, nullptr, 0, nullptr, nullptr, stream,
+                          nullptr, 0, nullptr, nullptr, 0, nullptr, wpack);
+}
+
+extern "C" long long tutel_amd_wpack_launches(void) { return g_wpack_launches; }
 
 extern "C" int tutel_amd_expert_gemm_glu(const void *A, int64_t a_stride_e, int64_t a_stride_w,
                                          int a_rows_per_w, int lda, const void *W, int w_kmajor,
diff --git a/tutel_amd/csrc/gemm_dev.h b/tutel_amd/csrc/gemm_dev.h
--- a/tutel_amd/csrc/gemm_dev.h
+++ b/tutel_amd/csrc/gemm_dev.h
@@ -1,5 +1,6 @@
 #pragma once
 #include "common.h"
+#include "wpack_dev.h"
 
 #ifndef GEMM_PROBE
 #define GEMM_PROBE(i)
@@ -84,6 +85,7 @@
   int act_rt;
   const int32_t *pk_off, *pk_tiles, *pk_ntiles, *pk_cap;
   const void *w_up;
+  const void *wpack;
 };
 
 __device__ __forceinline__ uint16_t *gemm_out_row(const GemmArgs &p, int e, int m) {
@@ -182,6 +184,10 @@
 template <bool NT>
 __device__ __forceinline__ void bdma16(__amdgpu_buffer_rsrc_t rs, int voff, int soff, uint16_t *l) {
   __builtin_amdgcn_raw_ptr_buffer_load_lds(rs, (__attribute__((address_space(3))) void *)l, 16, voff, soff, 0, NT ? 2 : 0);
+}
+
+__device__ __forceinline__ void bdma4(__amdgpu_buffer_rsrc_t rs, int voff, int soff, unsigned char *l) {
+  __builtin_amdgcn_raw_ptr_buffer_load_lds(rs, (__attribute__((address_space(3))) void *)l, 4, voff, soff, 0, 0);
 }
 
 #define EP_PITCH 272
@@ -310,15 +316,18 @@
 #define GB_THREADS 512
 
 struct GemmNoHook { __device__ __forceinline__ void operator()() const {} };
-template <typename T, bool W_KMAJOR, int ACT, int NI, int NS, bool BUF = false, int BM = GB_BM, bool FL = false, typename Tail = GemmNoHook>
+template <typename T, bool W_KMAJOR, int ACT, int NI, int NS, bool BUF = false, int BM = GB_BM, bool FL = false, typename Tail = GemmNoHook,
+          bool WP = false>
 __device__ __forceinline__ void gemm_big_tile(const GemmArgs &p, const int e, const int mt, const int nt, unsigned char *smem,
                                               Tail tail = Tail()) {
   static_assert(!FL || (BUF && NS == 3 && BM == 128 && W_KMAJOR), "FL: the 128 x 256 ring kernel only");
+  static_assert(!WP || (BUF && NS == 3 && BM == 128 && W_KMAJOR && NI == 4), "WP: the 128 x 256 ring kernel only");
   constexpr int NW = BM / 32;
   constexpr int NSUB = NI / 2;
-  constexpr int WPW = 16 * NSUB / NW;
+  constexpr int WPW = WP ? 7 : 16 * NSUB / NW;
   constexpr int BN = NI * 64;
   constexpr int A_STAGE = (BM / 128) * GL_STAGE;
+  constexpr int W_STAGE = WP ? (WPACK_EMAX_OFF + NW * WPACK_BN) / 2 : NSUB * GL_STAGE;
   uint16_t *sA = reinterpret_cast<uint16_t *>(smem);
   uint16_t *sW = sA + NS * A_STAGE;
 
@@ -371,7 +380,9 @@
 #pragma unroll
   for (int i = 0; i < WPW; ++i) {
     const int g = wid * WPW + i, dg = g >> 4, j = g & 15;
-    if (W_KMAJOR) {
+    if (WP) {
+      w_src[i] = nullptr;
+    } else if (W_KMAJOR) {
       const int r = 8 * j + (lane >> 3);
       const int c = (lane & 7) ^ ((r >> 1) & 7);
       const int gn = min(n0 + dg * GM_BN + r, p.N - 1);
@@ -397,11 +408,17 @@
   if (BUF) {
     if (!sg_on && !fl_on) { GB_A_OFF(); }
 #pragma unroll
-    for (int i = 0; i < WPW; ++i) w_off[i] = (int)(unsigned)((const char *)w_src[i] - (const char *)We);
+    for (int i = 0; i < WPW; ++i) w_off[i] = WP ? 0 : (int)(unsigned)((const char *)w_src[i] - (const char *)We);
+    if (WP) {
+#pragma unroll
+      for (int i = 0; i < WPW; ++i) w_off[i] = i < WPW - 1 ? (wid * (WPW - 1) + i) * 1024 + lane * 16 : WPACK_EMAX_OFF + lane * 4;
+    }
   }
   const __amdgpu_buffer_rsrc_t rs_a = __builtin_amdgcn_make_buffer_rsrc(
       const_cast<uint16_t *>(p.a_rows != nullptr ? reinterpret_cast<const uint16_t *>(p.A) : Ae), 0, p.a_span_bytes, 0x00020000);
-  const __amdgpu_buffer_rsrc_t rs_w = __builtin_amdgcn_make_buffer_rsrc(const_cast<uint16_t *>(We), 0, -1, 0x00020000);
+  const __amdgpu_buffer_rsrc_t rs_w = __builtin_amdgcn_make_buffer_rsrc(
+      WP ? const_cast<unsigned char *>(reinterpret_cast<const unsigned char *>(p.wpack) + (size_t)e * p.ntn * (p.K / GL_BK) * WPACK_TILE)
+         : reinterpret_cast<unsigned char *>(const_cast<uint16_t *>(We)), 0, -1, 0x00020000);
   const bool w_once = NI == 4 && p.ntm == 1 && gridDim.x >= 256;
 
   f32x16 acc[NI][2];
@@ -425,6 +442,15 @@
   int wt_c[NI];
 #pragma unroll
   for (int ni = 0; ni < NI; ++ni) wt_c[ni] = (((c_lo + 4 * ni) ^ (q4 << 2)) << 3) + (i16 & 1) * 4;
+
+  int wp_sm[4], wp_cd[4];
+  uint32_t wp_esc = 0u;
+#pragma unroll
+  for (int kk = 0; kk < 4; ++kk) {
+    wp_sm[kk] = wpack_sm_off(wn * 128 + l31, kk * 2 + kg);
+    wp_cd[kk] = wpack_code_off(wn * 128 + l31, kk * 2 + kg);
+  }
+  const int wp_em = WPACK_EMAX_OFF + wid * WPACK_BN + wn * 128 + l31;
 
   const int nk = p.K / GL_BK;
   const int npair = NI == 4 ? p.ntn : (p.ntn + 1) >> 1, pair = NI == 4 ? nt : nt >> 1;
@@ -445,8 +471,14 @@
 #define GB_ISSUE_W(KT, STG)                                                            \
   do {                                                                                 \
     int kr_ = (KT) + rot; kr_ = kr_ >= nk ? kr_ - nk : kr_;                            \
-    uint16_t *dw_ = sW + (STG) * NSUB * GL_STAGE + piece_w;                            \
-    if (BUF) {                                                                         \
+    uint16_t *dw_ = sW + (STG) * W_STAGE + piece_w;                                    \
+    if (WP) {                                                                          \
+      unsigned char *dp_ = reinterpret_cast<unsigned char *>(sW + (STG) * W_STAGE);    \
+      const int wo_ = (nt * nk + kr_) * WPACK_TILE;                                    \
+      if (w_once) { _Pragma("unroll") for (int i_ = 0; i_ < WPW - 1; ++i_) bdma16<true>(rs_w, w_off[i_], wo_, reinterpret_cast<uint16_t *>(dp_ + (wid * (WPW - 1) + i_) * 1024)); } \
+      else { _Pragma("unroll") for (int i_ = 0; i_ < WPW - 1; ++i_) bdma16<false>(rs_w, w_off[i_], wo_, reinterpret_cast<uint16_t *>(dp_ + (wid * (WPW - 1) + i_) * 1024)); } \
+      bdma4(rs_w, w_off[WPW - 1], wo_, dp_ + WPACK_EMAX_OFF + wid * WPACK_BN);         \
+    } else if (BUF) {                                                                  \
       const int wo_ = (int)(kr_ * (w_step * 2));                                       \
       if (w_once) { _Pragma("unroll") for (int i_ = 0; i_ < WPW; ++i_) bdma16<true>(rs_w, w_off[i_], wo_, dw_ + i_ * 512); } \
       else { _Pragma("unroll") for (int i_ = 0; i_ < WPW; ++i_) bdma16<false>(rs_w, w_off[i_], wo_, dw_ + i_ * 512); } \
@@ -461,7 +493,16 @@
     _Pragma("unroll") for (int mi = 0; mi < 2; ++mi)                                   \
       FA[mi] = *reinterpret_cast<const u32x4 *>(ca + a_row + mi * 32 * GL_BK + frag_k[KK]); \
     _Pragma("unroll") for (int ni = 0; ni < NI; ++ni) {                                \
-      if (W_KMAJOR) {                                                                  \
+      if (WP) {                                                                        \
+        const unsigned char *cb_ = reinterpret_cast<const unsigned char *>(cw);        \
+        const u32x2 s_ = *reinterpret_cast<const u32x2 *>(cb_ + wp_sm[KK] + ni * 32 * 64); \
+        const uint32_t c_ = *reinterpret_cast<const uint32_t *>(cb_ + wp_cd[KK] + ni * 32 * 32); \
+        uint32_t f_[4];                                                                \
+        wpack_frag8(s_[0], s_[1], c_, wp_eb[ni], f_);                                  \
+        wp_esc |= (c_ - 0x11111111u) & ~c_;                                            \
+        const u32x4 v_ = {f_[0], f_[1], f_[2], f_[3]};                                 \
+        FW[ni] = v_;                                                                   \
+      } else if (W_KMAJOR) {                                                           \
         FW[ni] = *reinterpret_cast<const u32x4 *>(cw + wk_row + ni * 32 * GL_BK + frag_k[KK]); \
       } else {                                                                         \
         const uint16_t *ptr = cw + wt_row + (KK) * 16 * GM_BN + wt_c[ni];              \
@@ -482,19 +523,45 @@
         acc[ni][mi] = Mma<T>::run(FW[ni], FA[mi], acc[ni][mi]);                        \
   } while (0)
 
+#define GB_WP_FIX(FW0, FW1, KK0)                                                       \
+  do {                                                                                 \
+    if (WP) {                                                                          \
+      if (__builtin_amdgcn_ballot_w64((wp_esc & 0x88888888u) != 0u) != 0ull) {         \
+        const unsigned char *cb_ = reinterpret_cast<const unsigned char *>(cw);        \
+        _Pragma("unroll") for (int h_ = 0; h_ < 2; ++h_)                               \
+          _Pragma("unroll") for (int ni = 0; ni < NI; ++ni) {                          \
+            const uint32_t c_ = *reinterpret_cast<const uint32_t *>(cb_ + wp_cd[(KK0) + h_] + ni * 32 * 32); \
+            if (wpack_has_escape(c_)) {                                                \
+              const u32x4 v_ = *reinterpret_cast<const u32x4 *>(We + (size_t)(n0 + wn * 128 + ni * 32 + l31) * p.ldw + \
+                                                                (size_t)krc_ * GL_BK + (((KK0) + h_) * 2 + kg) * 8); \
+              if (h_ == 0) FW0[ni] = v_; else FW1[ni] = v_;                            \
+            }                                                                          \
+          }                                                                            \
+      }                                                                                \
+      wp_esc = 0u;                                                                     \
+    }                                                                                  \
+  } while (0)
 #define GB_TILE(BUF)                                                                   \
   do {                                                                                 \
-    const uint16_t *ca = sA + (BUF) * A_STAGE, *cw = sW + ((BUF) * NSUB + wsub) * GL_STAGE; \
+    const uint16_t *ca = sA + (BUF) * A_STAGE, *cw = WP ? sW + (BUF) * W_STAGE : sW + ((BUF) * NSUB + wsub) * GL_STAGE; \
+    int krc_ = kt + rot; krc_ = krc_ >= nk ? krc_ - nk : krc_;                         \
+    uint32_t wp_eb[NI];                                                                \
+    if (WP) {                                                                          \
+      _Pragma("unroll") for (int ni = 0; ni < NI; ++ni)                                \
+        wp_eb[ni] = wpack_ebase(reinterpret_cast<const unsigned char *>(cw)[wp_em + ni * 32]); \
+    }                                                                                  \
                                                      \
     u32x4 fa[2][2], fw[2][NI];                                                         \
     GB_LOAD_FRAGS(fa[0], fw[0], 0);                                                    \
     GB_LOAD_FRAGS(fa[1], fw[1], 1);                                                    \
+    GB_WP_FIX(fw[0], fw[1], 0);                                                        \
     __builtin_amdgcn_sched_barrier(0);                                                 \
     GB_MMA(fa[0], fw[0]);                                                              \
     GB_MMA(fa[1], fw[1]);                                                              \
     __builtin_amdgcn_sched_barrier(0);                                                 \
     GB_LOAD_FRAGS(fa[0], fw[0], 2);                                                    \
     GB_LOAD_FRAGS(fa[1], fw[1], 3);                                                    \
+    GB_WP_FIX(fw[0], fw[1], 2);                                                        \
     __builtin_amdgcn_sched_barrier(0);                                                 \
     GB_MMA(fa[0], fw[0]);                                                              \
     GB_MMA(fa[1], fw[1]);                                                              \
@@ -513,9 +580,9 @@
     constexpr int OPS = 4 + WPW;
     static_assert(NS <= 3, "the prologue order below is worked out for rings of at most three slots");
     constexpr int FL_CH = 4;
-    unsigned char *s_fl = smem + (size_t)NS * (A_STAGE + NSUB * GL_STAGE) * 2;
+    unsigned char *s_fl = smem + (size_t)NS * (A_STAGE + W_STAGE) * 2;
     if (FL && fl_on) {
-      static_assert(!FL || WPW * (NS - 1) == 16, "the vmcnt(16) of the fused-location prologue counts the weight ops of the first two tiles");
+      static_assert(!FL || WPW * (NS - 1) == (WP ? 14 : 16), "the vmcnt of the fused-location prologue counts the weight ops of the first two tiles");
       const __amdgpu_buffer_rsrc_t rs_i = __builtin_amdgcn_make_buffer_rsrc(const_cast<uint8_t *>(p.fl_idx8), 0, (p.fl_n + 15) & ~15, 0x00020000);
       const int per_ = (((p.fl_n + 255) >> 8) + 15) & ~15, ipw = per_ >> 4;
       for (int i = wid * ipw; i < (wid + 1) * ipw; ++i)
@@ -549,7 +616,7 @@
       int *s_slot = reinterpret_cast<int *>(s_fl + 15360);
       int *s_wt = s_slot + 128;
       if (tid < 128) s_slot[tid] = -1;
-      asm volatile("s_waitcnt vmcnt(16)" ::: "memory");
+      asm volatile("s_waitcnt vmcnt(%0)" ::"n"(WPW * (NS - 1)) : "memory");
       const int per = (((p.fl_n + 255) >> 8) + 15) & ~15;
       const int nch = per >> 4;
       const int fl_e0 = tid * per;
@@ -646,6 +713,7 @@
     GEMM_PROBE(4);
   }
 #undef GB_TILE
+#undef GB_WP_FIX
 #undef GB_A_ADDR
 #undef GB_A_OFF
 #undef GB_ISSUE
diff --git a/tutel_amd/csrc/wpack.hip b/tutel_amd/csrc/wpack.hip
--- /dev/null
+++ b/tutel_amd/csrc/wpack.hip
@@ -0,0 +1,118 @@
+#include <stdlib.h>
+
+#include "common.h"
+#include "wpack_dev.h"
+
+static int g_wpack_mode = -2;
+static int wpack_mode_raw() {
+  if (g_wpack_mode == -2) {
+    const char *s = getenv("TUTEL_AMD_GEMM_WPACK");
+    g_wpack_mode = s ? atoi(s) : -1;
+    if (g_wpack_mode < -1 || g_wpack_mode > 1) g_wpack_mode = -1;
+  }
+  return g_wpack_mode;
+}
+int tutel_wpack_mode() { return wpack_mode_raw() == 1 ? 1 : 0; }
+
+extern "C" int tutel_amd_wpack_mode(int value) {
+  const int old = wpack_mode_raw();
+  if (value == -2) return old;
+  if (value < -1 || value > 1) {
+    tutel_set_error("tutel_amd_wpack_mode: value %d out of range (-2 query, -1 automatic = off, 0 never, 1 always where covered)", value);
+    return -3;
+  }
+  g_wpack_mode = value;
+  return old;
+}
+
+extern "C" size_t tutel_amd_wpack_bytes(int E, int N, int K) {
+  if (E < 1 || N < WPACK_BN || K < WPACK_BK || N % WPACK_BN != 0 || K % WPACK_BK != 0) return 0;
+  if ((long long)(N / WPACK_BN) * (K / WPACK_BK) * WPACK_TILE >= 0x7fffffffLL) return 0;
+  return (size_t)E * (N / WPACK_BN) * (K / WPACK_BK) * WPACK_TILE;
+}
+
+__global__ __launch_bounds__(256) void wpack_pack_kernel(const uint16_t *w, long long w_stride_e, int ldw, int E, int N, int K, unsigned char *out) {
+  const int nk = K / WPACK_BK;
+  const long long seg = (long long)blockIdx.x * 256 + threadIdx.x;
+  if (seg >= (long long)E * N * nk) return;
+  const int kt = (int)(seg % nk), n = (int)((seg / nk) % N), e = (int)(seg / nk / N);
+  const uint16_t *src = w + (size_t)e * w_stride_e + (size_t)n * ldw + (size_t)kt * WPACK_BK;
+  uint4 v[8];
+#pragma unroll
+  for (int c = 0; c < 8; ++c) v[c] = reinterpret_cast<const uint4 *>(src)[c];
+  uint32_t emax = 0;
+#pragma unroll
+  for (int c = 0; c < 8; ++c) {
+    const uint32_t d[4] = {v[c].x, v[c].y, v[c].z, v[c].w};
+#pragma unroll
+    for (int j = 0; j < 4; ++j) {
+      emax = max(emax, (d[j] >> 7) & 0xffu);
+      emax = max(emax, (d[j] >> 23) & 0xffu);
+    }
+  }
+  const int r = n % WPACK_BN;
+  unsigned char *tile = out + ((size_t)((size_t)e * (N / WPACK_BN) + n / WPACK_BN) * nk + kt) * WPACK_TILE;
+#pragma unroll
+  for (int c = 0; c < 8; ++c) {
+    const uint32_t d[4] = {v[c].x, v[c].y, v[c].z, v[c].w};
+    uint32_t sm[2] = {0u, 0u}, codes = 0u;
+#pragma unroll
+    for (int j = 0; j < 4; ++j) {
+      const uint32_t lo = d[j] & 0xffffu, hi = d[j] >> 16;
+      const uint32_t dl = emax - ((lo >> 7) & 0xffu), dh = emax - ((hi >> 7) & 0xffu);
+      const uint32_t cl = dl > 14u ? 15u : dl, ch = dh > 14u ? 15u : dh;
+      codes |= (15u - cl) << (4 * j);
+      codes |= (15u - ch) << (16 + 4 * j);
+      const uint32_t sl = ((lo >> 8) & 0x80u) | (lo & 0x7fu), sh = ((hi >> 8) & 0x80u) | (hi & 0x7fu);
+      sm[j >> 1] |= (sl | (sh << 8)) << (16 * (j & 1));
+    }
+    *reinterpret_cast<uint2 *>(tile + wpack_sm_off(r, c)) = make_uint2(sm[0], sm[1]);
+    *reinterpret_cast<uint32_t *>(tile + wpack_code_off(r, c)) = codes;
+  }
+  tile[WPACK_EMAX_OFF + r] = (unsigned char)emax;
+}
+
+__global__ __launch_bounds__(256) void wpack_unpack_kernel(const unsigned char *pack, const uint16_t *raw, int E, int N, int K, uint16_t *out) {
+  const int nc = K / 8;
+  const long long id = (long long)blockIdx.x * 256 + threadIdx.x;
+  if (id >= (long long)E * N * nc) return;
+  const int kc = (int)(id % nc), n = (int)((id / nc) % N), e = (int)(id / nc / N);
+  const int kt = kc >> 3, c = kc & 7, r = n % WPACK_BN;
+  const unsigned char *tile = pack + ((size_t)((size_t)e * (N / WPACK_BN) + n / WPACK_BN) * (K / WPACK_BK) + kt) * WPACK_TILE;
+  const uint2 sm = *reinterpret_cast<const uint2 *>(tile + wpack_sm_off(r, c));
+  const uint32_t codes = *reinterpret_cast<const uint32_t *>(tile + wpack_code_off(r, c));
+  uint32_t f[4];
+  wpack_frag8(sm.x, sm.y, codes, wpack_ebase(tile[WPACK_EMAX_OFF + r]), f);
+  const size_t at = ((size_t)e * N + n) * K + (size_t)kc * 8;
+  if (wpack_has_escape(codes)) {
+    const uint4 v = *reinterpret_cast<const uint4 *>(raw + at);
+    f[0] = v.x; f[1] = v.y; f[2] = v.z; f[3] = v.w;
+  }
+  *reinterpret_cast<uint4 *>(out + at) = make_uint4(f[0], f[1], f[2], f[3]);
+}
+
+extern "C" int tutel_amd_wpack_pack(const void *w_kmajor, int E, int N, int K, int ldw, void *out, tutel_stream_t stream) {
+  TUTEL_REQUIRE(tutel_amd_wpack_bytes(E, N, K) != 0, "tutel_amd_wpack_pack: shape E=%d N=%d K=%d is not covered (N %% 256, K %% 64)", E, N, K);
+  TUTEL_REQUIRE(w_kmajor != nullptr && out != nullptr && ((uintptr_t)w_kmajor & 15) == 0 && ((uintptr_t)out & 15) == 0,
+                "tutel_amd_wpack_pack: null or misaligned pointer");
+  TUTEL_REQUIRE(ldw >= K && ldw % 8 == 0, "tutel_amd_wpack_pack: ldw=%d must be >= K and keep rows 16-byte aligned", ldw);
+  const long long segs = (long long)E * N * (K / WPACK_BK);
+  TUTEL_REQUIRE((segs + 255) / 256 < 0x7fffffffLL, "tutel_amd_wpack_pack: grid too large");
+  hipLaunchKernelGGL(wpack_pack_kernel, dim3((unsigned)((segs + 255) / 256)), dim3(256), 0, (hipStream_t)stream,
+                     reinterpret_cast<const uint16_t *>(w_kmajor), (long long)N * ldw, ldw, E, N, K, reinterpret_cast<unsigned char *>(out));
+  TUTEL_CHECK_LAUNCH("tutel_amd_wpack_pack");
+  return 0;
+}
+
+extern "C" int tutel_amd_wpack_unpack(const void *pack, const void *raw, int E, int N, int K, void *out, tutel_stream_t stream) {
+  TUTEL_REQUIRE(tutel_amd_wpack_bytes(E, N, K) != 0, "tutel_amd_wpack_unpack: shape E=%d N=%d K=%d is not covered (N %% 256, K %% 64)", E, N, K);
+  TUTEL_REQUIRE(pack != nullptr && raw != nullptr && out != nullptr && ((uintptr_t)pack & 15) == 0 && ((uintptr_t)raw & 15) == 0 &&
+                    ((uintptr_t)out & 15) == 0, "tutel_amd_wpack_unpack: null or misaligned pointer");
+  const long long chunks = (long long)E * N * (K / 8);
+  TUTEL_REQUIRE((chunks + 255) / 256 < 0x7fffffffLL, "tutel_amd_wpack_unpack: grid too large");
+  hipLaunchKernelGGL(wpack_unpack_kernel, dim3((unsigned)((chunks + 255) / 256)), dim3(256), 0, (hipStream_t)stream,
+                     reinterpret_cast<const unsigned char *>(pack), reinterpret_cast<const uint16_t *>(raw), E, N, K,
+                     reinterpret_cast<uint16_t *>(out));
+  TUTEL_CHECK_LAUNCH("tutel_amd_wpack_unpack");
+  return 0;
+}
diff --git a/tutel_amd/csrc/wpack_dev.h b/tutel_amd/csrc/wpack_dev.h
--- /dev/null
+++ b/tutel_amd/csrc/wpack_dev.h
@@ -0,0 +1,29 @@
+#pragma once
+#include <stdint.h>
+
+#define WPACK_BN 256
+#define WPACK_BK 64
+#define WPACK_SM_BYTES (WPACK_BN * WPACK_BK)
+#define WPACK_CODE_OFF WPACK_SM_BYTES
+#define WPACK_CODE_BYTES (WPACK_BN * WPACK_BK / 2)
+#define WPACK_EMAX_OFF (WPACK_CODE_OFF + WPACK_CODE_BYTES)
+#define WPACK_TILE (WPACK_EMAX_OFF + WPACK_BN)
+
+__host__ __device__ __forceinline__ int wpack_sm_off(int r, int c) { return r * 64 + ((c ^ ((r >> 2) & 7)) << 3); }
+__host__ __device__ __forceinline__ int wpack_code_off(int r, int c) { return WPACK_CODE_OFF + r * 32 + ((c ^ (((r >> 3) & 3) << 1)) << 2); }
+
+__device__ __forceinline__ uint32_t wpack_ebase(uint32_t emax) { return (emax - 15u) * 0x00800080u; }
+
+__device__ __forceinline__ uint32_t wpack_bf16x2(uint32_t sm2, uint32_t code2, uint32_t ebase) {
+  return (sm2 & 0x807f807fu) | (code2 + ebase);
+}
+
+__device__ __forceinline__ bool wpack_has_escape(uint32_t codes) { return ((codes - 0x11111111u) & ~codes & 0x88888888u) != 0u; }
+
+__device__ __forceinline__ void wpack_frag8(uint32_t sm_lo, uint32_t sm_hi, uint32_t codes, uint32_t ebase, uint32_t (&f)[4]) {
+  const uint32_t c2 = codes >> 8;
+  f[0] = wpack_bf16x2(__builtin_amdgcn_perm(sm_lo, sm_lo, 0x01010000u), (codes & 0x000f000fu) << 7, ebase);
+  f[1] = wpack_bf16x2(__builtin_amdgcn_perm(sm_lo, sm_lo, 0x03030202u), (codes & 0x00f000f0u) << 3, ebase);
+  f[2] = wpack_bf16x2(__builtin_amdgcn_perm(sm_hi, sm_hi, 0x01010000u), (c2 & 0x000f000fu) << 7, ebase);
+  f[3] = wpack_bf16x2(__builtin_amdgcn_perm(sm_hi, sm_hi, 0x03030202u), (c2 & 0x00f000f0u) << 3, ebase);
+}
diff --git a/tutel_amd/experts/ffn.py b/tutel_amd/experts/ffn.py
--- a/tutel_amd/experts/ffn.py
+++ b/tutel_amd/experts/ffn.py
@@ -65,6 +65,17 @@
             hit = (key, t)
             self._store[name] = hit
         return hit[1]
+
+    def get_packed(self, name, w, transpose=True, dtype=None):
+        t = self.get(name, w, transpose=transpose, dtype=dtype)
+        if not t.is_cuda or t.dtype != torch.bfloat16 or ops.wpack_mode() != 1:
+            return t, None
+        hit = self._store[name]
+        if len(hit) == 2:
+            if torch.cuda.is_current_stream_capturing():
+                return t, None
+            hit = self._store[name] = (hit[0], t, ops.wpack_pack(t))
+        return t, hit[2]
 
     def invalidate(self):
         self._store.clear()
@@ -242,11 +253,23 @@
                 b2 = self._kmajor.get("b2.cast", b2[:, :self.output_dim], transpose=False, dtype=cast)
         return w1, b1, w2, b2, kmajor
 
+    def fused_packs(self, dtype):
+        if not _PREPACK or self.training or dtype != torch.bfloat16:
+            return None, None
+        w1, w2 = self.batched_fc1_w, self.batched_fc2_w
+        if torch.is_grad_enabled() and (w1.requires_grad or w2.requires_grad):
+            return None, None
+        cast = None if w1.dtype == dtype else dtype
+        p1 = self._kmajor.get_packed("fc1.cast", w1, transpose=False, dtype=cast)[1]
+        p2 = self._kmajor.get_packed("fc2", w2, transpose=True, dtype=cast)[1]
+        return p1, p2
+
     def forward_fused(self, x, ctx, a_layout=None, R=None, out=None, d_layout=None, slot_map=None, expert_range=None):
         counts, align = None, 1
         if getattr(ctx, "megablocks_size", 0) > 0:
             counts, align = ctx.dispatch_count, int(ctx.megablocks_size)
         w1, b1, w2, b2, w2_kmajor = self.fused_params(self.compute_dtype(x))
+        p1, p2 = self.fused_packs(w1.dtype) if expert_range is None else (None, None)
         if expert_range is not None:
             lo, hi = expert_range
             w1, w2 = w1[lo:hi], w2[lo:hi]
@@ -259,11 +282,12 @@
                 return y
         if slot_map is not None:
             h = ops.expert_gemm_gather(x, slot_map, w1, b1, True, self.fused_activation(), R,
-                                       row_counts=counts, row_align=align)
+                                       row_counts=counts, row_align=align, wpack=p1)
         else:
             h = ops.expert_gemm(x, w1, b1, True, act=self.fused_activation(), E_loc=w1.size(0), R=R,
-                                a_layout=a_layout, row_counts=counts, row_align=align)
-        return ops.expert_gemm(h, w2, b2, w2_kmajor, out=out, d_layout=d_layout, row_counts=counts, row_align=align)
+                                a_layout=a_layout, row_counts=counts, row_align=align, wpack=p1)
+        return ops.expert_gemm(h, w2, b2, w2_kmajor, out=out, d_layout=d_layout, row_counts=counts, row_align=align,
+                               wpack=p2 if w2_kmajor else None)
 
     def w2_kmajor_now(self):
         return _PREPACK and not self.training
diff --git a/tutel_amd/impls/ep_native.py b/tutel_amd/impls/ep_native.py
--- a/tutel_amd/impls/ep_native.py
+++ b/tutel_amd/impls/ep_native.py
@@ -513,6 +513,13 @@
     return ws
 
 
+def _pack_ptrs(ex, dtype, comm):
+    if comm is not None or not hasattr(ex, "fused_packs"):
+        return None, None
+    p1, p2 = ex.fused_packs(dtype)
+    return (p1.data_ptr() if p1 is not None else None), (p2.data_ptr() if p2 is not None else None)
+
+
 def forward(layer, x, crit, degree):
     ex = layer.experts
     W = layer.world_size
@@ -540,6 +547,7 @@
     a.w1, a.w2 = w1.data_ptr(), w2.data_ptr()
     a.b1 = b1.data_ptr() if b1 is not None else None
     a.b2 = b2.data_ptr() if b2 is not None else None
+    a.w1_pack, a.w2_pack = _pack_ptrs(ex, x.dtype, comm)
     a.y = y.data_ptr()
     mega = int(getattr(layer, "megablocks_size", 0))
     if mega > 0 and not with_comm:
@@ -613,6 +621,7 @@
         a.x, a.w1, a.w2 = x.data_ptr(), w1.data_ptr(), w2.data_ptr()
         a.b1 = b1.data_ptr() if b1 is not None else None
         a.b2 = b2.data_ptr() if b2 is not None else None
+        a.w1_pack, a.w2_pack = _pack_ptrs(ex, x.dtype, comm)
         a.y = y.data_ptr()
         if megablocks_size > 0 and not with_comm:
             a.row_counts, a.row_align = cnt.data_ptr(), int(megablocks_size)
diff --git a/tutel_amd/ops.py b/tutel_amd/ops.py
--- a/tutel_amd/ops.py
+++ b/tutel_amd/ops.py
@@ -231,8 +231,8 @@
 
 
 def expert_gemm(a, w, bias, w_kmajor, act="none", E_loc=None, R=None, a_layout=None, out=None,
-                d_layout=None, row_counts=None, row_align=1, mul=None):
-    _dev(a, w, bias, out, row_counts, mul)
+                d_layout=None, row_counts=None, row_align=1, mul=None, wpack=None):
+    _dev(a, w, bias, out, row_counts, mul, wpack)
     assert w.dim() == 3 and w.is_contiguous()
     if w_kmajor:
         El, N, K = w.shape
@@ -267,6 +267,15 @@
             E_loc, R, N, K, _code(a), ACT_CODES[act],
             _ptr(row_counts), int(row_align), _stream()), "tutel_amd_expert_gemm_glu")
         return out
+    if wpack is not None and w_kmajor:
+        _lib.check(_lib.lib().tutel_amd_expert_gemm_wpack(
+            _ptr(a), a_layout[0], a_layout[1], a_layout[2], a_layout[3],
+            _ptr(w), 1, w.stride(0), w.stride(1), _ptr(wpack),
+            _ptr(bias), (bias.stride(0) if bias is not None else 0),
+            _ptr(out), d_layout[0], d_layout[1], d_layout[2], d_layout[3],
+            E_loc, R, N, K, _code(a), ACT_CODES[act],
+            _ptr(row_counts), int(row_align), None, 0, None, _stream()), "tutel_amd_expert_gemm_wpack")
+        return out
     _lib.check(_lib.lib().tutel_amd_expert_gemm(
         _ptr(a), a_layout[0], a_layout[1], a_layout[2], a_layout[3],
         _ptr(w), int(bool(w_kmajor)), w.stride(0), w.stride(1),
@@ -296,8 +305,8 @@
 _zero_rows = {}
 
 
-def expert_gemm_gather(x, smap, w, bias, w_kmajor, act, R, row_counts=None, row_align=1):
-    _dev(x, smap, w, bias, row_counts)
+def expert_gemm_gather(x, smap, w, bias, w_kmajor, act, R, row_counts=None, row_align=1, wpack=None):
+    _dev(x, smap, w, bias, row_counts, wpack)
     assert x.dim() == 2 and x.is_contiguous() and w.dim() == 3 and w.is_contiguous() and w.dtype == x.dtype
     E_loc, N, K = (w.shape if w_kmajor else (w.shape[0], w.shape[2], w.shape[1]))
     assert x.shape[1] == K and smap.dtype == torch.int32 and smap.numel() == E_loc * R
@@ -307,6 +316,12 @@
     if z is None or z.numel() < K:
         z = _zero_rows[key] = torch.zeros([max(K, 8192)], dtype=x.dtype, device=x.device)
     out = torch.empty([E_loc, R, N], dtype=x.dtype, device=x.device)
+    if wpack is not None and w_kmajor:
+        _lib.check(_lib.lib().tutel_amd_expert_gemm_wpack(
+            _ptr(x), 0, 0, 1, x.stride(0), _ptr(w), 1, w.stride(0), w.stride(1), _ptr(wpack),
+            _ptr(bias), (bias.stride(0) if bias is not None else 0), _ptr(out), R * N, 0, R, N, E_loc, R, N, K, _code(x),
+            ACT_CODES[act], _ptr(row_counts), int(row_align), _ptr(smap), x.shape[0], _ptr(z), _stream()), "tutel_amd_expert_gemm_wpack")
+        return out
     _lib.check(_lib.lib().tutel_amd_expert_gemm_gather(
         _ptr(x), x.stride(0), _ptr(smap), x.shape[0], _ptr(z), _ptr(w), int(bool(w_kmajor)), w.stride(0), w.stride(1),
         _ptr(bias), (bias.stride(0) if bias is not None else 0), _ptr(out), R * N, N, E_loc, R, N, K, _code(x),
@@ -345,6 +360,44 @@
     return out
 
 
+def wpack_mode(value=-2):
+    old = _lib.lib().tutel_amd_wpack_mode(int(value))
+    if old == -3:
+        _lib.check(-1, "tutel_amd_wpack_mode")
+    return old
+
+
+def wpack_launches():
+    return int(_lib.lib().tutel_amd_wpack_launches())
+
+
+def wpack_bytes(E, N, K):
+    return int(_lib.lib().tutel_amd_wpack_bytes(int(E), int(N), int(K)))
+
+
+def wpack_pack(w):
+    _dev(w)
+    if w.dtype != torch.bfloat16 or w.dim() != 3 or not w.is_contiguous():
+        return None
+    E, N, K = w.shape
+    n = wpack_bytes(E, N, K)
+    if n == 0:
+        return None
+    out = torch.empty([n], dtype=torch.uint8, device=w.device)
+    _lib.check(_lib.lib().tutel_amd_wpack_pack(_ptr(w), E, N, K, w.stride(1), _ptr(out), _stream()), "tutel_amd_wpack_pack")
+    return out
+
+
+def wpack_unpack(pack, raw):
+    _dev(pack, raw)
+    assert raw.dtype == torch.bfloat16 and raw.dim() == 3 and raw.is_contiguous() and pack.dtype == torch.uint8
+    E, N, K = raw.shape
+    assert pack.numel() == wpack_bytes(E, N, K) != 0
+    out = torch.empty_like(raw)
+    _lib.check(_lib.lib().tutel_amd_wpack_unpack(_ptr(pack), _ptr(raw), E, N, K, _ptr(out), _stream()), "tutel_amd_wpack_unpack")
+    return out
+
+
 _OPT_ENV = {_lib.OPT_GEMM_IMPL: "TUTEL_AMD_GEMM_IMPL", _lib.OPT_GEMM_TILE: "TUTEL_AMD_GEMM_BIG", _lib.OPT_DECODE: "TUTEL_AMD_DECODE",
             _lib.OPT_EP_STAGE_GRID: "TUTEL_AMD_EP_STAGE_GRID", _lib.OPT_GEMM_PERSIST: "TUTEL_AMD_GEMM_PERSIST", _lib.OPT_EP_STREAMS: "TUTEL_AMD_EP_STREAMS",
             _lib.OPT_EP_CANARY: "TUTEL_AMD_EP_CANARY", _lib.OPT_GEMM_SPLITK: "TUTEL_AMD_GEMM_SPLITK", _lib.OPT_GEMM_STORE: "TUTEL_AMD_GEMM_STORE",
```
